# thygate/stable-diffusion-webui-depthmap-script

Measured on AMD Instinct MI355X. Metric: depth+stereo pairs/sec @1024x1024, higher is better.
Workload: dtype f16 (network) / f64 (stereo, normal map); 1 GPU; BASELINE config c3: MiDaS 3.1 DPT BEiT-L/16 512 forward (fp16, random-init weights seed 0, net 512x512, 1025 tokens) + depth->u16 + create_stereoimages(polylines_sharp, left-right, divergence 2.5%) + create_normalmap (Sobel 3) on 32 x 1024x1024 RGB per GPU, inputs resident in HBM; depth_network=dpt_beit_large_512, height=1024, width=1024, forward_launch=eager, library_convolutions=MIOpen, heuristic solver choice, overlap=single stream, parallelism=units sharded over 1 GPU(s), no data-path collective

## Files before the change

include/depthstereo.h:

```cpp
#ifndef DEPTHSTEREO_H
#define DEPTHSTEREO_H

#include <stddef.h>
#include <stdint.h>

#ifdef __cplusplus
extern "C" {
#endif

#define DS_VERSION 100

#define DS_OK            0
#define DS_EINVAL       -1
#define DS_EUNSUPPORTED -2
#define DS_EHIP         -3
#define DS_ENOMEM       -4

#define DS_DEPTH_U16 0
#define DS_DEPTH_F32 1
#define DS_DEPTH_F64 2

#define DS_FILL_NONE                0
#define DS_FILL_NAIVE               1
#define DS_FILL_NAIVE_INTERPOLATING 2
// ... 72 lines not shown
int ds_normalmap_gradient_blur_f32_wrap(ds_ctx *ctx, const float *depth, int n, int h, int w, int pre_blur, int post_blur, int invert,
                                        uint8_t *out, void *stream);

int ds_bilateral_u16(ds_ctx *ctx, const uint16_t *depth, int n, int h, int w, int radius, const double *ws, const double *wr,
                     int wrap, double *out, void *stream);

int ds_frame_luma_hist(ds_ctx *ctx, const uint8_t *frames, int n, int h, int w, int c, uint32_t *hist, void *stream);

int ds_temporal_smooth5_f32(ds_ctx *ctx, const float *src, int m, int64_t plane, int first, int count, int lo, int hi, float *out,
                            void *stream);

int ds_normalmap_selfcheck(ds_ctx *ctx, unsigned long long k0, unsigned long long stride, unsigned long long count,
                           unsigned long long *mismatches, void *stream);

int ds_depth_to_u16(ds_ctx *ctx, const float *pred, int n, int h, int w, int invert,
                    uint16_t *out, float *norm_out, void *stream);

int ds_colorize_u16(ds_ctx *ctx, const uint16_t *depth, int n, int h, int w, const double *vmin_vmax,
                    const uint8_t *lut_rgba, int lut_n, uint8_t *out, void *stream);

int ds_convert_to_i16(ds_ctx *ctx, const void *arr, int is_f64, int64_t count, uint16_t *out, void *stream);

#define DS_PIX_U8  0
#define DS_PIX_U16 1
#define DS_PIX_I32 2
#define DS_PIX_F32 3

int ds_resize_lanczos(ds_ctx *ctx, const void *src, int pix, int n, int in_h, int in_w, int64_t src_px_stride, int64_t src_row_stride,
                      int64_t src_img_stride, void *dst, int out_h, int out_w, const int32_t *h_bounds, const void *h_coeffs, int h_taps,
                      const int32_t *v_bounds, const void *v_coeffs, int v_taps, void *tmp, void *stream);

#define DS_CD_WIDEN       0
#define DS_CD_SINGLE_BAND 1
#define DS_CD_MULTI_BAND  2
#define DS_CD_WORKSPACE_BLOCKS 256
int ds_custom_depth_to_f64(ds_ctx *ctx, const void *src, int pix, int n, int h, int w, int64_t src_px_stride, int64_t src_row_stride,
                           int64_t src_img_stride, int rule, double *out, double *workspace, void *stream);

#define DS_DTYPE_F16  1
#define DS_DTYPE_BF16 2
#define DS_DTYPE_F32  3

int ds_attention_fwd(ds_ctx *ctx, const void *qk, const void *vt, const void *bias_packed, void *out,
                     int B, int Np, int H, int n_valid, float scale, int dtype, void *stream);

int ds_attention_bias_pack(ds_ctx *ctx, const float *bias, int H, int n, int Np, int dtype, void *packed, void *stream);

int ds_attention_reload_env(void);

int ds_preprocess_bicubic(ds_ctx *ctx, const void *images, void *out, int batch, int in_h, int in_w, int out_h, int out_w,
                          int flip_channels, const float *mean, const float *std, int dtype, void *stream);

int ds_residual_layernorm(ds_ctx *ctx, const void *x, const void *branch, const void *gamma, const void *ln_weight,
                          const void *ln_bias, void *x_out, void *h_out, int64_t rows, int channels, float eps, int dtype,
                          void *stream);

int ds_reassemble_readout(ds_ctx *ctx, const void *proj, const void *clsvec, void *out, int batch, int tokens, int channels,
                          int dtype, void *stream);

int ds_bias_act_nhwc(ds_ctx *ctx, const void *x, const void *bias, const void *res1, const void *res2, void *out,
                     int64_t elements, int channels, int relu, int dtype, void *stream);

int ds_group_norm_nchw(ds_ctx *ctx, const void *x, const void *gamma, const void *beta, const void *res, void *out, int n, int channels,
                       int hw, int groups, float eps, int relu, int dtype, void *stream);

int ds_linear(ds_ctx *ctx, const void *x, const void *w, const void *bias, void *y, int64_t rows, int64_t out_features,
              int64_t in_features, int64_t ldy, int act, int dtype, void *stream);

int ds_linear_residual(ds_ctx *ctx, const void *x, const void *w, const void *bias, const void *gamma, const void *res, void *y,
                       int64_t rows, int64_t out_features, int64_t in_features, int dtype, void *stream);

int ds_linear_vt(ds_ctx *ctx, const void *w_v, const void *h, void *vt, int64_t channels, int64_t batch, int64_t tokens,
                 int64_t in_features, int dtype, void *stream);

int ds_linear_qkv(ds_ctx *ctx, const void *h, const void *w_qk, const void *b_qk, const void *w_v, void *qk, void *vt,
                  int64_t batch, int64_t tokens, int64_t qk_features, int64_t v_channels, int64_t in_features, int dtype, void *stream);

int ds_linear_shuffle(ds_ctx *ctx, const void *x, const void *w, const void *bias, void *y, int64_t pixels, int64_t in_features,
                      int width, int stride, int out_channels, int dtype, void *stream);

int ds_linear_readout(ds_ctx *ctx, const void *x, const void *w_tok, const void *cls_vec, void *y, int64_t images,
                      int64_t tokens_padded, int64_t tokens, int64_t out_features, int64_t in_features, int dtype, void *stream);

int ds_row_stats(ds_ctx *ctx, const void *x, void *stats, int64_t rows, int channels, float eps, int dtype, void *stream);
int ds_linear_ln(ds_ctx *ctx, const void *x, const void *w_scaled, const float *colsum, const void *bias, const void *stats, void *y,
                 int64_t rows, int64_t out_features, int64_t in_features, int64_t ldy, int act, int dtype, void *stream);
int ds_linear_vt_ln(ds_ctx *ctx, const void *w_v_scaled, const float *colsum, const void *x, const void *stats, void *vt,
                    int64_t channels, int64_t batch, int64_t tokens, int64_t in_features, int dtype, void *stream);

int ds_linear_reload_env(void);

int ds_conv3x3_nhwc(ds_ctx *ctx, const void *x, const void *w, const void *bias, const void *res1, const void *res2, void *y,
                    int batch, int height, int width, int in_channels, int out_channels, int act, int dtype, void *stream);

int ds_conv3x3_nhwc_circular(ds_ctx *ctx, const void *x, const void *w, const void *bias, const void *res1, const void *res2, void *y,
                             int batch, int height, int width, int in_channels, int out_channels, int act, int dtype, void *stream);

int ds_upsample_bilinear_nhwc(ds_ctx *ctx, const void *in, void *out, int batch, int channels, int in_h, int in_w,
                              int out_h, int out_w, int align_corners, int dtype, void *stream);

int ds_dpt_head_tail(ds_ctx *ctx, const void *x, int batch, int in_h, int in_w, int out_h, int out_w,
                     const void *conv3_wfrag, const float *conv3_bias, const float *conv1_weight, float conv1_bias,
                     int relu_out, void *out, int dtype, void *stream);

int ds_dpt_head_tail_circular(ds_ctx *ctx, const void *x, int batch, int in_h, int in_w, int out_h, int out_w,
                              const void *conv3_wfrag, const float *conv3_bias, const float *conv1_weight, float conv1_bias,
                              int relu_out, void *out, int dtype, void *stream);

int ds_gconv3x3_nhwc_f32(ds_ctx *ctx, const float *x, const float *w_gtio, const float *bias, float *y, int batch, int height, int width,
                         int channels, int channels_per_group, int relu, void *stream);
int ds_add_relu_f32(ds_ctx *ctx, const float *a, const float *b, float *y, int64_t count, void *stream);

int ds_bias_act_f32(ds_ctx *ctx, const float *x, const float *bias, const float *res, float *y, int64_t pixels, int channels, int relu,
                    void *stream);

int ds_dwconv_nhwc(ds_ctx *ctx, const void *x, const float *w, const float *bias_in, const float *bias, void *y, int batch, int in_h,
                   int in_w, int channels, int out_h, int out_w, int kernel, int stride, int pad_top, int pad_left, int dtype, void *stream);
int ds_relu_cat_f32(ds_ctx *ctx, const float *a, const float *b, float *y, int batch, int64_t plane, int channels_a, int channels_b, int layout,
                    void *stream);

int ds_boost_blend(ds_ctx *ctx, float *dst, int64_t dst_row_stride, int height, int width, const void *patches,
                   int n_patches, const float *preds, int pred_size, const float *mask_template, int mask_size,
                   void *stream);

int ds_preprocess_bicubic_rows(ds_ctx *ctx, const void *images, void *rows, int batch, int in_h, int in_w, int out_h, int out_w,
                               int flip_channels, const float *mean, const float *std, int patch, int n_pad, int kpad, int dtype,
                               void *stream);

int ds_tokens_fixup(ds_ctx *ctx, void *tokens, const void *cls, int batch, int n_pad, int n_valid, int channels, int dtype, void *stream);

int ds_upsample_bicubic_to_f32(ds_ctx *ctx, const void *in, void *out, int batch, int in_h, int in_w, int out_h, int out_w, int dtype,
                               void *stream);

int ds_im2col3x3_s2_nhwc(ds_ctx *ctx, const void *x, void *rows, int batch, int height, int width, int channels, int circular, int dtype,
                         void *stream);

#ifdef __cplusplus
}
#endif
#endif
```

stable-diffusion-webui-depthmap-script_amd/csrc/ds_linear.hip:

```cpp
#include "ds_common.h"

#include <stdlib.h>
#include <atomic>
#include <type_traits>

typedef _Float16 lf16x8 __attribute__((ext_vector_type(8)));
typedef __bf16 lbf16x8 __attribute__((ext_vector_type(8)));
typedef _Float16 lf16x4 __attribute__((ext_vector_type(4)));
typedef __bf16 lbf16x4 __attribute__((ext_vector_type(4)));
typedef float lf32x16 __attribute__((ext_vector_type(16)));
typedef float lf32x4 __attribute__((ext_vector_type(4)));

#if defined(DS_EXPERIMENTS) && defined(DS_LIN_MFMA32)
#define LN_MF16 0
#else
#define LN_MF16 1
#endif

#define LN_THREADS 512
#define LN_LDS_BYTES 131072
#define LN_HALF 16384
#define LN_B_BASE 65536

template <int BF16> struct ln_traits;
template <> struct ln_traits<0> {
    typedef _Float16 T; typedef lf16x8 V8; typedef lf16x4 V4;
    static __device__ __forceinline__ lf32x16 mfma(V8 a, V8 b, lf32x16 c) { return __builtin_amdgcn_mfma_f32_32x32x16_f16(a, b, c, 0, 0, 0); }
    static __device__ __forceinline__ lf32x4 mfma16(V8 a, V8 b, lf32x4 c) { return __builtin_amdgcn_mfma_f32_16x16x32_f16(a, b, c, 0, 0, 0); }
    static __device__ __forceinline__ V8 relu(V8 v)
    {
        typedef unsigned lu32x4 __attribute__((ext_vector_type(4)));
        const lu32x4 x = __builtin_bit_cast(lu32x4, v);
        unsigned r0, r1, r2, r3;
        asm("v_pk_max_f16 %0, %1, 0" : "=v"(r0) : "v"(x[0]));
        asm("v_pk_max_f16 %0, %1, 0" : "=v"(r1) : "v"(x[1]));
        asm("v_pk_max_f16 %0, %1, 0" : "=v"(r2) : "v"(x[2]));
        asm("v_pk_max_f16 %0, %1, 0" : "=v"(r3) : "v"(x[3]));
        return __builtin_bit_cast(V8, (lu32x4){r0, r1, r2, r3});
    }
};
template <> struct ln_traits<1> {
    typedef __bf16 T; typedef lbf16x8 V8; typedef lbf16x4 V4;
    static __device__ __forceinline__ lf32x16 mfma(V8 a, V8 b, lf32x16 c) { return __builtin_amdgcn_mfma_f32_32x32x16_bf16(a, b, c, 0, 0, 0); }
    static __device__ __forceinline__ lf32x4 mfma16(V8 a, V8 b, lf32x4 c) { return __builtin_amdgcn_mfma_f32_16x16x32_bf16(a, b, c, 0, 0, 0); }
    static __device__ __forceinline__ V8 relu(V8 v)
    {
        typedef unsigned lu32x4 __attribute__((ext_vector_type(4)));
        lu32x4 x = __builtin_bit_cast(lu32x4, v);
#pragma unroll
        for (int i = 0; i < 4; ++i) {
            const unsigned neg = (x[i] >> 15) & 0x00010001u;
            x[i] &= ~(neg * 0xffffu);
        }
        return __builtin_bit_cast(V8, x);
    }
};

struct LinParams {
    const void *x, *w, *bias;
    const void *res1, *res2;
    const void *zeros;
    void *y;
    int M, N, K;
    int nbm, nbn;
    int bnw;
    int ablate;
    int stagger;
    int H, W, C, cpt, magic;
    long long ldy;
    const void *gamma;
    int early;
    int n_main;
    int vt_np, vt_c;
    unsigned vt_magic;
    int ps_w, ps_s, ps_c;
    unsigned ps_w_magic, ps_c_magic;
    int rd_np, rd_n, rd_dummy;
    unsigned rd_magic;
    float *rg_ws;
    int *rg_cnt;
    int rg_ksl;
    int th_nrb;
    int kt_kind;
    const float2 *ln_stats;
    const float *ln_colsum;
    const void *x1, *w1;
    void *y1;
    int seg_t0, M1, nbm1, nbn1;
};
typedef const __attribute__((address_space(4))) LinParams *LinParamsK;
__device__ __forceinline__ LinParamsK ln_kernarg()
{
    LinParamsK pk = (LinParamsK)__builtin_amdgcn_kernarg_segment_ptr();
    asm volatile("" : "+s"(pk));
    return pk;
}

__device__ __forceinline__ void ln_tile_origin(const int nbm, const int nbn, const int M, const int bnw, const int tile, int &bm0, int &bn0)
{
    const int grp8 = tile / (8 * nbn), rem8 = tile - grp8 * (8 * nbn);
    const int rows8 = min(8, nbm - 8 * grp8);
    const int bn = rem8 / rows8, bm = 8 * grp8 + (rem8 - bn * rows8);
    bm0 = min(bm * 256, M - 256);
    bn0 = bn * bnw;
}
__device__ __forceinline__ void ln_tile_origin(const LinParams &P, const int tile, int &bm0, int &bn0)
{
    ln_tile_origin(P.nbm, P.nbn, P.M, P.bnw, tile, bm0, bn0);
}

template <int VT>
__device__ __forceinline__ size_t ln_out_off(const LinParams &P, const int row, const int col)
{
    if (VT == 0) return (size_t)row * P.ldy + col;
    if (VT == 1) {
        const unsigned b = __umulhi((unsigned)col, P.vt_magic);
        const unsigned n = (unsigned)col - b * (unsigned)P.vt_np;
        return ((size_t)b * P.vt_c + row) * (size_t)P.vt_np + n;
    }
    if (VT == 2) {
        const unsigned q = __umulhi((unsigned)row, P.ps_w_magic), x = (unsigned)row - q * (unsigned)P.ps_w;
        const unsigned t = __umulhi((unsigned)col, P.ps_c_magic), co = (unsigned)col - t * (unsigned)P.ps_c;
        const unsigned ky = t / (unsigned)P.ps_s, kx = t - ky * (unsigned)P.ps_s;
        const size_t opix = ((size_t)q * P.ps_s + ky) * ((size_t)P.ps_w * P.ps_s) + (size_t)x * P.ps_s + kx;
        return opix * (size_t)P.ps_c + co;
    }
    const unsigned b = __umulhi((unsigned)row, P.rd_magic), t = (unsigned)row - b * (unsigned)P.rd_np;
    const bool live = t >= 1u && t < (unsigned)P.rd_n;
    const size_t orow = live ? (size_t)b * (size_t)(P.rd_n - 1) + (t - 1u) : (size_t)P.rd_dummy;
    return orow * (size_t)P.ldy + col;
}
template <int VT>
__device__ __forceinline__ size_t ln_res_off(const LinParams &P, const int row, const int col)
{
    if (VT != 3) return ln_out_off<VT>(P, row, col);
    const unsigned b = __umulhi((unsigned)row, P.rd_magic);
    return (size_t)b * (size_t)P.ldy + col;
}

__device__ __forceinline__ float ln_gelu(float v)
{
    const float u = fminf(fabsf(v), 6.0f);
    float q = 1.8896206483987044e-06f;
    q = __builtin_fmaf(q, u, -6.268127617659047e-05f);
    q = __builtin_fmaf(q, u, 0.000938866869546473f);
    q = __builtin_fmaf(q, u, -0.008539456874132156f);
    q = __builtin_fmaf(q, u, 0.054020676761865616f);
    q = __builtin_fmaf(q, u, 0.45840978622436523f);
    q = __builtin_fmaf(q, u, 1.1512691974639893f);
    q = __builtin_fmaf(q, u, 0.9999943375587463f);
    const float h = __builtin_amdgcn_exp2f(-q);
    return __builtin_fmaf(-u, h, fmaxf(v, 0.0f));
}
typedef float lf32x2 __attribute__((ext_vector_type(2)));
__device__ __forceinline__ lf32x2 ln_gelu2(lf32x2 v)
{
    const lf32x2 u = {fminf(fabsf(v[0]), 6.0f), fminf(fabsf(v[1]), 6.0f)};
    lf32x2 q = {1.8896206483987044e-06f, 1.8896206483987044e-06f};
#define LN_PK(c) q = __builtin_elementwise_fma(q, u, (lf32x2){c, c})
    LN_PK(-6.268127617659047e-05f); LN_PK(0.000938866869546473f); LN_PK(-0.008539456874132156f); LN_PK(0.054020676761865616f);
    LN_PK(0.45840978622436523f); LN_PK(1.1512691974639893f); LN_PK(0.9999943375587463f);
#undef LN_PK
    const lf32x2 h = {__builtin_amdgcn_exp2f(-q[0]), __builtin_amdgcn_exp2f(-q[1])};
    const lf32x2 r = {fmaxf(v[0], 0.0f), fmaxf(v[1], 0.0f)};
    return __builtin_elementwise_fma(-u, h, r);
}

__device__ __forceinline__ void ln_dma_s(const void *base_uniform, unsigned voff, unsigned lds_uniform)
{
    asm volatile("s_mov_b32 m0, %2\n\ts_nop 0\n\tglobal_load_lds_dwordx4 %0, %1" ::"v"(voff), "s"(base_uniform), "s"(lds_uniform) : "memory");
}
__device__ __forceinline__ void ln_dma_v(const void *ptr, unsigned lds_uniform)
{
    asm volatile("s_mov_b32 m0, %1\n\ts_nop 0\n\tglobal_load_lds_dwordx4 %0, off" ::"v"(ptr), "s"(lds_uniform) : "memory");
}

#ifdef DS_EXPERIMENTS
#define LN_ABLATE(bit) (P.ablate & (bit))
#define LN_STAGGER() (P.stagger)
#else
#define LN_ABLATE(bit) 0
#define LN_STAGGER() 0
#endif
#define LN_WAIT_VM(n) asm volatile("s_waitcnt vmcnt(" #n ")" ::: "memory")
template <int N> __device__ __forceinline__ void ln_wait_vm() { asm volatile("s_waitcnt vmcnt(%0)" ::"n"(N) : "memory"); }
#define LN_WAIT_LGKM0() asm volatile("s_waitcnt lgkmcnt(0)" ::: "memory")
#define LN_BARRIER()                              \
    do {                                          \
        __builtin_amdgcn_sched_barrier(0);        \
        __builtin_amdgcn_s_barrier();             \
        __builtin_amdgcn_sched_barrier(0);        \
    } while (0)

template <int BF16, int EPI, int CONV, int RES, int VT = 0, int NH = 0>
__global__ __launch_bounds__(LN_THREADS) void k_linear256(LinParams P)
{
    typedef ln_traits<BF16> TR;
    typedef typename TR::T T;
    typedef typename TR::V8 V8;
    extern __shared__ __attribute__((aligned(1024))) unsigned char lds[];

    const int tid = threadIdx.x;
    const int lane = tid & 63;
    const int wid = __builtin_amdgcn_readfirstlane(tid >> 6);
    const int wr = wid >> 2, wc = wid & 3;

    const int nwg = P.n_main;
    const int K = P.K;
    const int rowbytes = (CONV ? P.C : K) * (int)sizeof(T);

    unsigned srcA[2], srcB[2];
    int rowA[2];
#pragma unroll
    for (int i = 0; i < 2; ++i) {
        const int c = 2 * wid + i;
        const int j = 8 * c + (lane >> 3);
        const int slot = (lane & 7) ^ ((j >> 1) & 7);
        rowA[i] = (j >> 6) * 128 + (j & 63);
        srcA[i] = (unsigned)rowA[i] * (unsigned)rowbytes + slot * 16;
        const int col = NH ? j : (j >> 5) * 64 + (j & 31);
        srcB[i] = (unsigned)col * (unsigned)K * (unsigned)sizeof(T) + slot * 16;
    }
    const unsigned a_half = 64u * (unsigned)rowbytes;
    const unsigned b_half = NH ? 0u : 32u * (unsigned)K * (unsigned)sizeof(T);
    const unsigned lds_stage = (unsigned)(size_t)(__attribute__((address_space(3))) void *)lds + (unsigned)(2 * wid) * 1024u;

    static_assert(VT != 4 || (EPI == 0 && CONV == 0 && RES == 0 && NH == 0), "the two-segment tile list is built for the plain dense epilogue");
    int bm0 = 0, bn0 = 0;
    int seg = 0;
    const unsigned char *xb = nullptr, *wb = nullptr;
    unsigned okA = 0;
    auto set_tile = [&](const int orig) {
        const int xcd = orig & 7, q8 = nwg >> 3, r8 = nwg & 7;
        const int tile = (xcd < r8 ? xcd * (q8 + 1) : r8 * (q8 + 1) + (xcd - r8) * q8) + (orig >> 3);
        if constexpr (VT == 4) {
            const LinParamsK pk = ln_kernarg();
            const int t0 = pk->seg_t0;
            seg = tile >= t0 ? 1 : 0;
            if (seg) {
                ln_tile_origin(pk->nbm1, pk->nbn1, pk->M1, 256, tile - t0, bm0, bn0);
                xb = (const unsigned char *)pk->x1 + (size_t)bm0 * rowbytes;
                wb = (const unsigned char *)pk->w1 + (size_t)bn0 * K * sizeof(T);
                return;
            }
        }
        ln_tile_origin(P, tile, bm0, bn0);
        xb = (const unsigned char *)P.x + (size_t)bm0 * rowbytes;
        wb = (const unsigned char *)P.w + (size_t)bn0 * K * sizeof(T);
        if (CONV) {
            okA = 0;
#pragma unroll
            for (int i = 0; i < 2; ++i)
#pragma unroll
                for (int h = 0; h < 2; ++h) {
                    const unsigned pix = (unsigned)(bm0 + rowA[i] + 64 * h) % (unsigned)(P.H * P.W);
                    const int py = (int)(pix / (unsigned)P.W), px = (int)(pix % (unsigned)P.W);
                    const unsigned bits = (py > 0 ? 1u : 0u) | 2u | (py < P.H - 1 ? 4u : 0u) | (px > 0 ? 8u : 0u) | 16u | (px < P.W - 1 ? 32u : 0u);
                    okA |= bits << (6 * (2 * h + i));
                }
        }
    };

#define LN_STAGE(kind, kt, s)                                                                                            \
    do {                                                                                                                 \
        unsigned koff_ = (unsigned)(kt) * 128u;                                                                          \
        const unsigned dst_ = ((kind) >> 1) * LN_B_BASE + ((kind) & 1) * 2 * LN_HALF + (s) * LN_HALF + lds_stage;   \
        int dy_ = 0, dx_ = 0, aoff_ = (int)koff_;                                                                        \
        long wrapy_ = 0, wrapx_ = 0;      \
        if (CONV) {               \
            const int cc_ = ((kt) * 7282) >> 16, tap_ = (kt) - 9 * cc_;       \
            dy_ = ((tap_ * 11) >> 5) - 1; dx_ = tap_ - 3 * (dy_ + 1) - 1;                                                \
            aoff_ = cc_ * 128 + (dy_ * P.W + dx_) * rowbytes;                                                            \
            koff_ = (unsigned)(tap_ * P.cpt + cc_) * 128u;                            \
            if (CONV >= 3) { wrapy_ = -(long)dy_ * ((long)P.H * P.W * rowbytes); wrapx_ = -(long)dx_ * ((long)P.W * rowbytes); } \
        }                                                                                                                \
                   \
        const unsigned char *ub_ = ((kind) < 2) ? xb + ((long)aoff_ + (long)(((kind) & 1) * a_half))                     \
                                                : wb + (size_t)(((kind) & 1) * b_half + koff_);                          \
        _Pragma("unroll") for (int i_ = 0; i_ < 2; ++i_) {                                                               \
            if (CONV >= 3 && (kind) < 2) {    \
                const unsigned sh_ = 6 * (2 * ((kind) & 1) + i_);     \
                const long wrap_ = (((okA >> (sh_ + dy_ + 1)) & 1u) ? 0l : wrapy_) + (((okA >> (sh_ + 4 + dx_)) & 1u) ? 0l : wrapx_); \
                ln_dma_v(ub_ + ((long)srcA[i_] + wrap_), dst_ + i_ * 1024);                                              \
            } else if (CONV && (kind) < 2) {                                                                             \
                const unsigned sh_ = 6 * (2 * ((kind) & 1) + i_);                                                        \
                const unsigned ok_ = (okA >> (sh_ + dy_ + 1)) & (okA >> (sh_ + 4 + dx_)) & 1u;                           \
                const unsigned char *g_ = ok_ ? ub_ + (size_t)srcA[i_] : (const unsigned char *)P.zeros;                 \
                ln_dma_v(g_, dst_ + i_ * 1024);                                                                          \
            } else {                                                                                                     \
                ln_dma_s(ub_, ((kind) < 2) ? srcA[i_] : srcB[i_], dst_ + i_ * 1024);                                     \
            }                                                                                                            \
        }                                                                                                                \
    } while (0)

    constexpr bool MF16 = LN_MF16 && CONV == 0;
    constexpr int NKS = MF16 ? 2 : 4;
    unsigned offA[NKS], offB[NKS];
#pragma unroll
    for (int ks = 0; ks < NKS; ++ks) {
        const int lrow = MF16 ? (lane & 15) : (lane & 31);
        const unsigned sl = (unsigned)((MF16 ? 4 * ks + (lane >> 4) : 2 * ks + (lane >> 5)) ^ ((lane >> 1) & 7)) << 4;
        offA[ks] = (unsigned)(wr * 64 + lrow) * 128u + sl;
        offB[ks] = LN_B_BASE + (unsigned)(wc * 32 + lrow) * 128u + sl;
    }
    const int c8 = MF16 ? 16 * ((lane >> 4) & 1) + 8 * (lane >> 5) : 8 * (lane >> 5);
    constexpr int NBK = MF16 ? 1 : 2;
    constexpr int NBIAS = 2 * NBK;
    V8 bv[2][2];
#define LN_NULL_BIAS() (!P.bias || (VT == 4 && seg))
#define LN_LOAD_BIAS()                                                                                                   \
    do {                                                                                                                 \
        const T *bias_ = LN_NULL_BIAS() ? (const T *)nullptr : (const T *)P.bias;                                        \
        _Pragma("unroll") for (int hb_ = 0; hb_ < 2; ++hb_) _Pragma("unroll") for (int k_ = 0; k_ < NBK; ++k_) {         \
            const int c_ = bn0 + (NH ? wc * 32 : wc * 64 + hb_ * 32) + c8 + 16 * k_;                                     \
            bv[hb_][k_] = *(const V8 *)(bias_ ? bias_ + c_ : (const T *)P.w);                                            \
        }                                                                                                                \
    } while (0)
#define LN_ZERO_NULL_BIAS()                                                                                              \
    do {                                                                                                                 \
        if (LN_NULL_BIAS()) {                                                                                            \
            _Pragma("unroll") for (int hb_ = 0; hb_ < 2; ++hb_) _Pragma("unroll") for (int k_ = 0; k_ < NBK; ++k_)       \
                _Pragma("unroll") for (int t_ = 0; t_ < 8; ++t_) bv[hb_][k_][t_] = (T)0.f;                               \
        }                                                                                                                \
    } while (0)
    V8 fa[2][2][4];
    V8 fb[2][4];
    lf32x16 acc[2][2][2];
    V8 fa16[2][4][2];
    V8 fb16[2][2][2];
    lf32x4 acc16[2][4][2][2];

#define LN_READ_A(h, s)                                                                                                  \
    do {                                                                                                                 \
        if constexpr (MF16) {                                                                                            \
            _Pragma("unroll") for (int rb_ = 0; rb_ < 4; ++rb_) _Pragma("unroll") for (int ks_ = 0; ks_ < 2; ++ks_)      \
                fa16[h][rb_][ks_] = *(const V8 *)(lds + offA[ks_] + ((h) * 2 * LN_HALF + (s) * LN_HALF + rb_ * 2048));   \
        } else {                                                                                                         \
            _Pragma("unroll") for (int rb_ = 0; rb_ < 2; ++rb_) _Pragma("unroll") for (int ks_ = 0; ks_ < 4; ++ks_)      \
                fa[h][rb_][ks_] = *(const V8 *)(lds + offA[ks_] + ((h) * 2 * LN_HALF + (s) * LN_HALF + rb_ * 4096));     \
        }                                                                                                                \
    } while (0)
#define LN_RELU_A(h)                                                                                                     \
    do {                                                                                                                 \
        if constexpr (CONV == 2 || CONV == 4) {                                                                          \
            _Pragma("unroll") for (int rb_ = 0; rb_ < 2; ++rb_) _Pragma("unroll") for (int ks_ = 0; ks_ < 4; ++ks_)      \
                fa[h][rb_][ks_] = TR::relu(fa[h][rb_][ks_]);                                                             \
        }                                                                                                                \
    } while (0)
#define LN_READ_B(h, s)                                                                                                  \
    do {                                                                                                                 \
        if constexpr (MF16) {                                                                                            \
            _Pragma("unroll") for (int cb_ = 0; cb_ < 2; ++cb_) _Pragma("unroll") for (int ks_ = 0; ks_ < 2; ++ks_)      \
                if (!(NH && (h) == 1)) fb16[h][cb_][ks_] = *(const V8 *)(lds + offB[ks_] + ((h) * 2 * LN_HALF + (s) * LN_HALF + cb_ * 2048)); \
        } else {                                                                                                         \
            _Pragma("unroll") for (int ks_ = 0; ks_ < 4; ++ks_)                                                          \
// ... 32 lines not shown
    } while (0)
#define LN_MEM(READ, STAGE)                                                                                              \
    do { READ; STAGE; } while (0)

    auto iteration = [&](const int i, auto kind_c) {
        constexpr int KIND = decltype(kind_c)::value;
        constexpr bool LAST = KIND == 1;
        const int e2 = 2 * i + 2, o2 = 2 * i + 3;
#define LN_WAIT_HEAD()                                                                                                   \
        do {                                                                                                             \
            if constexpr (KIND == 2) { if constexpr (NH) LN_WAIT_VM(18); else LN_WAIT_VM(26); }                          \
            else if constexpr (KIND == 1) ln_wait_vm<10 + NBIAS>();                                                   \
            else LN_WAIT_VM(10);                                                                                         \
        } while (0)
        LN_MEM(LN_READ_B(0, 0), LN_STAGE(1, 2 * i + 1, 1)); LN_WAIT_HEAD();
        LN_PHASE_END(0, 0);
        if constexpr (!LAST) { LN_MEM(LN_READ_B(1, 0), LN_STAGE(0, e2, 0)); LN_WAIT_HEAD(); } else { LN_READ_B(1, 0); ln_wait_vm<8 + NBIAS>(); }
        LN_PHASE_END(0, 1);
        if constexpr (!LAST) { LN_MEM(LN_READ_A(1, 0), LN_STAGE(2, e2, 0)); LN_RELU_A(1); LN_WAIT_HEAD(); } else { LN_READ_A(1, 0); LN_RELU_A(1); ln_wait_vm<6 + NBIAS>(); }
        LN_PHASE_END(1, 1);
        if constexpr (!LAST) { LN_MEM(LN_READ_A(0, 1), LN_STAGE(3, e2, 0)); LN_RELU_A(0); LN_WAIT_HEAD(); } else { LN_READ_A(0, 1); LN_RELU_A(0); ln_wait_vm<4 + NBIAS>(); }
        LN_PHASE_END(1, 0);
        if constexpr (!LAST) { LN_MEM(LN_READ_B(0, 1), LN_STAGE(1, e2, 0)); LN_WAIT_HEAD(); } else { LN_READ_B(0, 1); ln_wait_vm<2 + NBIAS>(); }
        LN_PHASE_END(0, 0);
#undef LN_WAIT_HEAD
        if constexpr (!LAST) { LN_MEM(LN_READ_B(1, 1), LN_STAGE(0, o2, 1)); LN_WAIT_VM(10); } else { LN_READ_B(1, 1); LN_WAIT_VM(0); }
        LN_PHASE_END(0, 1);
        if constexpr (!LAST) { LN_MEM(LN_READ_A(1, 1), LN_STAGE(2, o2, 1)); LN_RELU_A(1); LN_WAIT_VM(10); } else { LN_READ_A(1, 1); LN_RELU_A(1); }
        LN_PHASE_END(1, 1);
        if constexpr (!LAST) { LN_MEM(LN_READ_A(0, 0), LN_STAGE(3, o2, 1)); LN_RELU_A(0); LN_WAIT_VM(10); }
        LN_PHASE_END(1, 0);
    };
    if (LN_STAGGER() > 0 && ((blockIdx.x >> 3) & 1)) {
        const unsigned long long t0 = wall_clock64();
        while (wall_clock64() - t0 < (unsigned long long)LN_STAGGER()) __builtin_amdgcn_s_sleep(32);
    }
    const bool early = P.early != 0;
    bool stores_ahead = false;
    set_tile(blockIdx.x);
    LN_PROLOGUE();
    for (int orig = blockIdx.x;;) {
    if constexpr (MF16) {
#pragma unroll
        for (int a = 0; a < 2; ++a)
#pragma unroll
            for (int b = 0; b < 4; ++b)
#pragma unroll
                for (int c = 0; c < 2; ++c)
#pragma unroll
                    for (int d = 0; d < 2; ++d)
#pragma unroll
                        for (int r = 0; r < 4; ++r) acc16[a][b][c][d][r] = 0.f;
    } else {
#pragma unroll
        for (int a = 0; a < 2; ++a)
#pragma unroll
            for (int b = 0; b < 2; ++b)
#pragma unroll
                for (int c = 0; c < 2; ++c)
#pragma unroll
                    for (int r = 0; r < 16; ++r) acc[a][b][c][r] = 0.f;
    }
    if (!early) LN_WAIT_VM(10);
    else if (stores_ahead) { if constexpr (NH) LN_WAIT_VM(18); else LN_WAIT_VM(26); }
    else LN_WAIT_VM(0);
    LN_BARRIER();
    LN_READ_A(0, 0);
    LN_WAIT_LGKM0();
    LN_RELU_A(0);
    if (wr == 1) LN_BARRIER();
    if (LN_ABLATE(2)) {
        LN_LOAD_BIAS();
        LN_WAIT_VM(0);
        if (wr == 0) LN_BARRIER();
    } else {
        int i0 = 0;
        if (early && ni >= 2) { iteration(0, std::integral_constant<int, 2>()); i0 = 1; }
        for (int i = i0; i < ni - 1; ++i) iteration(i, std::integral_constant<int, 0>());
        LN_LOAD_BIAS();
        iteration(ni - 1, std::integral_constant<int, 1>());
        if (wr == 0) LN_BARRIER();
    }
    const int cbm0 = bm0, cbn0 = bn0;
    const bool cseg = VT == 4 && seg != 0;
    const int next = orig + (int)gridDim.x;
    int elane = lane;
    if constexpr (VT == 4) asm volatile("" : "+v"(elane));
    const int hi8 = 8 * (elane >> 5);
    const int ec8 = MF16 ? 16 * ((elane >> 4) & 1) + 8 * (elane >> 5) : 8 * (elane >> 5);
    LN_ZERO_NULL_BIAS();
    T *yb = (T *)P.y;
    unsigned s1_np = 0, s1_c = 0, s1_magic = 0;
    if constexpr (VT == 4) {
        if (cseg) {
            const LinParamsK pk = ln_kernarg();
            yb = (T *)pk->y1;
            s1_np = (unsigned)pk->vt_np; s1_c = (unsigned)pk->vt_c; s1_magic = pk->vt_magic;
        }
    }
    auto tile_out_off = [&](const int row, const int col, const size_t o0) -> size_t {
        if constexpr (VT == 4) {
            if (!cseg) return o0;
            const unsigned b = __umulhi((unsigned)col, s1_magic), n = (unsigned)col - b * s1_np;
            return ((size_t)b * s1_c + row) * (size_t)s1_np + n;
        } else return VT ? ln_out_off<VT>(P, row, col) : o0;
    };
    if constexpr (CONV >= 3) asm volatile("" : "+s"(yb));
    const T *r1 = (const T *)P.res1, *r2 = (const T *)P.res2;
    if (early && next < nwg) {
#pragma unroll
        for (int hb = 0; hb < 2; ++hb)
#pragma unroll
            for (int k = 0; k < NBK; ++k) {
                asm volatile("" ::"v"(bv[hb][k]));
            }
        set_tile(next);
        LN_PROLOGUE();
    }

    if constexpr (MF16) {
        V8 gv[2];
        if (EPI == 3) {
#pragma unroll
            for (int hb = 0; hb < 2; ++hb) gv[hb] = *(const V8 *)((const T *)P.gamma + cbn0 + (NH ? wc * 32 : wc * 64 + hb * 32) + ec8);
        }
        constexpr int NHB = NH ? 1 : 2;
        const int wcol = NH ? wc * 32 : wc * 64;
#pragma unroll
        for (int ha = 0; ha < 2; ++ha)
#pragma unroll
            for (int rb = 0; rb < 4; ++rb) {
                const int row = cbm0 + wr * 128 + ha * 64 + rb * 16 + (elane & 15);
                const int col = cbn0 + wcol + ec8;
                const size_t o0 = (size_t)row * P.ldy + col;
                V8 ra[2], rb2[2];
                constexpr bool LNF = EPI == 4 || EPI == 5;
                float2 st_row = {1.f, 0.f};
                float cs_row = 0.f;
                static_assert(!LNF || VT == 0 || VT == 1, "the folded LayerNorm exists for the row-major and the V^T store only");
                if (LNF && VT == 0) st_row = P.ln_stats[row];
                if (LNF && VT == 1) cs_row = P.ln_colsum[row];
#pragma unroll
                for (int hb = 0; hb < NHB; ++hb) {
                    if (RES >= 1) ra[hb] = *(const V8 *)(r1 + (VT == 3 ? ln_res_off<VT>(P, row, col + hb * 32) : o0 + hb * 32));
                    if (RES >= 2) rb2[hb] = *(const V8 *)(r2 + o0 + hb * 32);
                }
#pragma unroll
                for (int hb = 0; hb < NHB; ++hb) {
                    float v[8];
#pragma unroll
                    for (int t = 0; t < 4; ++t) {
                        const float fa = acc16[ha][rb][hb][0][t], fb = acc16[ha][rb][hb][1][t];
                        const auto sw = __builtin_amdgcn_permlane16_swap(__float_as_uint(fa), __float_as_uint(fb), false, false);
                        v[t] = __uint_as_float(sw[0]);
                        v[4 + t] = __uint_as_float(sw[1]);
                    }
                    V8 o;
                    if (LNF) {
                        const int c0 = col + hb * 32;
                        if (!VT) {
                            const float4 s0 = *(const float4 *)(P.ln_colsum + c0), s1 = *(const float4 *)(P.ln_colsum + c0 + 4);
                            const float sc[8] = {s0.x, s0.y, s0.z, s0.w, s1.x, s1.y, s1.z, s1.w};
#pragma unroll
                            for (int t = 0; t < 8; ++t) v[t] = __builtin_fmaf(v[t], st_row.x, st_row.y * sc[t]);
                        } else {
                            const float4 *sp = (const float4 *)(P.ln_stats + c0);
                            const float4 q0 = sp[0], q1 = sp[1], q2 = sp[2], q3 = sp[3];
                            const float rs[8] = {q0.x, q0.z, q1.x, q1.z, q2.x, q2.z, q3.x, q3.z};
                            const float nm[8] = {q0.y, q0.w, q1.y, q1.w, q2.y, q2.w, q3.y, q3.w};
#pragma unroll
                            for (int t = 0; t < 8; ++t) v[t] = __builtin_fmaf(v[t], rs[t], nm[t] * cs_row);
                        }
                    }
#pragma unroll
                    for (int t = 0; t < 8; t += 2) {
                        lf32x2 u = {v[t] + (float)bv[hb][0][t], v[t + 1] + (float)bv[hb][0][t + 1]};
                        if (EPI == 3) u *= (lf32x2){(float)gv[hb][t], (float)gv[hb][t + 1]};
                        if (RES >= 1) u += (lf32x2){(float)ra[hb][t], (float)ra[hb][t + 1]};
                        if (RES >= 2) u += (lf32x2){(float)rb2[hb][t], (float)rb2[hb][t + 1]};
                        if (EPI == 1 || EPI == 5) u = ln_gelu2(u);
                        if (EPI == 2) u = (lf32x2){fmaxf(u[0], 0.f), fmaxf(u[1], 0.f)};
                        o[t] = (T)u[0];
                        o[t + 1] = (T)u[1];
                    }
                    T *dst = yb + tile_out_off(row, col + hb * 32, o0 + hb * 32);
                    if (!LN_ABLATE(1)) *(V8 *)dst = o;
                    else asm volatile("" ::"v"(o));
// ... 362 lines not shown
        const int j = 8 * (wid & 3) + (lane >> 3);
        srcA = (unsigned)j * rowbytes + (unsigned)(((lane & 7) ^ ((j >> 1) & 7)) << 4) + (unsigned)(wid >> 2) * 128u;
    }
#pragma unroll
    for (int i = 0; i < 2; ++i) {
        const int j = 8 * ((2 * wid + i) & 7) + (lane >> 3);
        srcB[i] = (unsigned)j * rowbytes + (unsigned)(((lane & 7) ^ ((j >> 1) & 7)) << 4) + (unsigned)(wid >> 2) * 128u;
    }
    const unsigned char *xb = (const unsigned char *)P.x + (size_t)row0 * rowbytes;
    const unsigned char *wb = (const unsigned char *)P.w + (size_t)col0 * rowbytes;
    const unsigned lds0 = (unsigned)(size_t)(__attribute__((address_space(3))) void *)lds;
#define TH_STAGE(st_)                                                                                                    \
    do {                                                                                                                 \
        const int sc_ = min((st_), nst - 1);                 \
        const unsigned sl_ = lds0 + (unsigned)((st_) % S) * RG_SLOT;                                                      \
        const unsigned char *xa_ = xb + (size_t)sc_ * 256, *wa_ = wb + (size_t)sc_ * 256;                                 \
        ln_dma_s(xa_, srcA, sl_ + (unsigned)wid * 1024u);                                                                 \
        ln_dma_s(wa_, srcB[0], sl_ + 8192u + (unsigned)(2 * wid) * 1024u);                                                \
        ln_dma_s(wa_, srcB[1], sl_ + 8192u + (unsigned)(2 * wid + 1) * 1024u);                                            \
    } while (0)
    const bool mw = wid < 2;
    unsigned offA[8], offB[8];
#pragma unroll
    for (int u = 0; u < 8; ++u) {
        const int j = u >> 2, ks = u & 3;
        const unsigned sl = (unsigned)((LN_MF16 ? 4 * (ks >> 1) + (lane >> 4) : 2 * ks + hi) ^ ((lane >> 1) & 7)) << 4;
        const int lrow = LN_MF16 ? 16 * (ks & 1) + (lane & 15) : l31;
        offA[u] = (unsigned)j * 4096u + (unsigned)lrow * 128u + sl;
        offB[u] = 8192u + (unsigned)j * 8192u + (unsigned)((wid & 1) * 32 + lrow) * 128u + sl;
    }
    LN_SMALL_ACC(mine);
    const int e_row = row0 + LN_SMALL_ROW;
    const int e_cb = col0 + (wid & 1) * 32 + LN_SMALL_COL;
    V8 e_bv[2], e_gv[2], e_rv[2];
    if (mw) {
#pragma unroll
        for (int k = 0; k < 2; ++k) {
            const int row = e_row + LN_SMALL_DROW(k), col = e_cb + LN_SMALL_DCOL(k);
            if (P.bias) e_bv[k] = *(const V8 *)((const T *)P.bias + col);
            if (EPI == 3) e_gv[k] = *(const V8 *)((const T *)P.gamma + col);
            if (RES >= 1) e_rv[k] = *(const V8 *)((const T *)P.res1 + (size_t)row * P.ldy + col);
        }
    }
#pragma unroll
    for (int t = 0; t < S - 1; ++t) TH_STAGE(t);
    V8 fa0[8], fb0[8], fa1[8], fb1[8];
#define TH_READ(fa_, fb_, st_)                                                                                           \
    do {                                                                                                                 \
        const unsigned char *sb_ = lds + ((st_) % S) * RG_SLOT;                                                          \
        _Pragma("unroll") for (int u = 0; u < 8; ++u) {                                                                  \
            fa_[u] = *(const V8 *)(sb_ + offA[u]);                                                                       \
            fb_[u] = *(const V8 *)(sb_ + offB[u]);                                                                       \
        }                                                                                                                \
    } while (0)
#define TH_STEP(ca_, cb_, na_, nb_, st_)                                                                                 \
    do {                                                                                                                 \
        LN_WAIT_VM(9);                                                                                                   \
        LN_BARRIER();                                                                                                    \
        TH_STAGE((st_) + S - 1);                                                                                         \
        if (mw) {                                                                                                        \
            TH_READ(na_, nb_, (st_) + 1);                                                                                \
            __builtin_amdgcn_sched_barrier(0);                                                                           \
            LN_SMALL_MMA(mine, cb_, ca_, 0);                                                                             \
            LN_SMALL_MMA(mine, cb_, ca_, 4);                                                                             \
            __builtin_amdgcn_sched_barrier(0);                                                                           \
            LN_WAIT_LGKM0();                                                                                             \
            __builtin_amdgcn_sched_barrier(0);                                                                           \
        }                                                                                                                \
    } while (0)
    LN_WAIT_VM(12);
    LN_BARRIER();
    if (mw) {
        TH_READ(fa0, fb0, 0);
        __builtin_amdgcn_sched_barrier(0);
        LN_WAIT_LGKM0();
        __builtin_amdgcn_sched_barrier(0);
    }
    int st = 0;
    for (; st + 1 < nst; st += 2) {
        TH_STEP(fa0, fb0, fa1, fb1, st);
        TH_STEP(fa1, fb1, fa0, fb0, st + 1);
    }
    if (st < nst) TH_STEP(fa0, fb0, fa1, fb1, st);
#undef TH_STEP
#undef TH_READ
#undef TH_STAGE
    LN_WAIT_VM(0);
    if (!mw) return;

    T *yb = (T *)P.y;
#pragma unroll
    for (int k = 0; k < 2; ++k) {
        const int row = e_row + LN_SMALL_DROW(k), col = e_cb + LN_SMALL_DCOL(k);
        const size_t off = (size_t)row * P.ldy + col;
        V8 bv;
        if (P.bias) bv = e_bv[k];
        else {
#pragma unroll
            for (int t = 0; t < 8; ++t) bv[t] = (T)0.f;
        }
        float v[8];
        LN_SMALL_V(v, mine, k);
        if (EPI == 4 || EPI == 5) {
            const float2 stt = P.ln_stats[row];
            const float4 s0 = *(const float4 *)(P.ln_colsum + col), s1 = *(const float4 *)(P.ln_colsum + col + 4);
            const float sc[8] = {s0.x, s0.y, s0.z, s0.w, s1.x, s1.y, s1.z, s1.w};
#pragma unroll
            for (int t = 0; t < 8; ++t) v[t] = __builtin_fmaf(v[t], stt.x, stt.y * sc[t]);
        }
        V8 o;
#pragma unroll
        for (int t = 0; t < 8; t += 2) {
            lf32x2 u = {v[t] + (float)bv[t], v[t + 1] + (float)bv[t + 1]};
            if (EPI == 3) u *= (lf32x2){(float)e_gv[k][t], (float)e_gv[k][t + 1]};
            if (RES >= 1) u += (lf32x2){(float)e_rv[k][t], (float)e_rv[k][t + 1]};
            if (EPI == 1 || EPI == 5) u = ln_gelu2(u);
            if (EPI == 2) u = (lf32x2){fmaxf(u[0], 0.f), fmaxf(u[1], 0.f)};
            o[t] = (T)u[0];
            o[t + 1] = (T)u[1];
        }
        *(V8 *)(yb + off) = o;
    }
}

struct LinOptions { int early, grid, ragged, ragged_den, ragged_ring, ragged_ksplit, ragged_ksplit_min, ragged_ksplit_keep, ragged_pipe, ragged_thin; };
static LinOptions g_lin_options;
static std::atomic<int> g_lin_options_state{0};
static void ln_read_options()
{
    auto geti = [](const char *name, int dflt) { const char *e = getenv(name); return e ? atoi(e) : dflt; };
    LinOptions o;
    o.early = geti("DS_LIN_EARLY", 1);
    o.grid = geti("DS_LIN_GRID", 0);
    o.ragged = geti("DS_LIN_RAGGED", 1);
    o.ragged_den = geti("DS_LIN_RAGGED_DEN", 4);
    o.ragged_ring = geti("DS_LIN_RAGGED_RING", 0);
    o.ragged_ksplit = geti("DS_LIN_RAGGED_KSPLIT", 1);
    o.ragged_ksplit_min = geti("DS_LIN_RAGGED_KSPLIT_MIN", 32);
    o.ragged_ksplit_keep = geti("DS_LIN_RAGGED_KSPLIT_KEEP", 8);
    if (o.ragged_ksplit_keep < 1) o.ragged_ksplit_keep = 1;
    o.ragged_pipe = geti("DS_LIN_RAGGED_PIPE", 1);
    o.ragged_thin = geti("DS_LIN_RAGGED_THIN", 1);
    g_lin_options = o;
    g_lin_options_state.store(1, std::memory_order_release);
}
static const LinOptions &ln_options()
{
    if (!g_lin_options_state.load(std::memory_order_acquire)) ln_read_options();
    return g_lin_options;
}
DS_API int ds_linear_reload_env(void)
{
    ln_read_options();
    return DS_OK;
}

#define LN_RG_COUNTER_BYTES 4096
#define LN_RG_MAX_WG 1024
static int ln_ragged_workspace(ds_ctx *ctx, int grid, hipStream_t stream)
{
    if (grid > LN_RG_MAX_WG) return 1;
    if (ctx->lin_ws && ctx->lin_ws_cleared == ctx->lin_ws) return DS_OK;
    hipStreamCaptureStatus cap = hipStreamCaptureStatusNone;
    if (hipStreamIsCapturing(stream, &cap) != hipSuccess || cap != hipStreamCaptureStatusNone) { (void)hipGetLastError(); return 1; }
    if (!ctx->lin_ws) {
        const int rc = ds_ctx_reserve(ctx, &ctx->lin_ws, &ctx->lin_ws_bytes, LN_RG_COUNTER_BYTES + (size_t)LN_RG_MAX_WG * 32768);
        if (rc != DS_OK) return rc;
    }
    DS_HIP_CHECK(hipMemsetAsync(ctx->lin_ws, 0, LN_RG_COUNTER_BYTES, stream));
    DS_HIP_CHECK(hipStreamSynchronize(stream));
    ctx->lin_ws_cleared = ctx->lin_ws;
    return DS_OK;
}

static int ln_ksplit_arch_ok(ds_ctx *ctx)
{
    static std::atomic<uint64_t> checked{0}, ok{0};
    const uint64_t bit = 1ull << (ctx->device & 63);
    if (!(checked.load(std::memory_order_acquire) & bit)) {
        hipDeviceProp_t prop;
        bool good = false;
        if (hipGetDeviceProperties(&prop, ctx->device) == hipSuccess)
            good = strncmp(prop.gcnArchName, "gfx950", 6) == 0 || strncmp(prop.gcnArchName, "gfx942", 6) == 0;
        else (void)hipGetLastError();
        if (good) ok.fetch_or(bit, std::memory_order_relaxed);
        checked.fetch_or(bit, std::memory_order_release);
    }
    return (ok.load(std::memory_order_relaxed) & bit) != 0;
}

template <int BF16, int EPI, int CONV, int RES, int VT = 0, int NH = 0>
static int ln_launch(ds_ctx *ctx, const LinParams &P0, hipStream_t stream)
{
    static std::atomic<uint64_t> attr_done{0};
    auto fn = k_linear256<BF16, EPI, CONV, RES, VT, NH>;
    DS_HIP_CHECK(hipSetDevice(ctx->device));
    const uint64_t bit = 1ull << (ctx->device & 63);
    if (!(attr_done.load(std::memory_order_relaxed) & bit)) {
        DS_HIP_CHECK(hipFuncSetAttribute((const void *)fn, hipFuncAttributeMaxDynamicSharedMemorySize, LN_LDS_BYTES));
        if constexpr (CONV == 0) {
            DS_HIP_CHECK(hipFuncSetAttribute((const void *)k_linear_ragged<BF16, EPI, RES, VT, 3>, hipFuncAttributeMaxDynamicSharedMemorySize, 3 * RG_SLOT));
            DS_HIP_CHECK(hipFuncSetAttribute((const void *)k_linear_ragged<BF16, EPI, RES, VT, 6>, hipFuncAttributeMaxDynamicSharedMemorySize, 6 * RG_SLOT));
            DS_HIP_CHECK(hipFuncSetAttribute((const void *)k_linear_ragged<BF16, EPI, RES, VT, 6, 1>, hipFuncAttributeMaxDynamicSharedMemorySize, 6 * RG_SLOT));
            if constexpr (VT == 0 && RES <= 1)
                DS_HIP_CHECK(hipFuncSetAttribute((const void *)k_linear_thin<BF16, EPI, RES>, hipFuncAttributeMaxDynamicSharedMemorySize, 6 * RG_SLOT));
        }
// ... 165 lines not shown
    P.ablate = getenv("DS_LIN_ABLATE") ? atoi(getenv("DS_LIN_ABLATE")) : 0;
    P.stagger = getenv("DS_LIN_STAGGER_US") ? (int)(atof(getenv("DS_LIN_STAGGER_US")) * 100.0) : 0;
#endif
    return dtype == DS_DTYPE_F16 ? ln_dispatch_dense<0>(ctx, P, act, (hipStream_t)stream) : ln_dispatch_dense<1>(ctx, P, act, (hipStream_t)stream);
}

DS_API int ds_linear_residual(ds_ctx *ctx, const void *x, const void *w, const void *bias, const void *gamma, const void *res, void *y,
                              int64_t rows, int64_t out_features, int64_t in_features, int dtype, void *stream)
{
    DS_REQUIRE(ctx && x && w && y && res, DS_EINVAL, "ds_linear_residual: null argument");
    DS_REQUIRE(rows >= 256 && rows < (1ll << 31) - 256, DS_EINVAL, "ds_linear_residual: rows must be >= 256 (one tile)");
    DS_REQUIRE(out_features > 0 && out_features % 256 == 0, DS_EINVAL, "ds_linear_residual: out_features must be a multiple of 256");
    DS_REQUIRE(in_features >= 128 && in_features % 128 == 0 && in_features <= 16384, DS_EINVAL,
               "ds_linear_residual: in_features must be a multiple of 128 (<= 16384)");
    DS_REQUIRE(dtype == DS_DTYPE_F16 || dtype == DS_DTYPE_BF16, DS_EINVAL, "ds_linear_residual: dtype must be f16 or bf16");
    DS_REQUIRE(((uintptr_t)x & 15) == 0 && ((uintptr_t)w & 15) == 0 && ((uintptr_t)y & 15) == 0 && ((uintptr_t)res & 15) == 0 &&
               ((uintptr_t)bias & 15) == 0 && ((uintptr_t)gamma & 15) == 0 && y != res,
               DS_EINVAL, "ds_linear_residual: x, w, y, res, bias and gamma must be 16-byte aligned, and y must not alias res");
    LinParams P;
    memset(&P, 0, sizeof(P));
    P.x = x; P.w = w; P.bias = bias; P.gamma = gamma; P.res1 = res; P.y = y;
    P.M = (int)rows; P.N = (int)out_features; P.K = (int)in_features;
    P.nbm = (int)((rows + 255) / 256); P.nbn = (int)(out_features / 256);
    P.ldy = out_features;
    P.kt_kind = DS_KT_LINEAR_RESIDUAL;
    hipStream_t st = (hipStream_t)stream;
    if (dtype == DS_DTYPE_F16) return gamma ? ln_launch<0, 3, 0, 1>(ctx, P, st) : ln_launch<0, 0, 0, 1>(ctx, P, st);
    return gamma ? ln_launch<1, 3, 0, 1>(ctx, P, st) : ln_launch<1, 0, 0, 1>(ctx, P, st);
}

template <int CIRC>
static int ln_conv3x3(const char *NAME, ds_ctx *ctx, const void *x, const void *w, const void *bias, const void *res1, const void *res2, void *y,
                      int batch, int height, int width, int in_channels, int out_channels, int act, int dtype, void *stream)
{
    DS_REQUIRE(ctx && x && w && y, DS_EINVAL, "%s: null argument", NAME);
    DS_REQUIRE(batch > 0 && height > 0 && width > 0 && height < 32768 && width < 32768, DS_EINVAL, "%s: bad image shape", NAME);
    DS_REQUIRE((int64_t)batch * height * width < (1ll << 31) - 256 && (int64_t)batch * height * width >= 256, DS_EINVAL,
               "%s: batch * height * width must be in [256, 2^31)", NAME);
    DS_REQUIRE(in_channels >= 64 && in_channels % 64 == 0 && (9 * in_channels / 64) % 2 == 0 && in_channels <= 4096, DS_EINVAL,
               "%s: in_channels must be a multiple of 128 (<= 4096)", NAME);
    DS_REQUIRE(out_channels > 0 && out_channels % 128 == 0, DS_EINVAL, "%s: out_channels must be a multiple of 128", NAME);
    DS_REQUIRE(out_channels % 256 == 0 || (!res1 && !res2), DS_EUNSUPPORTED,
               "%s: residual operands need out_channels to be a multiple of 256 (the 128-column tiles have no residual epilogue)", NAME);
    DS_REQUIRE(act == 0 || act == 2 || act == 6, DS_EINVAL, "%s: act must be 0 (none), 2 (ReLU) or 6 (ReLU, and ReLU on x)", NAME);
    DS_REQUIRE(dtype == DS_DTYPE_F16 || dtype == DS_DTYPE_BF16, DS_EINVAL, "%s: dtype must be f16 or bf16", NAME);
    DS_REQUIRE(((uintptr_t)x & 15) == 0 && ((uintptr_t)w & 15) == 0 && ((uintptr_t)y & 15) == 0 && (!bias || ((uintptr_t)bias & 15) == 0) &&
               ((uintptr_t)res1 & 15) == 0 && ((uintptr_t)res2 & 15) == 0,
               DS_EINVAL, "%s: x, w, y, bias, res1 and res2 must be 16-byte aligned", NAME);
    int rc = ds_ctx_reserve(ctx, &ctx->zero_line, &ctx->zero_line_bytes, 256);
    if (rc != DS_OK) return rc;
    if (!ctx->zero_line_cleared) {
        DS_HIP_CHECK(hipMemsetAsync(ctx->zero_line, 0, 256, (hipStream_t)stream));
        DS_HIP_CHECK(hipStreamSynchronize((hipStream_t)stream));
        ctx->zero_line_cleared = 1;
    }
    LinParams P;
    memset(&P, 0, sizeof(P));
    if (!res1 && res2) { res1 = res2; res2 = nullptr; }
    P.x = x; P.w = w; P.bias = bias; P.res1 = res1; P.res2 = res2; P.y = y; P.zeros = ctx->zero_line;
    P.M = batch * height * width; P.N = out_channels; P.K = 9 * in_channels;
    P.nbm = (P.M + 255) / 256; P.nbn = out_channels % 256 == 0 ? out_channels / 256 : out_channels / 128;
    P.H = height; P.W = width; P.C = in_channels; P.cpt = in_channels / 64; P.magic = 65536 / P.cpt + 1;
    for (int kt = 0; kt < P.K / 64; ++kt)
        DS_REQUIRE(((kt * 7282) >> 16) == kt / 9, DS_EUNSUPPORTED, "%s: K-tile arithmetic does not cover %d channels", NAME, in_channels);
    P.ldy = out_channels;
    P.kt_kind = DS_KT_CONV3X3;
#ifdef DS_EXPERIMENTS
    P.ablate = getenv("DS_LIN_ABLATE") ? atoi(getenv("DS_LIN_ABLATE")) : 0;
    P.stagger = getenv("DS_LIN_STAGGER_US") ? (int)(atof(getenv("DS_LIN_STAGGER_US")) * 100.0) : 0;
#endif
    return dtype == DS_DTYPE_F16 ? ln_dispatch_conv<0, CIRC>(ctx, P, act, (hipStream_t)stream) : ln_dispatch_conv<1, CIRC>(ctx, P, act, (hipStream_t)stream);
}

DS_API int ds_conv3x3_nhwc(ds_ctx *ctx, const void *x, const void *w, const void *bias, const void *res1, const void *res2, void *y,
                           int batch, int height, int width, int in_channels, int out_channels, int act, int dtype, void *stream)
{
    return ln_conv3x3<0>("ds_conv3x3_nhwc", ctx, x, w, bias, res1, res2, y, batch, height, width, in_channels, out_channels, act, dtype, stream);
}

DS_API int ds_conv3x3_nhwc_circular(ds_ctx *ctx, const void *x, const void *w, const void *bias, const void *res1, const void *res2, void *y,
                                    int batch, int height, int width, int in_channels, int out_channels, int act, int dtype, void *stream)
{
    return ln_conv3x3<1>("ds_conv3x3_nhwc_circular", ctx, x, w, bias, res1, res2, y, batch, height, width, in_channels, out_channels, act, dtype, stream);
}

DS_API int ds_linear_vt(ds_ctx *ctx, const void *w_v, const void *h, void *vt, int64_t channels, int64_t batch, int64_t tokens,
                        int64_t in_features, int dtype, void *stream)
{
    DS_REQUIRE(ctx && w_v && h && vt, DS_EINVAL, "ds_linear_vt: null argument");
    DS_REQUIRE(channels >= 256, DS_EINVAL, "ds_linear_vt: channels must be >= 256 (one tile)");
    DS_REQUIRE(batch > 0 && tokens > 0 && tokens % 8 == 0 && (batch * tokens) % 256 == 0 && batch * tokens < (1ll << 31) - 256, DS_EINVAL,
               "ds_linear_vt: tokens must be a multiple of 8 and batch * tokens a multiple of 256");
    DS_REQUIRE(batch * tokens * tokens < (1ll << 32), DS_EUNSUPPORTED, "ds_linear_vt: batch * tokens^2 must stay below 2^32");
    DS_REQUIRE(in_features >= 128 && in_features % 128 == 0 && in_features <= 16384, DS_EINVAL,
               "ds_linear_vt: in_features must be a multiple of 128 (<= 16384)");
    DS_REQUIRE(dtype == DS_DTYPE_F16 || dtype == DS_DTYPE_BF16, DS_EINVAL, "ds_linear_vt: dtype must be f16 or bf16");
    DS_REQUIRE(((uintptr_t)w_v & 15) == 0 && ((uintptr_t)h & 15) == 0 && ((uintptr_t)vt & 15) == 0, DS_EINVAL,
               "ds_linear_vt: w_v, h and vt must be 16-byte aligned");
    LinParams P;
    memset(&P, 0, sizeof(P));
    P.x = w_v; P.w = h; P.y = vt;
    P.M = (int)channels; P.N = (int)(batch * tokens); P.K = (int)in_features;
    P.nbm = (int)((channels + 255) / 256); P.nbn = (int)(batch * tokens / 256);
    P.ldy = batch * tokens;
    P.vt_np = (int)tokens; P.vt_c = (int)channels; P.vt_magic = (unsigned)((1ull << 32) / (unsigned long long)tokens + 1ull);
    P.kt_kind = DS_KT_LINEAR_VT;
    hipStream_t st = (hipStream_t)stream;
    return dtype == DS_DTYPE_F16 ? ln_launch<0, 0, 0, 0, 1>(ctx, P, st) : ln_launch<1, 0, 0, 0, 1>(ctx, P, st);
}

DS_API int ds_linear_qkv(ds_ctx *ctx, const void *h, const void *w_qk, const void *b_qk, const void *w_v, void *qk, void *vt,
                         int64_t batch, int64_t tokens, int64_t qk_features, int64_t v_channels, int64_t in_features, int dtype, void *stream)
{
    DS_REQUIRE(ctx && h && w_qk && w_v && qk && vt, DS_EINVAL, "ds_linear_qkv: null argument");
    DS_REQUIRE(batch > 0 && tokens > 0 && tokens % 8 == 0 && (batch * tokens) % 256 == 0 && batch * tokens < (1ll << 31) - 256, DS_EINVAL,
               "ds_linear_qkv: tokens must be a multiple of 8 and batch * tokens a multiple of 256");
    DS_REQUIRE(batch * tokens * tokens < (1ll << 32), DS_EUNSUPPORTED, "ds_linear_qkv: batch * tokens^2 must stay below 2^32");
    DS_REQUIRE(qk_features > 0 && qk_features % 256 == 0, DS_EINVAL, "ds_linear_qkv: qk_features must be a multiple of 256");
    DS_REQUIRE(v_channels >= 256 && v_channels < (1ll << 31) - 256, DS_EINVAL, "ds_linear_qkv: v_channels must be >= 256 (one tile)");
    DS_REQUIRE(in_features >= 128 && in_features % 128 == 0 && in_features <= 16384, DS_EINVAL,
               "ds_linear_qkv: in_features must be a multiple of 128 (<= 16384)");
    DS_REQUIRE((batch * tokens / 256) * (qk_features / 256) + ((v_channels + 255) / 256) * (batch * tokens / 256) < (1ll << 31), DS_EINVAL,
               "ds_linear_qkv: too many tiles");
    DS_REQUIRE(dtype == DS_DTYPE_F16 || dtype == DS_DTYPE_BF16, DS_EINVAL, "ds_linear_qkv: dtype must be f16 or bf16");
    DS_REQUIRE(((uintptr_t)h & 15) == 0 && ((uintptr_t)w_qk & 15) == 0 && ((uintptr_t)w_v & 15) == 0 && ((uintptr_t)qk & 15) == 0 &&
               ((uintptr_t)vt & 15) == 0 && (!b_qk || ((uintptr_t)b_qk & 15) == 0), DS_EINVAL,
               "ds_linear_qkv: h, w_qk, w_v (the LDS-DMA sources), qk, vt and b_qk must be 16-byte aligned");
    const int64_t rows = batch * tokens;
    LinParams PQ, PV;
    memset(&PQ, 0, sizeof(PQ));
    memset(&PV, 0, sizeof(PV));
    PQ.x = h; PQ.w = w_qk; PQ.bias = b_qk; PQ.y = qk;
    PQ.M = (int)rows; PQ.N = (int)qk_features; PQ.K = (int)in_features;
    PQ.nbm = (int)(rows / 256); PQ.nbn = (int)(qk_features / 256);
    PQ.ldy = qk_features;
    PQ.kt_kind = DS_KT_LINEAR;
    PV.x = w_v; PV.w = h; PV.y = vt;
    PV.M = (int)v_channels; PV.N = (int)rows; PV.K = (int)in_features;
    PV.nbm = (int)((v_channels + 255) / 256); PV.nbn = (int)(rows / 256);
    PV.ldy = rows;
    PV.vt_np = (int)tokens; PV.vt_c = (int)v_channels; PV.vt_magic = (unsigned)((1ull << 32) / (unsigned long long)tokens + 1ull);
    PV.kt_kind = DS_KT_LINEAR;
    hipStream_t st = (hipStream_t)stream;
    return dtype == DS_DTYPE_F16 ? ln_launch_qkv<0>(ctx, PQ, PV, st) : ln_launch_qkv<1>(ctx, PQ, PV, st);
}

DS_API int ds_linear_shuffle(ds_ctx *ctx, const void *x, const void *w, const void *bias, void *y, int64_t pixels, int64_t in_features,
                             int width, int stride, int out_channels, int dtype, void *stream)
{
    DS_REQUIRE(ctx && x && w && y, DS_EINVAL, "ds_linear_shuffle: null argument");
    DS_REQUIRE(stride >= 1 && stride <= 8 && width >= 1 && out_channels >= 8 && out_channels % 8 == 0, DS_EINVAL,
               "ds_linear_shuffle: stride must be 1..8, out_channels a multiple of 8");
    const int64_t n = (int64_t)stride * stride * out_channels;
    DS_REQUIRE(pixels >= 256 && pixels % width == 0 && pixels < (1ll << 31) - 256, DS_EINVAL,
               "ds_linear_shuffle: pixels must be >= 256 (one tile) and a whole number of image rows");
    DS_REQUIRE(n % 256 == 0, DS_EUNSUPPORTED, "ds_linear_shuffle: stride^2 * out_channels must be a multiple of 256 (got %lld)", (long long)n);
    DS_REQUIRE(in_features >= 128 && in_features % 128 == 0 && in_features <= 16384, DS_EINVAL,
               "ds_linear_shuffle: in_features must be a multiple of 128 (<= 16384)");
    DS_REQUIRE(pixels * width < (1ll << 32) && n * out_channels < (1ll << 32) && pixels * n < (1ll << 40), DS_EUNSUPPORTED,
               "ds_linear_shuffle: shape too large for the index arithmetic");
    DS_REQUIRE(dtype == DS_DTYPE_F16 || dtype == DS_DTYPE_BF16, DS_EINVAL, "ds_linear_shuffle: dtype must be f16 or bf16");
    DS_REQUIRE(((uintptr_t)x & 15) == 0 && ((uintptr_t)w & 15) == 0 && ((uintptr_t)y & 15) == 0 && (!bias || ((uintptr_t)bias & 15) == 0), DS_EINVAL,
               "ds_linear_shuffle: x, w, y and bias must be 16-byte aligned");
    LinParams P;
    memset(&P, 0, sizeof(P));
    P.x = x; P.w = w; P.bias = bias; P.y = y;
    P.M = (int)pixels; P.N = (int)n; P.K = (int)in_features;
    P.nbm = (int)((pixels + 255) / 256); P.nbn = (int)(n / 256);
    P.ldy = n;
    P.ps_w = width; P.ps_s = stride; P.ps_c = out_channels;
    P.ps_w_magic = (unsigned)((1ull << 32) / (unsigned long long)width + 1ull);
    P.ps_c_magic = (unsigned)((1ull << 32) / (unsigned long long)out_channels + 1ull);
    P.kt_kind = DS_KT_LINEAR_SHUFFLE;
    hipStream_t st = (hipStream_t)stream;
    return dtype == DS_DTYPE_F16 ? ln_launch<0, 0, 0, 0, 2>(ctx, P, st) : ln_launch<1, 0, 0, 0, 2>(ctx, P, st);
}

DS_API int ds_linear_readout(ds_ctx *ctx, const void *x, const void *w_tok, const void *cls_vec, void *y, int64_t images,
                             int64_t tokens_padded, int64_t tokens, int64_t out_features, int64_t in_features, int dtype, void *stream)
{
    DS_REQUIRE(ctx && x && w_tok && cls_vec && y, DS_EINVAL, "ds_linear_readout: null argument");
    DS_REQUIRE(images > 0 && tokens >= 2 && tokens <= tokens_padded, DS_EINVAL, "ds_linear_readout: need 2 <= tokens <= tokens_padded");
    const int64_t rows = images * tokens_padded;
    DS_REQUIRE(rows >= 256 && rows < (1ll << 31) - 256 && rows * tokens_padded < (1ll << 32), DS_EINVAL,
               "ds_linear_readout: images * tokens_padded must be in [256, 2^31) and images * tokens_padded^2 below 2^32");
    DS_REQUIRE(out_features > 0 && out_features % 256 == 0, DS_EINVAL, "ds_linear_readout: out_features must be a multiple of 256");
    DS_REQUIRE(in_features >= 128 && in_features % 128 == 0 && in_features <= 16384, DS_EINVAL,
               "ds_linear_readout: in_features must be a multiple of 128 (<= 16384)");
    DS_REQUIRE(dtype == DS_DTYPE_F16 || dtype == DS_DTYPE_BF16, DS_EINVAL, "ds_linear_readout: dtype must be f16 or bf16");
    DS_REQUIRE(((uintptr_t)x & 15) == 0 && ((uintptr_t)w_tok & 15) == 0 && ((uintptr_t)y & 15) == 0 && ((uintptr_t)cls_vec & 15) == 0, DS_EINVAL,
               "ds_linear_readout: x, w_tok, cls_vec and y must be 16-byte aligned");
    LinParams P;
    memset(&P, 0, sizeof(P));
    P.x = x; P.w = w_tok; P.res1 = cls_vec; P.y = y;
    P.M = (int)rows; P.N = (int)out_features; P.K = (int)in_features;
    P.nbm = (int)((rows + 255) / 256); P.nbn = (int)(out_features / 256);
    P.ldy = out_features;
    P.rd_np = (int)tokens_padded; P.rd_n = (int)tokens; P.rd_dummy = (int)(images * (tokens - 1));
    P.rd_magic = (unsigned)((1ull << 32) / (unsigned long long)tokens_padded + 1ull);
    P.kt_kind = DS_KT_LINEAR_READOUT;
    hipStream_t st = (hipStream_t)stream;
    return dtype == DS_DTYPE_F16 ? ln_launch<0, 1, 0, 1, 3>(ctx, P, st) : ln_launch<1, 1, 0, 1, 3>(ctx, P, st);
}

DS_API int ds_linear_ln(ds_ctx *ctx, const void *x, const void *w_scaled, const float *colsum, const void *bias, const void *stats, void *y,
                        int64_t rows, int64_t out_features, int64_t in_features, int64_t ldy, int act, int dtype, void *stream)
{
    DS_REQUIRE(ctx && x && w_scaled && colsum && stats && y, DS_EINVAL, "ds_linear_ln: null argument");
    DS_REQUIRE(rows >= 256 && rows < (1ll << 31) - 256, DS_EINVAL, "ds_linear_ln: rows must be >= 256 (one tile)");
    DS_REQUIRE(out_features > 0 && out_features % 256 == 0, DS_EINVAL, "ds_linear_ln: out_features must be a multiple of 256");
    DS_REQUIRE(in_features >= 128 && in_features % 128 == 0 && in_features <= 16384, DS_EINVAL, "ds_linear_ln: in_features must be a multiple of 128 (<= 16384)");
    DS_REQUIRE(ldy >= out_features && ldy % 8 == 0, DS_EINVAL, "ds_linear_ln: ldy must be >= out_features and a multiple of 8");
    DS_REQUIRE(((uintptr_t)x & 15) == 0 && ((uintptr_t)w_scaled & 15) == 0 && ((uintptr_t)y & 15) == 0 && (!bias || ((uintptr_t)bias & 15) == 0) &&
               ((uintptr_t)colsum & 15) == 0 && ((uintptr_t)stats & 15) == 0, DS_EINVAL, "ds_linear_ln: operands must be 16-byte aligned");
    DS_REQUIRE(act == 0 || act == 1, DS_EINVAL, "ds_linear_ln: act must be 0 (none) or 1 (erf-GELU)");
    DS_REQUIRE(dtype == DS_DTYPE_F16 || dtype == DS_DTYPE_BF16, DS_EINVAL, "ds_linear_ln: dtype must be f16 or bf16");
    LinParams P;
    memset(&P, 0, sizeof(P));
    P.x = x; P.w = w_scaled; P.bias = bias; P.y = y; P.ln_stats = (const float2 *)stats; P.ln_colsum = colsum;
    P.M = (int)rows; P.N = (int)out_features; P.K = (int)in_features;
    P.nbm = (int)((rows + 255) / 256); P.nbn = (int)(out_features / 256);
    P.ldy = ldy;
    P.kt_kind = act == 1 ? DS_KT_LINEAR_GELU : DS_KT_LINEAR;
    hipStream_t st = (hipStream_t)stream;
    if (dtype == DS_DTYPE_F16) return act == 1 ? ln_launch<0, 5, 0, 0>(ctx, P, st) : ln_launch<0, 4, 0, 0>(ctx, P, st);
    return act == 1 ? ln_launch<1, 5, 0, 0>(ctx, P, st) : ln_launch<1, 4, 0, 0>(ctx, P, st);
}

DS_API int ds_linear_vt_ln(ds_ctx *ctx, const void *w_v_scaled, const float *colsum, const void *x, const void *stats, void *vt,
                           int64_t channels, int64_t batch, int64_t tokens, int64_t in_features, int dtype, void *stream)
{
    DS_REQUIRE(ctx && w_v_scaled && colsum && x && stats && vt, DS_EINVAL, "ds_linear_vt_ln: null argument");
    DS_REQUIRE(channels >= 256, DS_EINVAL, "ds_linear_vt_ln: channels must be >= 256 (one tile)");
    DS_REQUIRE(batch > 0 && tokens > 0 && tokens % 8 == 0 && (batch * tokens) % 256 == 0 && batch * tokens < (1ll << 31) - 256, DS_EINVAL,
               "ds_linear_vt_ln: tokens must be a multiple of 8 and batch * tokens a multiple of 256");
    DS_REQUIRE(batch * tokens * tokens < (1ll << 32), DS_EUNSUPPORTED, "ds_linear_vt_ln: batch * tokens^2 must stay below 2^32");
    DS_REQUIRE(in_features >= 128 && in_features % 128 == 0 && in_features <= 16384, DS_EINVAL, "ds_linear_vt_ln: in_features must be a multiple of 128 (<= 16384)");
    DS_REQUIRE(dtype == DS_DTYPE_F16 || dtype == DS_DTYPE_BF16, DS_EINVAL, "ds_linear_vt_ln: dtype must be f16 or bf16");
    DS_REQUIRE(((uintptr_t)w_v_scaled & 15) == 0 && ((uintptr_t)x & 15) == 0 && ((uintptr_t)vt & 15) == 0 && ((uintptr_t)colsum & 15) == 0 &&
               ((uintptr_t)stats & 15) == 0, DS_EINVAL, "ds_linear_vt_ln: operands must be 16-byte aligned");
    LinParams P;
    memset(&P, 0, sizeof(P));
    P.x = w_v_scaled; P.w = x; P.y = vt; P.ln_stats = (const float2 *)stats; P.ln_colsum = colsum;
    P.M = (int)channels; P.N = (int)(batch * tokens); P.K = (int)in_features;
    P.nbm = (int)((channels + 255) / 256); P.nbn = (int)(batch * tokens / 256);
    P.ldy = batch * tokens;
    P.vt_np = (int)tokens; P.vt_c = (int)channels; P.vt_magic = (unsigned)((1ull << 32) / (unsigned long long)tokens + 1ull);
    P.kt_kind = DS_KT_LINEAR_VT;
    hipStream_t st = (hipStream_t)stream;
    return dtype == DS_DTYPE_F16 ? ln_launch<0, 4, 0, 0, 1>(ctx, P, st) : ln_launch<1, 4, 0, 0, 1>(ctx, P, st);
}
```

stable-diffusion-webui-depthmap-script_amd/ddepth_anything_v2/depth_anything_v2/dpt.py:

```python
import numpy as np
import torch
import torch.nn as nn
import torch.nn.functional as F

from src import vit_mi355x as vm

from .dinov2 import DINOv2


class ResidualConvUnit(nn.Module):
    def __init__(self, features):
        super().__init__()
        self.conv1 = nn.Conv2d(features, features, kernel_size=3, stride=1, padding=1, bias=True)
        self.conv2 = nn.Conv2d(features, features, kernel_size=3, stride=1, padding=1, bias=True)

    def forward(self, x):
        return vm.residual_conv_unit(self.conv1, self.conv2, x)


class FeatureFusionBlock(nn.Module):
    def __init__(self, features):
        super().__init__()
        self.out_conv = nn.Conv2d(features, features, kernel_size=1, stride=1, padding=0, bias=True)
        self.resConfUnit1 = ResidualConvUnit(features)
        self.resConfUnit2 = ResidualConvUnit(features)

    def forward(self, *xs, size=None):
        output = xs[0]
        if len(xs) == 2:
            output = vm.residual_conv_unit(self.resConfUnit1.conv1, self.resConfUnit1.conv2, xs[1], skip=output)
        output = self.resConfUnit2(output)
        output = vm.conv_module(self.out_conv, output)
        if size is None:
            return vm.interpolate_bilinear(output, scale_factor=2, align_corners=True)
        return vm.interpolate_bilinear(output, size=tuple(size), align_corners=True)


class DPTHead(nn.Module):
    def __init__(self, in_channels, features=256, use_bn=False, out_channels=(256, 512, 1024, 1024), use_clstoken=False):
        super().__init__()
        if use_bn or use_clstoken:
            raise NotImplementedError("use_bn / use_clstoken are never enabled by the reference's model table "
                                      "(src/depthmap_generation.py:243-247)")
        oc = list(out_channels)
        self.projects = nn.ModuleList([nn.Conv2d(in_channels, c, kernel_size=1) for c in oc])
        self.resize_layers = nn.ModuleList([
            nn.ConvTranspose2d(oc[0], oc[0], kernel_size=4, stride=4, padding=0),
            nn.ConvTranspose2d(oc[1], oc[1], kernel_size=2, stride=2, padding=0),
            nn.Identity(),
            nn.Conv2d(oc[3], oc[3], kernel_size=3, stride=2, padding=1)])
        scratch = nn.Module()
        for i in range(4):
            setattr(scratch, f"layer{i + 1}_rn", nn.Conv2d(oc[i], features, kernel_size=3, stride=1, padding=1, bias=False))
        for i in range(1, 5):
            setattr(scratch, f"refinenet{i}", FeatureFusionBlock(features))
        scratch.output_conv1 = nn.Conv2d(features, features // 2, kernel_size=3, stride=1, padding=1)
        scratch.output_conv2 = nn.Sequential(
            nn.Conv2d(features // 2, 32, kernel_size=3, stride=1, padding=1), nn.ReLU(True),
            nn.Conv2d(32, 1, kernel_size=1, stride=1, padding=0), nn.ReLU(True), nn.Identity())
        self.scratch = scratch

    def forward(self, out_features, patch_h, patch_w):
        out = []
        for i, x in enumerate(out_features):
            x = x[0]
            x = x.reshape(x.shape[0], patch_h, patch_w, x.shape[-1]).permute(0, 3, 1, 2)
            if vm.half_on_gpu(x) and not x.is_contiguous(memory_format=torch.channels_last):
                x = x.contiguous(memory_format=torch.channels_last)
            x = vm.conv_module(self.resize_layers[i], vm.conv_module(self.projects[i], x))
            out.append(x)
        l1, l2, l3, l4 = out
        s = self.scratch
        l1, l2, l3, l4 = vm.conv2d(s.layer1_rn, l1), vm.conv2d(s.layer2_rn, l2), vm.conv2d(s.layer3_rn, l3), vm.conv2d(s.layer4_rn, l4)
        path_4 = s.refinenet4(l4, size=l3.shape[2:])
        path_3 = s.refinenet3(path_4, l3, size=l2.shape[2:])
        path_2 = s.refinenet2(path_3, l2, size=l1.shape[2:])
        path_1 = s.refinenet1(path_2, l1)
        out = vm.conv2d(s.output_conv1, path_1)
        size = (int(patch_h * 14), int(patch_w * 14))
        if (vm.half_on_gpu(out) and tuple(s.output_conv2[0].weight.shape) == (32, 128, 3, 3)
                and s.output_conv2[0].padding_mode in ('zeros', 'circular') and vm.circular_hip_ok(s.output_conv2[0])):
            from src import _native
            return _native.dpt_head_tail(out, size, s.output_conv2[0], s.output_conv2[2], relu_out=True)
        out = vm.interpolate_bilinear(out, size=size, align_corners=True)
        return s.output_conv2(out)


_LAYER_IDX = {'vits': [2, 5, 8, 11], 'vitb': [2, 5, 8, 11], 'vitl': [4, 11, 17, 23]}


def _constrain(x, multiple, min_val):
    y = int(np.round(x / multiple) * multiple)
    if y < min_val:
        y = int(np.ceil(x / multiple) * multiple)
    return y


def lower_bound_size(width, height, target, multiple=14):
    scale_h, scale_w = target / height, target / width
    if scale_w > scale_h:
        scale_h = scale_w
    else:
        scale_w = scale_h
    return _constrain(scale_w * width, multiple, target), _constrain(scale_h * height, multiple, target)


class DepthAnythingV2(nn.Module):
    def __init__(self, encoder='vitl', features=256, out_channels=(256, 512, 1024, 1024), use_bn=False, use_clstoken=False):
        super().__init__()
        self.intermediate_layer_idx = dict(_LAYER_IDX)
        self.encoder = encoder
        self.pretrained = DINOv2(model_name=encoder)
        self.depth_head = DPTHead(self.pretrained.embed_dim, features, use_bn, out_channels=out_channels, use_clstoken=use_clstoken)

    @vm.deterministic_forward
    def forward(self, x):
        patch_h, patch_w = x.shape[-2] // 14, x.shape[-1] // 14
        features = self.pretrained.get_intermediate_layers(x, self.intermediate_layer_idx[self.encoder], return_class_token=True)
        depth = self.depth_head(features, patch_h, patch_w)
        return F.relu(depth).squeeze(1)

    @torch.no_grad()
    def image2tensor_device(self, images_u8, input_size=518):
        b, h, w, _ = images_u8.shape
        nw, nh = lower_bound_size(w, h, input_size)
        if images_u8.is_cuda and vm.PREPROCESS_HIP and not vm.STOCK[0]:
            from src import _native
            dtype = self.pretrained.blocks[0].norm1.weight.dtype
            return _native.preprocess_bicubic(images_u8, (nh, nw), vm.IMAGENET_MEAN, vm.IMAGENET_STD, flip=True, dtype=dtype), (h, w)
        x = images_u8.flip(-1).permute(0, 3, 1, 2).float() / 255.0
        x = F.interpolate(x, size=(nh, nw), mode="bicubic", align_corners=False)
        mean = vm.device_constant(vm.IMAGENET_MEAN, x.device).view(1, 3, 1, 1)
        std = vm.device_constant(vm.IMAGENET_STD, x.device).view(1, 3, 1, 1)
        return (x - mean) / std, (h, w)

    @torch.no_grad()
    def infer_batch(self, images_u8, input_size=518):
        x, (h, w) = self.image2tensor_device(images_u8, input_size)
        dtype = self.pretrained.blocks[0].norm1.weight.dtype
        depth = self.forward(x.to(dtype)).float()
        return F.interpolate(depth[:, None], (h, w), mode="bilinear", align_corners=True)[:, 0]
```

stable-diffusion-webui-depthmap-script_amd/dmidas/backbones/beit.py:

```python
import torch
import torch.nn as nn
import torch.nn.functional as F

from src import vit_mi355x as vm


def gen_relative_position_index(window_size):
    num_relative_distance = (2 * window_size[0] - 1) * (2 * window_size[1] - 1) + 3
    window_area = window_size[0] * window_size[1]
    coords = torch.stack(torch.meshgrid([torch.arange(window_size[0]), torch.arange(window_size[1])], indexing='ij'))
    coords_flatten = torch.flatten(coords, 1)
    relative_coords = coords_flatten[:, :, None] - coords_flatten[:, None, :]
    relative_coords = relative_coords.permute(1, 2, 0).contiguous()
    relative_coords[:, :, 0] += window_size[0] - 1
    relative_coords[:, :, 1] += window_size[1] - 1
    relative_coords[:, :, 0] *= 2 * window_size[1] - 1
    relative_position_index = torch.zeros(size=(window_area + 1,) * 2, dtype=relative_coords.dtype)
    relative_position_index[1:, 1:] = relative_coords.sum(-1)
    relative_position_index[0, 0:] = num_relative_distance - 3
    relative_position_index[0:, 0] = num_relative_distance - 2
    relative_position_index[0, 0] = num_relative_distance - 1
    return relative_position_index


# ... 112 lines not shown
        if qe > q0:
            out[:, :qe - q0, :self.n] = self.table[index[q0:qe].reshape(-1)].view(qe - q0, self.n, -1).permute(2, 0, 1)
        return out


class PatchEmbed(nn.Module):
    def __init__(self, patch_size, embed_dim):
        super().__init__()
        self.proj = nn.Conv2d(3, embed_dim, kernel_size=patch_size, stride=patch_size)

    def forward(self, x):
        if vm.patch_embed_hip_ok(self.proj, x):
            return vm.patch_embed_tokens(self.proj, x)
        return self.proj(x).flatten(2).transpose(1, 2)


class Beit(nn.Module):

    def __init__(self, img_size, embed_dim, depth, num_heads, init_values, num_classes=1000):
        super().__init__()
        self.patch_size = [16, 16]
        self.embed_dim = embed_dim
        window = (img_size // 16, img_size // 16)
        self.patch_embed = PatchEmbed(16, embed_dim)
        self.cls_token = nn.Parameter(torch.zeros(1, 1, embed_dim))
        self.blocks = nn.ModuleList([Block(embed_dim, num_heads, window, 4.0, init_values) for _ in range(depth)])
        self.fc_norm = nn.LayerNorm(embed_dim, eps=1e-6)
        self.head = nn.Linear(embed_dim, num_classes)
        nn.init.trunc_normal_(self.cls_token, std=0.02)
        for m in self.modules():
            if isinstance(m, nn.Linear):
                nn.init.trunc_normal_(m.weight, std=0.02)
                if m.bias is not None:
                    nn.init.zeros_(m.bias)

    def forward_taps(self, x, hooks, padded=False):
        grid = (x.shape[2] // 16, x.shape[3] // 16)
        t = self.patch_embed(x)
        t = torch.cat((self.cls_token.expand(t.shape[0], -1, -1).to(t.dtype), t), dim=1)
        n_valid = t.shape[1]
        t = vm.pad_tokens(t, vm.pad_len(n_valid, t.shape[0]))
        _, taps = vm.run_blocks(self.blocks, t, n_valid, grid, set(hooks), padded_taps=padded)
        return [taps[i] for i in hooks], grid, n_valid

    def forward_taps_rows(self, rows, grid, hooks, padded=False):
        n_valid = grid[0] * grid[1] + 1
        t = vm.patch_rows_tokens(self.patch_embed.proj, self.cls_token, rows, n_valid)
        _, taps = vm.run_blocks(self.blocks, t, n_valid, grid, set(hooks), padded_taps=padded)
        return [taps[i] for i in hooks], grid, n_valid


class ProjectReadout(nn.Module):

    def __init__(self, in_features, start_index=1):
        super().__init__()
        self.start_index = start_index
        self.project = nn.Sequential(nn.Linear(2 * in_features, in_features), nn.GELU())

    def _split(self):
        lin = self.project[0]
        key = (lin.weight._version, lin.weight.data_ptr(), lin.weight.dtype)
        hit = getattr(self, "_w_split", None)
        if hit is None or hit[0] != key:
            if hit is not None:
                vm.cache_evicted()
            c = lin.in_features // 2
            hit = (key, lin.weight[:, :c].contiguous(), lin.weight[:, c:].contiguous())
            if not torch.is_grad_enabled():
                self._w_split = hit
        return hit[1], hit[2]

    def forward(self, x):
        if self.start_index != 1:
            readout = x[:, 0].unsqueeze(1).expand_as(x[:, self.start_index:])
            return self.project(torch.cat((x[:, self.start_index:], readout), -1))
        w_tok, w_cls = self._split()
        clsvec = F.linear(x[:, 0], w_cls, self.project[0].bias)
        proj = F.linear(x, w_tok)
        if vm.half_on_gpu(x) and x.shape[-1] % 8 == 0:
            from src import _native
            return _native.reassemble_readout(proj, clsvec)
        return F.gelu(proj[:, 1:] + clsvec[:, None])

    def forward_padded(self, xp, n_valid):
        from src import _native
        w_tok, w_cls = self._split()
        if (self.start_index == 1 and vm.READOUT_HIP and vm.LINEAR_HIP == "all" and vm.half_on_gpu(xp) and xp.is_contiguous()
                and _native.linear_readout_supported(xp, w_tok) and vm.hip_gemm_ok(xp.shape[0] * xp.shape[1], w_tok.shape[0])):
            x0 = xp[:, 0].contiguous()
            if vm.invariant() and _native.linear_supported(x0, w_cls):
                clsvec = _native.linear(x0, w_cls, self.project[0].bias)
            else:
                clsvec = F.linear(x0, w_cls, self.project[0].bias)
            return _native.linear_readout(xp, n_valid, w_tok, clsvec)
        return self.forward(xp[:, :n_valid])


class _Skip(nn.Module):
    def forward(self, x):
        return x


def _postprocess(vit_features, out_features, tail):
    return nn.Sequential(ProjectReadout(vit_features), _Skip(), _Skip(), nn.Conv2d(vit_features, out_features, 1), *tail)


class BeitBackbone(nn.Module):

    def __init__(self, model, features, vit_features, hooks):
        super().__init__()
        self.model = model
        self.hooks = list(hooks)
        f = features
        self.act_postprocess1 = _postprocess(vit_features, f[0], [nn.ConvTranspose2d(f[0], f[0], 4, 4, 0)])
        self.act_postprocess2 = _postprocess(vit_features, f[1], [nn.ConvTranspose2d(f[1], f[1], 2, 2, 0)])
        self.act_postprocess3 = _postprocess(vit_features, f[2], [])
        self.act_postprocess4 = _postprocess(vit_features, f[3], [nn.Conv2d(f[3], f[3], 3, 2, 1)])

    def forward(self, x, rows=None):
        if rows is not None:
            taps, grid, n_valid = self.model.forward_taps_rows(rows[0], rows[1], self.hooks, padded=True)
        else:
            taps, grid, n_valid = self.model.forward_taps(x, self.hooks, padded=True)
        outs = []
        for tap, post in zip(taps, (self.act_postprocess1, self.act_postprocess2, self.act_postprocess3, self.act_postprocess4)):
            y = post[0].forward_padded(tap, n_valid)
            y = y.reshape(y.shape[0], grid[0], grid[1], y.shape[2]).permute(0, 3, 1, 2)
            for layer in list(post)[3:]:
                y = vm.conv_module(layer, y)
            outs.append(y)
        return outs


def make_beit(name, hooks):
    cfg = {"beitl16_512": (512, 1024, 24, 16, [256, 512, 1024, 1024]),
           "beitl16_384": (384, 1024, 24, 16, [256, 512, 1024, 1024]),
           "beitb16_384": (384, 768, 12, 12, [96, 192, 384, 768])}[name]
    img, dim, depth, heads, features = cfg
    model = Beit(img, dim, depth, heads, init_values=1e-5 if dim == 1024 else 0.1)
    return BeitBackbone(model, features, dim, hooks), features
```

stable-diffusion-webui-depthmap-script_amd/dmidas/backbones/vit.py:

```python
import math
import os

import torch
import torch.nn as nn
import torch.nn.functional as F

from src import vit_mi355x as vm
from .beit import ProjectReadout, _Skip


def _pad_same(x, k, s, value=0.0):
    ih, iw = x.shape[-2:]
    ph = max((math.ceil(ih / s) - 1) * s + (k - 1) + 1 - ih, 0)
    pw = max((math.ceil(iw / s) - 1) * s + (k - 1) + 1 - iw, 0)
    if ph > 0 or pw > 0:
        x = F.pad(x, (pw // 2, pw - pw // 2, ph // 2, ph - ph // 2), value=value)
    return x


class StdConv2dSame(nn.Conv2d):

    def __init__(self, in_ch, out_ch, kernel_size, stride=1, eps=1e-8):
        super().__init__(in_ch, out_ch, kernel_size, stride=stride, padding=0, bias=False)
        self.eps = eps
        self._std_cache = None

    def std_weight(self):
        w = self.weight
        key = (w._version, w.dtype, w.device, w.data_ptr())
        if self._std_cache is not None and self._std_cache[0] == key:
            return self._std_cache[1]
        wf = w.float().reshape(w.shape[0], -1)
        mean = wf.mean(dim=1, keepdim=True)
        var = wf.var(dim=1, keepdim=True, unbiased=False)
        ws = ((wf - mean) / torch.sqrt(var + self.eps)).reshape_as(w).to(w.dtype)
        if not torch.is_grad_enabled():
            if self._std_cache is not None:
                vm.cache_evicted()
            self._std_cache = (key, ws)
        return ws

    def forward(self, x):
        k, st = self.kernel_size[0], self.stride[0]
        ih, iw = x.shape[-2:]
        ph = max((math.ceil(ih / st) - 1) * st + (k - 1) + 1 - ih, 0)
        pw = max((math.ceil(iw / st) - 1) * st + (k - 1) + 1 - iw, 0)
        if ph % 2 == 0 and pw % 2 == 0:
            return F.conv2d(x, self.std_weight(), None, self.stride, (ph // 2, pw // 2))
        x = _pad_same(x, k, st)
        return F.conv2d(x, self.std_weight(), None, self.stride, 0)


GROUPNORM_HIP = os.environ.get("DS_GROUPNORM", "1") != "0"


class GroupNormAct(nn.GroupNorm):
    def __init__(self, ch, apply_act=True):
        super().__init__(32, ch, eps=1e-5)
        self.apply_act = apply_act

    def forward(self, x, res=None, relu_after_res=False):
        if GROUPNORM_HIP and vm.half_on_gpu(x) and not vm.STOCK[0] and not (torch.is_grad_enabled() and x.requires_grad):
            from src import _native
            if not x.is_contiguous():
                x = x.contiguous()
            if res is not None and not res.is_contiguous():
                res = res.contiguous()
            if _native.group_norm_supported(x, self.num_groups):
                return _native.group_norm(x, self.num_groups, self.weight, self.bias, self.eps,
                                          relu=self.apply_act or (res is not None and relu_after_res), res=res)
        x = F.group_norm(x, self.num_groups, self.weight, self.bias, self.eps)
        if res is not None:
            x = x + res
            return F.relu(x) if relu_after_res else x
        return F.relu(x) if self.apply_act else x


class _Downsample(nn.Module):
    def __init__(self, in_ch, out_ch, stride):
        super().__init__()
        self.conv = StdConv2dSame(in_ch, out_ch, 1, stride)
        self.norm = GroupNormAct(out_ch, apply_act=False)

    def forward(self, x):
        return self.norm(self.conv(x))


class _Bottleneck(nn.Module):
    def __init__(self, in_ch, out_ch, stride, downsample):
        super().__init__()
        mid = out_ch // 4
# ... 93 lines not shown
        self.start_index = 1
        self.hybrid = hybrid
        self.patch_embed = _HybridEmbed(embed_dim) if hybrid else _PatchEmbed(embed_dim)
        n = (img_size // 16) ** 2
        self.cls_token = nn.Parameter(torch.zeros(1, 1, embed_dim))
        self.pos_embed = nn.Parameter(torch.zeros(1, n + 1, embed_dim))
        self.blocks = nn.ModuleList([Block(embed_dim, num_heads) for _ in range(depth)])
        self.norm = nn.LayerNorm(embed_dim, eps=1e-6)
        self.head = nn.Linear(embed_dim, num_classes)
        self._pos_cache = {}
        nn.init.trunc_normal_(self.pos_embed, std=0.02)
        nn.init.normal_(self.cls_token, std=1e-6)
        for m in self.modules():
            if isinstance(m, nn.Linear):
                nn.init.trunc_normal_(m.weight, std=0.02)
                nn.init.zeros_(m.bias)

    def resized_pos_embed(self, gs_h, gs_w, dtype):
        key = (gs_h, gs_w, dtype, self.pos_embed.device, self.pos_embed._version)
        hit = self._pos_cache.get(key)
        if hit is not None:
            return hit
        posemb = self.pos_embed
        tok, grid = posemb[:, :1], posemb[0, 1:]
        gs_old = int(math.sqrt(len(grid)))
        grid = grid.reshape(1, gs_old, gs_old, -1).permute(0, 3, 1, 2)
        grid = F.interpolate(grid.float(), size=(gs_h, gs_w), mode="bilinear").to(posemb.dtype)
        grid = grid.permute(0, 2, 3, 1).reshape(1, gs_h * gs_w, -1)
        out = torch.cat([tok, grid], dim=1).to(dtype)
        if not torch.is_grad_enabled():
            vm.cache_store(self._pos_cache, key, out)
        return out

    def forward_taps(self, x, hooks, n_stage_taps):
        b, c, h, w = x.shape
        grid = (h // 16, w // 16)
        stage_outs = []
        if self.hybrid:
            feats = self.patch_embed.backbone.forward_stages(x)
            stage_outs = feats[:n_stage_taps]
            t = self.patch_embed.proj(feats[-1]).flatten(2).transpose(1, 2)
        elif vm.patch_embed_hip_ok(self.patch_embed.proj, x):
            t = vm.patch_embed_tokens(self.patch_embed.proj, x)
        else:
            t = self.patch_embed.proj(x).flatten(2).transpose(1, 2)
        t = torch.cat((self.cls_token.expand(b, -1, -1).to(t.dtype), t), dim=1)
        t = t + self.resized_pos_embed(grid[0], grid[1], t.dtype)
        n_valid = t.shape[1]
        t = vm.pad_tokens(t, vm.pad_len(n_valid, t.shape[0]))
        block_hooks = list(hooks[n_stage_taps:])
        _, taps = vm.run_blocks(self.blocks, t, n_valid, grid, set(block_hooks), padded_taps=True)
        return stage_outs, [taps[i] for i in block_hooks], grid, n_valid


def _token_postprocess(vit_features, out_features, tail):
    return nn.Sequential(ProjectReadout(vit_features), _Skip(), _Skip(), nn.Conv2d(vit_features, out_features, 1), *tail)


class VitBackbone(nn.Module):

    def __init__(self, model, features, vit_features, hooks, number_stages):
        super().__init__()
        self.model = model
        self.hooks = list(hooks)
        self.number_stages = number_stages
        f = features
        posts = []
        for s in range(4):
            if s < number_stages:
                posts.append(nn.Sequential(nn.Identity(), nn.Identity(), nn.Identity()))
                continue
            if number_stages == 0:
                tail = [[nn.ConvTranspose2d(f[0], f[0], 4, 4, 0)], [nn.ConvTranspose2d(f[1], f[1], 2, 2, 0)], [],
                        [nn.Conv2d(f[3], f[3], 3, 2, 1)]][s]
            else:
                tail = [] if s == number_stages else [nn.Conv2d(f[3], f[3], 3, 2, 1)]
            posts.append(_token_postprocess(vit_features, f[s], tail))
        self.act_postprocess1, self.act_postprocess2, self.act_postprocess3, self.act_postprocess4 = posts

    def forward(self, x):
        stage_outs, taps, grid, n_valid = self.model.forward_taps(x, self.hooks, self.number_stages)
        posts = (self.act_postprocess1, self.act_postprocess2, self.act_postprocess3, self.act_postprocess4)
        outs = list(stage_outs)
        for tap, post in zip(taps, posts[self.number_stages:]):
            y = post[0].forward_padded(tap, n_valid)
            y = y.reshape(y.shape[0], grid[0], grid[1], y.shape[2]).permute(0, 3, 1, 2)
            for layer in list(post)[3:]:
                y = vm.conv_module(layer, y)
            outs.append(y)
        return outs


def make_vit(name, hooks):
    if name == "vitl16_384":
        model = VisionTransformer(1024, 24, 16, hybrid=False)
        features = [256, 512, 1024, 1024]
        return VitBackbone(model, features, 1024, hooks, 0), features
    if name == "vitb_rn50_384":
        model = VisionTransformer(768, 12, 12, hybrid=True)
        features = [256, 512, 768, 768]
        return VitBackbone(model, features, 768, hooks, 2), features
    raise KeyError(name)
```

stable-diffusion-webui-depthmap-script_amd/dmidas/dpt_depth.py:

```python
import numpy as np
import torch
import torch.nn as nn
import torch.nn.functional as F

from src import vit_mi355x as vm

from .backbones.beit import make_beit
from .backbones.vit import make_vit

_HOOKS = {"beitl16_512": [5, 11, 17, 23], "beitl16_384": [5, 11, 17, 23], "beitb16_384": [2, 5, 8, 11],
          "vitl16_384": [5, 11, 17, 23], "vitb_rn50_384": [0, 1, 8, 11]}


class ResidualConvUnit_custom(nn.Module):
    def __init__(self, features):
        super().__init__()
        self.conv1 = nn.Conv2d(features, features, kernel_size=3, stride=1, padding=1, bias=True)
        self.conv2 = nn.Conv2d(features, features, kernel_size=3, stride=1, padding=1, bias=True)

    def forward(self, x):
        return vm.residual_conv_unit(self.conv1, self.conv2, x)


class FeatureFusionBlock_custom(nn.Module):
    def __init__(self, features):
        super().__init__()
        self.out_conv = nn.Conv2d(features, features, kernel_size=1, stride=1, padding=0, bias=True)
        self.resConfUnit1 = ResidualConvUnit_custom(features)
        self.resConfUnit2 = ResidualConvUnit_custom(features)

    def forward(self, *xs, size=None):
        output = xs[0]
        if len(xs) == 2:
            output = vm.residual_conv_unit(self.resConfUnit1.conv1, self.resConfUnit1.conv2, xs[1], skip=output)
        output = self.resConfUnit2(output)
        output = vm.conv_module(self.out_conv, output)
        if size is None:
            return vm.interpolate_bilinear(output, scale_factor=2, align_corners=True)
        return vm.interpolate_bilinear(output, size=tuple(size), align_corners=True)


class Interpolate(nn.Module):
    def __init__(self, scale_factor, mode, align_corners=False):
        super().__init__()
        self.scale_factor, self.mode, self.align_corners = scale_factor, mode, align_corners

    def forward(self, x):
        if self.mode == "bilinear":
            return vm.interpolate_bilinear(x, scale_factor=self.scale_factor, align_corners=bool(self.align_corners))
        return F.interpolate(x, scale_factor=self.scale_factor, mode=self.mode, align_corners=self.align_corners)


class DPT(nn.Module):
    def __init__(self, head, features=256, backbone="beitl16_512", readout="project", channels_last=False, use_bn=False, **kwargs):
        super().__init__()
        if backbone not in _HOOKS:
            raise NotImplementedError(f"DPT backbone '{backbone}' is not built (built: {sorted(_HOOKS)})")
        if readout != "project" or use_bn:
            raise NotImplementedError("only readout='project', use_bn=False (what src/depthmap_generation.py:129-176 uses)")
        self.channels_last = channels_last
        self.size_routed = backbone == "vitb_rn50_384"
        make = make_beit if backbone.startswith("beit") else make_vit
        self.pretrained, in_shape = make(backbone, _HOOKS[backbone])
        scratch = nn.Module()
        for i in range(4):
            setattr(scratch, f"layer{i + 1}_rn", nn.Conv2d(in_shape[i], features, kernel_size=3, stride=1, padding=1, bias=False))
        for i in range(1, 5):
            setattr(scratch, f"refinenet{i}", FeatureFusionBlock_custom(features))
        scratch.output_conv = head
        self.scratch = scratch

    def forward(self, x, features=None, rows=None):
        if getattr(self, "size_routed", False):
            with vm.size_routed():
                return self._forward(x, features, rows)
        return self._forward(x, features, rows)

    def _forward(self, x, features=None, rows=None):
        l1, l2, l3, l4 = self.pretrained(x) if rows is None else self.pretrained(x, rows=rows)
        s = self.scratch
        l1, l2, l3, l4 = vm.conv2d(s.layer1_rn, l1), vm.conv2d(s.layer2_rn, l2), vm.conv2d(s.layer3_rn, l3), vm.conv2d(s.layer4_rn, l4)
        path_4 = s.refinenet4(l4, size=l3.shape[2:])
        path_3 = s.refinenet3(path_4, l3, size=l2.shape[2:])
        path_2 = s.refinenet2(path_3, l2, size=l1.shape[2:])
        path_1 = s.refinenet1(path_2, l1)
        head = s.output_conv
        if features is not None:
            features.update(l4_rn=l4, r4=path_4, r3=path_3, r2=path_2, r1=path_1)
            y = path_1
            for i, layer in enumerate(head):
                y = layer(y)
                if i == 3:
                    features['out_conv'] = y
            return y
        if (vm.half_on_gpu(path_1) and isinstance(head[1], Interpolate)
                and head[1].mode == "bilinear" and head[1].align_corners and tuple(head[2].weight.shape) == (32, 128, 3, 3)
                and head[2].padding_mode in ('zeros', 'circular') and vm.circular_hip_ok(head[2])):
            from src import _native
            y = vm.conv2d(head[0], path_1) if vm.conv3x3_hip_ok(head[0], path_1) else vm.conv_module(head[0], path_1)
            size = (int(y.shape[2] * head[1].scale_factor), int(y.shape[3] * head[1].scale_factor))
            return _native.dpt_head_tail(y, size, head[2], head[4], relu_out=isinstance(head[5], nn.ReLU))
        return head(path_1)


def _constrain(x, multiple, min_val=0, max_val=None):
    y = int(np.round(x / multiple) * multiple)
    if max_val is not None and y > max_val:
        y = int(np.floor(x / multiple) * multiple)
    if y < min_val:
        y = int(np.ceil(x / multiple) * multiple)
    return y


def midas_net_size(width, height, net_w, net_h, resize_method="minimal", multiple=32):
    scale_h, scale_w = net_h / height, net_w / width
    if resize_method == "lower_bound":
        scale_h = scale_w = max(scale_w, scale_h)
    elif resize_method == "upper_bound":
        scale_h = scale_w = min(scale_w, scale_h)
    elif resize_method == "minimal":
        if abs(1 - scale_w) < abs(1 - scale_h):
            scale_h = scale_w
        else:
            scale_w = scale_h
    else:
        raise ValueError(f"resize_method {resize_method} not implemented")
    if resize_method == "lower_bound":
        return _constrain(scale_w * width, multiple, min_val=net_w), _constrain(scale_h * height, multiple, min_val=net_h)
    if resize_method == "upper_bound":
        return _constrain(scale_w * width, multiple, max_val=net_w), _constrain(scale_h * height, multiple, max_val=net_h)
    return _constrain(scale_w * width, multiple), _constrain(scale_h * height, multiple)


def _patch_rows(model, images_u8, net_size, net_h, resize_mode, mean, std, dtype):
    from .backbones.beit import BeitBackbone
    pre = getattr(model, "pretrained", None)
    if not (images_u8.is_cuda and isinstance(pre, BeitBackbone)):
        return None
    b, h, w, _ = images_u8.shape
    nw, nh = midas_net_size(w, h, int(net_size), int(net_size if net_h is None else net_h), resize_mode)
    conv = pre.model.patch_embed.proj
    if not (vm.patch_rows_ok(conv, dtype, (nh, nw)) and pre.model.cls_token.dtype == dtype):
        return None
    from src import _native
    grid, _, n_pad, kpad = vm.patch_rows_geometry(conv, (nh, nw), b)
    rows = _native.preprocess_bicubic_rows(images_u8, (nh, nw), mean, std, conv.kernel_size[0], n_pad, kpad, flip=True, dtype=dtype)
    return rows, grid


class DPTDepthModel(DPT):
    def __init__(self, path=None, non_negative=True, **kwargs):
        features = kwargs.get("features", 256)
        head_features_1 = kwargs.pop("head_features_1", features)
        head_features_2 = kwargs.pop("head_features_2", 32)
        head = nn.Sequential(
            nn.Conv2d(head_features_1, head_features_1 // 2, kernel_size=3, stride=1, padding=1),
            Interpolate(scale_factor=2, mode="bilinear", align_corners=True),
            nn.Conv2d(head_features_1 // 2, head_features_2, kernel_size=3, stride=1, padding=1),
            nn.ReLU(True),
            nn.Conv2d(head_features_2, 1, kernel_size=1, stride=1, padding=0),
            nn.ReLU(True) if non_negative else nn.Identity(),
            nn.Identity())
        super().__init__(head, **kwargs)
        if path is not None:
# ... 45 lines not shown
```

stable-diffusion-webui-depthmap-script_amd/src/_native.py:

```python
import collections
import ctypes
import math
import os
import threading

import numpy as np

_PKG_ROOT = os.path.dirname(os.path.dirname(os.path.abspath(__file__)))
LIB_PATH = os.environ.get("DS_NATIVE_LIB") or os.path.join(_PKG_ROOT, "libdepthstereo_hip.so")

DS_DEPTH_U16, DS_DEPTH_F32, DS_DEPTH_F64 = 0, 1, 2
FILL_IDS = {"none": 0, "naive": 1, "naive_interpolating": 2, "polylines_soft": 3, "polylines_sharp": 4}

EXPORTS = [
    "ds_version", "ds_last_error", "ds_normalmap_f64", "ds_normalmap_gradient_f32", "ds_reassemble_readout", "ds_bias_act_nhwc", "ds_linear", "ds_linear_residual", "ds_linear_vt", "ds_linear_qkv", "ds_conv3x3_nhwc", "ds_ctx_create", "ds_ctx_destroy", "ds_stereo_warp", "ds_depth_minmax",
    "ds_stereo_last_exact_rows", "ds_copy_view", "ds_overlap_red_cyan", "ds_normalmap", "ds_depth_to_u16",
    "ds_convert_to_i16", "ds_profile_enable", "ds_profile_last_ms", "ds_stereo_last_stats", "ds_attention_fwd", "ds_attention_bias_pack", "ds_colorize_u16", "ds_residual_layernorm", "ds_boost_blend", "ds_upsample_bilinear_nhwc", "ds_dpt_head_tail", "ds_preprocess_bicubic", "ds_linear_reload_env", "ds_attention_reload_env", "ds_normalmap_selfcheck", "ds_normalmap_gradient_f16", "ds_normalmap_gradient_blur_f32",
    "ds_linear_shuffle", "ds_linear_readout", "ds_kernel_timer_enable", "ds_kernel_timer_read", "ds_kernel_timer_read_each", "ds_group_norm_nchw",
    "ds_row_stats", "ds_linear_ln", "ds_linear_vt_ln", "ds_gconv3x3_nhwc_f32", "ds_add_relu_f32", "ds_bias_act_f32", "ds_relu_cat_f32",
    "ds_dwconv_nhwc", "ds_resize_lanczos", "ds_custom_depth_to_f64", "ds_conv3x3_nhwc_circular", "ds_dpt_head_tail_circular",
    "ds_normalmap_wrap", "ds_normalmap_f64_wrap", "ds_normalmap_gradient_f32_wrap", "ds_normalmap_gradient_f16_wrap", "ds_normalmap_gradient_blur_f32_wrap",
    "ds_bilateral_u16", "ds_frame_luma_hist", "ds_temporal_smooth5_f32",
    "ds_preprocess_bicubic_rows", "ds_tokens_fixup", "ds_upsample_bicubic_to_f32", "ds_im2col3x3_s2_nhwc",
]


class DepthStereoError(RuntimeError):
    pass


class ds_eye(ctypes.Structure):
    _fields_ = [("divergence_px", ctypes.c_double), ("separation_px", ctypes.c_double),
                ("out", ctypes.c_void_p), ("out_row_stride", ctypes.c_int64), ("out_img_stride", ctypes.c_int64)]


_lib = None
_lib_lock = threading.Lock()

CALLS = collections.Counter()


def lib():
    global _lib
    with _lib_lock:
        if _lib is None:
            if not os.path.exists(LIB_PATH):
                raise DepthStereoError(
                    f"{LIB_PATH} is missing: build it with `python __graft_entry__.py build` "
                    "(hipcc --offload-arch=gfx950).  There is no CPU fallback.")
            L = ctypes.CDLL(LIB_PATH)
            vp, ci, cd, i64 = ctypes.c_void_p, ctypes.c_int, ctypes.c_double, ctypes.c_int64
            L.ds_version.restype = ci
            L.ds_last_error.restype = ctypes.c_char_p
            L.ds_ctx_create.argtypes = [ctypes.POINTER(vp), ci]
            L.ds_ctx_destroy.argtypes = [vp]
            L.ds_stereo_warp.argtypes = [vp, vp, vp, ci, ci, ci, ci, ci, cd, vp, ci, ctypes.POINTER(ds_eye), ci, vp]
            L.ds_depth_minmax.argtypes = [vp, vp, ci, ci, ci, ci, vp, vp]
            L.ds_stereo_last_exact_rows.argtypes = [vp, ctypes.POINTER(i64), vp]
            L.ds_copy_view.argtypes = [vp, vp, i64, i64, vp, i64, i64, ci, ci, i64, vp]
            L.ds_overlap_red_cyan.argtypes = [vp, vp, i64, i64, vp, i64, i64, ci, ci, ci, ci, vp, vp]
            L.ds_normalmap.argtypes = [vp, vp, ci, ci, ci, ci, ci, ci, ci, vp, vp]
            L.ds_normalmap_f64.argtypes = [vp, vp, ci, ci, ci, ci, ci, ci, ci, vp, vp]
            L.ds_normalmap_gradient_f32.argtypes = [vp, vp, ci, ci, ci, ci, vp, vp]
            L.ds_normalmap_gradient_f16.argtypes = [vp, vp, ci, ci, ci, ci, vp, vp]
            L.ds_normalmap_gradient_blur_f32.argtypes = [vp, vp, ci, ci, ci, ci, ci, ci, vp, vp]
            for name in ("ds_normalmap", "ds_normalmap_f64", "ds_normalmap_gradient_f32", "ds_normalmap_gradient_f16", "ds_normalmap_gradient_blur_f32"):
                getattr(L, name + "_wrap").argtypes = getattr(L, name).argtypes
            L.ds_bilateral_u16.argtypes = [vp, vp, ci, ci, ci, ci, vp, vp, ci, vp, vp]
            L.ds_frame_luma_hist.argtypes = [vp, vp, ci, ci, ci, ci, vp, vp]
            L.ds_temporal_smooth5_f32.argtypes = [vp, vp, ci, i64, ci, ci, ci, ci, vp, vp]
            L.ds_depth_to_u16.argtypes = [vp, vp, ci, ci, ci, ci, vp, vp, vp]
            L.ds_convert_to_i16.argtypes = [vp, vp, ci, i64, vp, vp]
            L.ds_stereo_last_stats.argtypes = [vp, ctypes.POINTER(i64), vp]
            L.ds_attention_fwd.argtypes = [vp, vp, vp, vp, vp, ci, ci, ci, ci, ctypes.c_float, ci, vp]
            L.ds_normalmap_selfcheck.argtypes = [vp, ctypes.c_ulonglong, ctypes.c_ulonglong, ctypes.c_ulonglong, ctypes.POINTER(ctypes.c_ulonglong), vp]
            L.ds_attention_bias_pack.argtypes = [vp, vp, ci, ci, ci, ci, vp, vp]
            L.ds_colorize_u16.argtypes = [vp, vp, ci, ci, ci, vp, vp, ci, vp, vp]
            L.ds_residual_layernorm.argtypes = [vp, vp, vp, vp, vp, vp, vp, vp, i64, ci, ctypes.c_float, ci, vp]
            L.ds_boost_blend.argtypes = [vp, vp, i64, ci, ci, vp, ci, vp, ci, vp, ci, vp]
            L.ds_upsample_bilinear_nhwc.argtypes = [vp, vp, vp, ci, ci, ci, ci, ci, ci, ci, ci, vp]
            L.ds_dpt_head_tail.argtypes = [vp, vp, ci, ci, ci, ci, ci, vp, vp, vp, ctypes.c_float, ci, vp, ci, vp]
            L.ds_dpt_head_tail_circular.argtypes = L.ds_dpt_head_tail.argtypes
            L.ds_preprocess_bicubic.argtypes = [vp, vp, vp, ci, ci, ci, ci, ci, ci, ctypes.POINTER(ctypes.c_float),
                                                ctypes.POINTER(ctypes.c_float), ci, vp]
            L.ds_preprocess_bicubic_rows.argtypes = [vp, vp, vp, ci, ci, ci, ci, ci, ci, ctypes.POINTER(ctypes.c_float),
                                                     ctypes.POINTER(ctypes.c_float), ci, ci, ci, ci, vp]
            L.ds_tokens_fixup.argtypes = [vp, vp, vp, ci, ci, ci, ci, ci, vp]
            L.ds_upsample_bicubic_to_f32.argtypes = [vp, vp, vp, ci, ci, ci, ci, ci, ci, vp]
            L.ds_im2col3x3_s2_nhwc.argtypes = [vp, vp, vp, ci, ci, ci, ci, ci, ci, vp]
            L.ds_reassemble_readout.argtypes = [vp, vp, vp, vp, ci, ci, ci, ci, vp]
            L.ds_bias_act_nhwc.argtypes = [vp, vp, vp, vp, vp, vp, i64, ci, ci, ci, vp]
            L.ds_group_norm_nchw.argtypes = [vp, vp, vp, vp, vp, vp, ci, ci, ci, ci, ctypes.c_float, ci, ci, vp]
            L.ds_linear.argtypes = [vp, vp, vp, vp, vp, i64, i64, i64, i64, ci, ci, vp]
            L.ds_linear_residual.argtypes = [vp, vp, vp, vp, vp, vp, vp, i64, i64, i64, ci, vp]
            L.ds_linear_vt.argtypes = [vp, vp, vp, vp, i64, i64, i64, i64, ci, vp]
            L.ds_linear_qkv.argtypes = [vp, vp, vp, vp, vp, vp, vp, i64, i64, i64, i64, i64, ci, vp]
            L.ds_conv3x3_nhwc.argtypes = [vp, vp, vp, vp, vp, vp, vp, ci, ci, ci, ci, ci, ci, ci, vp]
            L.ds_conv3x3_nhwc_circular.argtypes = L.ds_conv3x3_nhwc.argtypes
            L.ds_linear_shuffle.argtypes = [vp, vp, vp, vp, vp, i64, i64, ci, ci, ci, ci, vp]
            L.ds_linear_readout.argtypes = [vp, vp, vp, vp, vp, i64, i64, i64, i64, i64, ci, vp]
            L.ds_row_stats.argtypes = [vp, vp, vp, i64, ci, ctypes.c_float, ci, vp]
            L.ds_linear_ln.argtypes = [vp, vp, vp, vp, vp, vp, vp, i64, i64, i64, i64, ci, ci, vp]
            L.ds_linear_vt_ln.argtypes = [vp, vp, vp, vp, vp, vp, i64, i64, i64, i64, ci, vp]
            L.ds_gconv3x3_nhwc_f32.argtypes = [vp, vp, vp, vp, vp, ci, ci, ci, ci, ci, ci, vp]
            L.ds_add_relu_f32.argtypes = [vp, vp, vp, vp, i64, vp]
            L.ds_bias_act_f32.argtypes = [vp, vp, vp, vp, vp, i64, ci, ci, vp]
            L.ds_relu_cat_f32.argtypes = [vp, vp, vp, vp, ci, i64, ci, ci, ci, vp]
            L.ds_dwconv_nhwc.argtypes = [vp, vp, vp, vp, vp, vp, ci, ci, ci, ci, ci, ci, ci, ci, ci, ci, ci, vp]
            L.ds_resize_lanczos.argtypes = [vp, vp, ci, ci, ci, ci, i64, i64, i64, vp, ci, ci, vp, vp, ci, vp, vp, ci, vp, vp]
            L.ds_custom_depth_to_f64.argtypes = [vp, vp, ci, ci, ci, ci, i64, i64, i64, ci, vp, vp, vp]
            L.ds_kernel_timer_enable.argtypes = [vp, ci]
            L.ds_kernel_timer_read.argtypes = [vp, ci, ctypes.POINTER(i64), ctypes.POINTER(cd)]
            L.ds_kernel_timer_read_each.argtypes = [vp, ci, ctypes.POINTER(ctypes.c_float), i64, ctypes.POINTER(i64)]
            L.ds_profile_enable.argtypes = [vp, ci]
            L.ds_profile_last_ms.argtypes = [vp, ctypes.POINTER(ctypes.c_float), ctypes.POINTER(ctypes.c_float)]
            for name in EXPORTS:
                getattr(L, name)
            _lib = L
    return _lib


def _check(rc):
    if rc != 0:
        raise DepthStereoError(f"libdepthstereo_hip error {rc}: {lib().ds_last_error().decode(errors='replace')}")


_ctxs = {}


def ctx_for(device_index):
    key = (threading.get_ident(), int(device_index))
    c = _ctxs.get(key)
    if c is None:
        h = ctypes.c_void_p()
        _check(lib().ds_ctx_create(ctypes.byref(h), int(device_index)))
        _ctxs[key] = c = h
    return c


def _torch():
    import torch
    return torch


def require_gpu():
    torch = _torch()
    if not torch.cuda.is_available():
        raise DepthStereoError("no MI355X visible to torch (torch.cuda.is_available() is False); "
                               "this package has no CPU path")
    return torch


def _stream(t):
    torch = _torch()
    return ctypes.c_void_p(torch.cuda.current_stream(t.device).cuda_stream)


def _dev_index(t):
    torch = _torch()
    return t.device.index if t.device.index is not None else torch.cuda.current_device()


def _depth_dtype_id(t):
    torch = _torch()
    if t.dtype in (torch.uint16, torch.int16):
        return DS_DEPTH_U16
    if t.dtype == torch.float32:
        return DS_DEPTH_F32
    if t.dtype == torch.float64:
        return DS_DEPTH_F64
    raise DepthStereoError(f"unsupported device depth dtype {t.dtype}")


def depth_minmax(depth):
    torch = require_gpu()
    n, h, w = depth.shape
    out = torch.empty((n, 2), dtype=torch.float64, device=depth.device)
    CALLS["ds_depth_minmax"] += 1
    _check(lib().ds_depth_minmax(ctx_for(_dev_index(depth)), depth.data_ptr(), _depth_dtype_id(depth), n, h, w,
                                 out.data_ptr(), _stream(depth)))
    return out


# ... 392 lines not shown
    for k, v in switches.items():
        assert k.startswith("DS_ATT_")
        if v is None:
            os.environ.pop(k, None)
        else:
            os.environ[k] = str(v)
    _check(lib().ds_attention_reload_env())


def linear_supported(x, weight):
    return weight.shape[0] % 256 == 0 and weight.shape[1] % 128 == 0 and 128 <= weight.shape[1] <= 16384 and x.numel() > 0


def linear(x, weight, bias=None, gelu=False):
    torch = require_gpu()
    assert x.is_cuda and x.dtype in (torch.float16, torch.bfloat16) and linear_supported(x, weight)
    k = x.shape[-1]
    n = weight.shape[0]
    assert weight.shape[1] == k
    x2 = x.reshape(-1, k)
    if not x2.is_contiguous():
        x2 = x2.contiguous()
    rows = x2.shape[0]
    if rows < 256:
        x2 = torch.cat([x2, x2.new_zeros((256 - rows, k))])
    w = weight.detach()
    w = w if (w.dtype == x.dtype and w.is_contiguous()) else w.to(x.dtype).contiguous()
    b = None
    if bias is not None:
        b = bias.detach()
        b = b if (b.dtype == x.dtype and b.is_contiguous()) else b.to(x.dtype).contiguous()
    out = torch.empty((x2.shape[0], n), dtype=x.dtype, device=x.device)
    CALLS["ds_linear"] += 1
    _check(lib().ds_linear(ctx_for(_dev_index(x)), x2.data_ptr(), w.data_ptr(), None if b is None else b.data_ptr(),
                           out.data_ptr(), x2.shape[0], n, k, n, 1 if gelu else 0,
                           1 if x.dtype == torch.float16 else 2, _stream(x)))
    return out[:rows].view(x.shape[:-1] + (n,))


def linear_residual(x, weight, bias, gamma, residual):
    torch = require_gpu()
    assert x.is_cuda and x.dtype in (torch.float16, torch.bfloat16) and linear_supported(x, weight)
    k, n = x.shape[-1], weight.shape[0]
    x2 = x.reshape(-1, k).contiguous()
    r2 = residual.reshape(-1, n).contiguous()
    assert x2.shape[0] == r2.shape[0] >= 256 and r2.dtype == x.dtype

    def prep(t):
        if t is None:
            return None
        t = t.detach()
        return t if (t.dtype == x.dtype and t.is_contiguous()) else t.to(x.dtype).contiguous()
    w, b, g = prep(weight), prep(bias), prep(gamma)
    out = torch.empty_like(r2)
    CALLS["ds_linear_residual"] += 1
    _check(lib().ds_linear_residual(ctx_for(_dev_index(x)), x2.data_ptr(), w.data_ptr(), None if b is None else b.data_ptr(),
                                    None if g is None else g.data_ptr(), r2.data_ptr(), out.data_ptr(), x2.shape[0], n, k,
                                    1 if x.dtype == torch.float16 else 2, _stream(x)))
    return out.view(residual.shape)


def linear_readout_supported(x_padded, w_tok):
    return (x_padded.dim() == 3 and x_padded.is_contiguous() and x_padded.shape[0] * x_padded.shape[1] >= 256
            and w_tok.shape[0] % 256 == 0 and w_tok.shape[1] == x_padded.shape[2] and x_padded.shape[2] % 128 == 0
            and 128 <= x_padded.shape[2] <= 16384 and x_padded.shape[0] * x_padded.shape[1] * x_padded.shape[1] < (1 << 32))


def linear_readout(x_padded, n_tokens, w_tok, cls_vec):
    torch = require_gpu()
    assert x_padded.is_cuda and x_padded.dtype in (torch.float16, torch.bfloat16) and linear_readout_supported(x_padded, w_tok)
    b, npad, k = x_padded.shape
    n = w_tok.shape[0]
    assert 2 <= n_tokens <= npad and tuple(cls_vec.shape) == (b, n)
    w = w_tok.detach()
    w = w if (w.dtype == x_padded.dtype and w.is_contiguous()) else w.to(x_padded.dtype).contiguous()
    cv = cls_vec if (cls_vec.dtype == x_padded.dtype and cls_vec.is_contiguous()) else cls_vec.to(x_padded.dtype).contiguous()
    out = torch.empty((b * (n_tokens - 1) + 1, n), dtype=x_padded.dtype, device=x_padded.device)
    CALLS["ds_linear_readout"] += 1
    _check(lib().ds_linear_readout(ctx_for(_dev_index(x_padded)), x_padded.data_ptr(), w.data_ptr(), cv.data_ptr(), out.data_ptr(),
                                   b, npad, n_tokens, n, k, 1 if x_padded.dtype == torch.float16 else 2, _stream(x_padded)))
    return out[:b * (n_tokens - 1)].view(b, n_tokens - 1, n)


def conv_transpose_shuffle_supported(layer, x):
    ks, st = tuple(layer.kernel_size), tuple(layer.stride)
    return (ks == st and ks[0] == ks[1] and 1 <= ks[0] <= 8 and tuple(layer.padding) == (0, 0) and tuple(layer.output_padding) == (0, 0)
            and tuple(layer.dilation) == (1, 1) and layer.groups == 1 and layer.in_channels % 128 == 0 and 128 <= layer.in_channels <= 16384
            and layer.out_channels % 8 == 0 and (ks[0] * ks[0] * layer.out_channels) % 256 == 0 and x.dim() == 4
            and x.shape[1] == layer.in_channels and x.shape[0] * x.shape[2] * x.shape[3] >= 256)


def conv_transpose_shuffle(layer, x):
    torch = require_gpu()
    assert x.is_cuda and x.dtype in (torch.float16, torch.bfloat16) and conv_transpose_shuffle_supported(layer, x)
    x = x.contiguous(memory_format=torch.channels_last)
    b, c, h, w = x.shape
    s, co = layer.stride[0], layer.out_channels
    key = (layer.weight.data_ptr(), layer.weight._version, x.dtype, None if layer.bias is None else layer.bias._version)
    hit = getattr(layer, "_ds_shuffle", None)
    if hit is None or hit[0] != key:
        if hit is not None:
            from . import vit_mi355x as _vm
            _vm.cache_evicted()
        wg = layer.weight.detach().permute(2, 3, 1, 0).reshape(s * s * co, c).to(x.dtype).contiguous()
        bg = None if layer.bias is None else layer.bias.detach().to(x.dtype).repeat(s * s).contiguous()
        hit = (key, wg, bg)
        if not torch.is_grad_enabled():
            layer._ds_shuffle = hit
    _, wg, bg = hit
    out = torch.empty((b, h * s, w * s, co), dtype=x.dtype, device=x.device)
    xr = x.permute(0, 2, 3, 1)
    CALLS["ds_linear_shuffle"] += 1
    _check(lib().ds_linear_shuffle(ctx_for(_dev_index(x)), xr.data_ptr(), wg.data_ptr(), None if bg is None else bg.data_ptr(), out.data_ptr(),
                                   b * h * w, c, w, s, co, 1 if x.dtype == torch.float16 else 2, _stream(x)))
    return out.permute(0, 3, 1, 2)


def gconv3x3_supported(x, weight, stride, padding, dilation, groups):
    torch = _torch()
    if not (x.is_cuda and x.dtype == torch.float32 and x.dim() == 4 and groups > 1 and tuple(weight.shape[2:]) == (3, 3)):
        return False
    c = x.shape[1]
    cpg = c // groups
    return (weight.shape[0] == c and weight.shape[1] == cpg and cpg in (8, 16, 32) and c % 32 == 0 and tuple(stride) == (1, 1)
            and tuple(padding) == (1, 1) and tuple(dilation) == (1, 1) and x.is_contiguous(memory_format=torch.channels_last))


def gconv_weight_image(weight, groups):
    c, cpg = weight.shape[0], weight.shape[1]
    w = weight.detach().float().reshape(groups, c // groups, cpg, 9)
    return w.permute(0, 3, 2, 1).contiguous()


def gconv3x3(x, w_gtio, bias, relu, cpg):
    torch = require_gpu()
    b, c, h, w = x.shape
    assert x.is_cuda and x.dtype == torch.float32 and x.is_contiguous(memory_format=torch.channels_last)
    assert w_gtio.dtype == torch.float32 and w_gtio.is_contiguous() and w_gtio.numel() == (c // cpg) * 9 * cpg * cpg
    bb = None if bias is None else bias.detach().float().contiguous()
    out = torch.empty_like(x, memory_format=torch.channels_last)
    CALLS["ds_gconv3x3_nhwc_f32"] += 1
    _check(lib().ds_gconv3x3_nhwc_f32(ctx_for(_dev_index(x)), x.data_ptr(), w_gtio.data_ptr(), None if bb is None else bb.data_ptr(), out.data_ptr(),
                                      b, h, w, c, cpg, 1 if relu else 0, _stream(x)))
    return out


def add_relu(a, b):
    torch = require_gpu()
    assert a.is_cuda and a.dtype == torch.float32 and b.dtype == torch.float32 and a.shape == b.shape and a.stride() == b.stride()
    assert a.numel() % 4 == 0 and (a.is_contiguous() or a.is_contiguous(memory_format=torch.channels_last))
    out = torch.empty_like(a)
    assert out.stride() == a.stride()
    CALLS["ds_add_relu_f32"] += 1
    _check(lib().ds_add_relu_f32(ctx_for(_dev_index(a)), a.data_ptr(), b.data_ptr(), out.data_ptr(), a.numel(), _stream(a)))
    return out


def bias_act_f32_ok(x, bias, res=None):
    torch = require_gpu()
    if not (x.is_cuda and x.dtype == torch.float32 and bias is not None and bias.dtype == torch.float32 and bias.is_cuda and bias.numel() == x.shape[1]):
        return False
    if not (x.dim() == 4 and x.shape[1] % 4 == 0 and x.is_contiguous(memory_format=torch.channels_last) and x.numel() > 0):
        return False
    return res is None or (res.dtype == torch.float32 and res.shape == x.shape and res.is_cuda and res.is_contiguous(memory_format=torch.channels_last))


# ... 113 lines not shown
    assert w_v_scaled.dtype == x.dtype and w_v_scaled.is_contiguous() and colsum.dtype == torch.float32 and colsum.numel() == c
    assert stats.dtype == torch.float32 and stats.numel() == 2 * b * npad
    out = torch.empty((b, c, npad), dtype=x.dtype, device=x.device)
    CALLS["ds_linear_vt_ln"] += 1
    _check(lib().ds_linear_vt_ln(ctx_for(_dev_index(x)), w_v_scaled.data_ptr(), colsum.data_ptr(), x.data_ptr(), stats.data_ptr(), out.data_ptr(),
                                 c, b, npad, k, 1 if x.dtype == torch.float16 else 2, _stream(x)))
    return out


def linear_vt_supported(w_v, h):
    return (h.dim() == 3 and h.shape[1] % 8 == 0 and (h.shape[0] * h.shape[1]) % 256 == 0 and w_v.shape[0] >= 256
            and w_v.shape[1] == h.shape[2] and h.shape[2] % 128 == 0 and 128 <= h.shape[2] <= 16384
            and h.shape[0] * h.shape[1] * h.shape[1] < (1 << 32))


def linear_vt(w_v, h):
    torch = require_gpu()
    assert h.is_cuda and h.dtype in (torch.float16, torch.bfloat16) and linear_vt_supported(w_v, h)
    b, npad, k = h.shape
    c = w_v.shape[0]
    h2 = h if h.is_contiguous() else h.contiguous()
    w = w_v.detach()
    w = w if (w.dtype == h.dtype and w.is_contiguous()) else w.to(h.dtype).contiguous()
    out = torch.empty((b, c, npad), dtype=h.dtype, device=h.device)
    CALLS["ds_linear_vt"] += 1
    _check(lib().ds_linear_vt(ctx_for(_dev_index(h)), w.data_ptr(), h2.data_ptr(), out.data_ptr(), c, b, npad, k,
                              1 if h.dtype == torch.float16 else 2, _stream(h)))
    return out


def linear_qkv_supported(h, w_qk, w_v):
    return linear_vt_supported(w_v, h) and linear_supported(h, w_qk) and w_qk.shape[1] == h.shape[2]


def linear_qkv(h, w_qk, b_qk, w_v, out=None):
    torch = require_gpu()
    assert h.is_cuda and h.dtype in (torch.float16, torch.bfloat16) and linear_qkv_supported(h, w_qk, w_v)
    b, npad, k = h.shape
    n, c = w_qk.shape[0], w_v.shape[0]
    h2 = h if h.is_contiguous() else h.contiguous()

    def prep(t):
        if t is None:
            return None
        t = t.detach()
        return t if (t.dtype == h.dtype and t.is_contiguous()) else t.to(h.dtype).contiguous()
    wq, bq, wv = prep(w_qk), prep(b_qk), prep(w_v)
    if out is None:
        qk = torch.empty((b, npad, n), dtype=h.dtype, device=h.device)
        vt = torch.empty((b, c, npad), dtype=h.dtype, device=h.device)
    else:
        qk, vt = out
        assert tuple(qk.shape) == (b, npad, n) and tuple(vt.shape) == (b, c, npad) and qk.is_contiguous() and vt.is_contiguous()
        assert qk.dtype == vt.dtype == h.dtype and qk.device == vt.device == h.device
    CALLS["ds_linear_qkv"] += 1
    CALLS["ds_linear"] += 1
    CALLS["ds_linear_vt"] += 1
    _check(lib().ds_linear_qkv(ctx_for(_dev_index(h)), h2.data_ptr(), wq.data_ptr(), None if bq is None else bq.data_ptr(), wv.data_ptr(),
                               qk.data_ptr(), vt.data_ptr(), b, npad, n, c, k, 1 if h.dtype == torch.float16 else 2, _stream(h)))
    return qk, vt


def conv3x3_supported(conv, x):
    return (tuple(conv.kernel_size) == (3, 3) and tuple(conv.stride) == (1, 1) and tuple(conv.padding) == (1, 1)
            and tuple(conv.dilation) == (1, 1) and conv.groups == 1 and conv.padding_mode == 'zeros'
            and conv.in_channels % 128 == 0 and conv.out_channels % 128 == 0 and x.dim() == 4 and x.shape[1] == conv.in_channels
            and x.shape[0] * x.shape[2] * x.shape[3] >= 256)


def conv3x3_circular_supported(conv, x):
    return (tuple(conv.kernel_size) == (3, 3) and tuple(conv.stride) == (1, 1) and tuple(conv.padding) == (1, 1)
            and tuple(conv.dilation) == (1, 1) and conv.groups == 1 and conv.padding_mode == 'circular'
            and conv.in_channels % 128 == 0 and conv.out_channels % 128 == 0 and x.dim() == 4 and x.shape[1] == conv.in_channels
            and x.shape[0] * x.shape[2] * x.shape[3] >= 256)


def conv3x3(conv, x, relu=False, res1=None, res2=None, relu_in=False):
    torch = require_gpu()
    circular = conv.padding_mode == 'circular'
    assert x.is_cuda and x.dtype in (torch.float16, torch.bfloat16)
    assert conv3x3_circular_supported(conv, x) if circular else conv3x3_supported(conv, x)
    x = x.contiguous(memory_format=torch.channels_last)
    b, c, h, w = x.shape
    key = (conv.weight.data_ptr(), conv.weight._version, x.dtype, None if conv.bias is None else conv.bias._version)
    hit = getattr(conv, "_ds_ohwi", None)
    if hit is None or hit[0] != key:
        if hit is not None:
            from . import vit_mi355x as _vm
            _vm.cache_evicted()
        wk = conv.weight.detach().to(x.dtype).permute(0, 2, 3, 1).contiguous()
        bk = None if conv.bias is None else conv.bias.detach().to(x.dtype).contiguous()
        hit = conv._ds_ohwi = (key, wk, bk)
    _, wk, bk = hit
    out = torch.empty((b, conv.out_channels, h, w), dtype=x.dtype, device=x.device, memory_format=torch.channels_last)
    for r in (res1, res2):
        assert r is None or (r.shape == out.shape and r.dtype == x.dtype and r.is_contiguous(memory_format=torch.channels_last))
    name = "ds_conv3x3_nhwc_circular" if circular else "ds_conv3x3_nhwc"
    CALLS[name] += 1
    _check(getattr(lib(), name)(ctx_for(_dev_index(x)), x.data_ptr(), wk.data_ptr(), None if bk is None else bk.data_ptr(),
                                None if res1 is None else res1.data_ptr(), None if res2 is None else res2.data_ptr(),
                                out.data_ptr(), b, h, w, c, conv.out_channels, (2 if relu else 0) | (4 if relu_in else 0),
                                1 if x.dtype == torch.float16 else 2, _stream(x)))
    return out


def bias_act(x, bias, relu=False, res1=None, res2=None, inplace=True):
    torch = require_gpu()
    assert x.is_cuda and x.dtype in (torch.float16, torch.bfloat16) and x.dim() == 4 and x.shape[1] % 8 == 0
    assert x.is_contiguous(memory_format=torch.channels_last)
    for r in (res1, res2):
        assert r is None or (r.shape == x.shape and r.dtype == x.dtype and r.is_contiguous(memory_format=torch.channels_last))
    out = x if inplace else torch.empty_like(x)
    b = bias.detach().to(x.dtype).contiguous()
    CALLS["ds_bias_act_nhwc"] += 1
    _check(lib().ds_bias_act_nhwc(ctx_for(_dev_index(x)), x.data_ptr(), b.data_ptr(), None if res1 is None else res1.data_ptr(),
                                  None if res2 is None else res2.data_ptr(), out.data_ptr(), x.numel(), x.shape[1], 1 if relu else 0,
                                  1 if x.dtype == torch.float16 else 2, _stream(x)))
    return out


def group_norm_supported(x, groups):
    torch = _torch()
    return (x.is_cuda and x.dtype in (torch.float16, torch.bfloat16) and x.dim() == 4 and x.is_contiguous() and x.shape[1] % groups == 0
            and (x.shape[2] * x.shape[3]) % 8 == 0 and x.shape[0] * groups <= 4096 and x.data_ptr() % 16 == 0)


def group_norm(x, groups, weight, bias, eps, relu=False, res=None):
    torch = require_gpu()
    assert group_norm_supported(x, groups)
    assert res is None or (res.shape == x.shape and res.dtype == x.dtype and res.is_contiguous() and res.data_ptr() % 16 == 0)
    out = torch.empty_like(x)
    g, b = weight.detach().to(x.dtype).contiguous(), bias.detach().to(x.dtype).contiguous()
    CALLS["ds_group_norm_nchw"] += 1
    _check(lib().ds_group_norm_nchw(ctx_for(_dev_index(x)), x.data_ptr(), g.data_ptr(), b.data_ptr(), None if res is None else res.data_ptr(),
                                    out.data_ptr(), x.shape[0], x.shape[1], x.shape[2] * x.shape[3], int(groups), float(eps), 1 if relu else 0,
                                    1 if x.dtype == torch.float16 else 2, _stream(x)))
    return out


def boost_blend(dst, rects, coefs, preds, mask_template):
    torch = require_gpu()
    assert dst.is_cuda and dst.dtype == torch.float32 and dst.dim() == 2 and dst.stride(1) == 1
    n = len(rects)
    if n == 0:
        return dst
    preds = preds.contiguous()
    mask_template = mask_template.contiguous()
    assert preds.dtype == torch.float32 and preds.shape[0] == n and preds.shape[1] == preds.shape[2]
    assert mask_template.dtype == torch.float32 and mask_template.shape[0] == mask_template.shape[1]
    rec = np.zeros(n, dtype=[('x0', '<i4'), ('y0', '<i4'), ('w', '<i4'), ('h', '<i4'), ('p0', '<f8'), ('p1', '<f8')])
    for i, (r, c) in enumerate(zip(rects, coefs)):
        rec[i] = (int(r[0]), int(r[1]), int(r[2]), int(r[3]), float(c[0]), float(c[1]))
    buf = torch.from_numpy(rec.view(np.uint8).copy()).to(dst.device)
    CALLS["ds_boost_blend"] += 1
    _check(lib().ds_boost_blend(ctx_for(_dev_index(dst)), dst.data_ptr(), dst.stride(0), dst.shape[0], dst.shape[1],
                                buf.data_ptr(), n, preds.data_ptr(), preds.shape[1], mask_template.data_ptr(),
                                mask_template.shape[0], _stream(dst)))
    return dst


def preprocess_bicubic(images_u8, size_hw, mean, std, flip=True, dtype=None):
    torch = require_gpu()
    assert images_u8.is_cuda and images_u8.dtype == torch.uint8 and images_u8.dim() == 4 and images_u8.shape[3] == 3
    dtype = torch.float32 if dtype is None else dtype
    code = {torch.float16: 1, torch.bfloat16: 2, torch.float32: 3}[dtype]
    x = images_u8.contiguous()
    b, h, w, _ = x.shape
    oh, ow = int(size_hw[0]), int(size_hw[1])
    out = torch.empty((b, 3, oh, ow), dtype=dtype, device=x.device, memory_format=torch.channels_last)
    m = (ctypes.c_float * 3)(*[float(v) for v in (mean if hasattr(mean, "__len__") else (mean,) * 3)])
    s = (ctypes.c_float * 3)(*[float(v) for v in (std if hasattr(std, "__len__") else (std,) * 3)])
    CALLS["ds_preprocess_bicubic"] += 1
    _check(lib().ds_preprocess_bicubic(ctx_for(_dev_index(x)), x.data_ptr(), out.data_ptr(), b, h, w, oh, ow, 1 if flip else 0, m, s, code,
                                       _stream(x)))
    return out


def preprocess_bicubic_rows(images_u8, size_hw, mean, std, patch, n_pad, kpad, flip=True, dtype=None, out=None):
    torch = require_gpu()
    assert images_u8.is_cuda and images_u8.dtype == torch.uint8 and images_u8.dim() == 4 and images_u8.shape[3] == 3
    code = {torch.float16: 1, torch.bfloat16: 2}[dtype]
    x = images_u8.contiguous()
    b, h, w, _ = x.shape
    oh, ow = int(size_hw[0]), int(size_hw[1])
    if out is None:
        out = torch.empty((b, int(n_pad), int(kpad)), dtype=dtype, device=x.device)
# ... 88 lines not shown
```

stable-diffusion-webui-depthmap-script_amd/src/vit_mi355x.py:

```python
import contextlib
import functools
import math
import os
import threading

import torch
import torch.nn as nn
import torch.nn.functional as F

HEAD_DIM = 64
SEQ_ALIGN = 64

_CONSTANTS = {}

CACHE_EPOCH = [0]
SIZE_CACHE_ENTRIES = 6


def cache_evicted():
    CACHE_EPOCH[0] += 1


def cache_store(cache, key, value, entries=None):
    if len(cache) >= (SIZE_CACHE_ENTRIES if entries is None else entries):
# ... 308 lines not shown

def run_blocks(blocks, x, n_valid, grid_hw, take, padded_taps=False):
    taps = {}
    fast = half_on_gpu(x)
    if not fast:
        for i, blk in enumerate(blocks):
            x = blk.forward_padded(x, n_valid, grid_hw)
            if i in take:
                taps[i] = x if padded_taps else x[:, :n_valid]
        return x, taps
    if _ln_fold_ok(blocks, x):
        return _run_blocks_ln_fold(blocks, x, n_valid, grid_hw, take, padded_taps)
    from . import _native
    n = len(blocks)
    _, h = _native.residual_layernorm(x, None, None, blocks[0].norm1.weight, blocks[0].norm1.bias, blocks[0].norm1.eps)
    big = hip_gemm_ok(x.shape[0] * x.shape[1], x.shape[2])
    for i, blk in enumerate(blocks):
        g1, g2 = blk.gammas()
        pr = getattr(getattr(blk, "attn", None), "proj", None)
        if (LINEAR_HIP in ("proj", "all") and pr is not None and big and _native.linear_supported(x, pr.weight)):
            o, b_v = blk.attend_o(h, n_valid, grid_hw)
            x = _native.linear_residual(o, pr.weight, folded_proj_bias(pr, b_v), g1, x)
            _, h2 = _native.residual_layernorm(x, None, None, blk.norm2.weight, blk.norm2.bias, blk.norm2.eps)
        else:
            p = blk.attend(h, n_valid, grid_hw)
            x, h2 = _native.residual_layernorm(x, p, g1, blk.norm2.weight, blk.norm2.bias, blk.norm2.eps)
        mlp = blk.mlp
        fused_fc2 = (LINEAR_HIP == "all" and isinstance(mlp, Mlp) and big and _native.linear_supported(x, mlp.fc2.weight)
                     and _native.linear_supported(h2, mlp.fc1.weight) and mlp.fc2.bias is not None)
        if fused_fc2:
            a = _native.linear(h2, mlp.fc1.weight, mlp.fc1.bias, True)
            x = _native.linear_residual(a, mlp.fc2.weight, mlp.fc2.bias, g2, x)
            if i + 1 < n:
                nxt = blocks[i + 1].norm1
                _, h = _native.residual_layernorm(x, None, None, nxt.weight, nxt.bias, nxt.eps)
        else:
            m = mlp(h2)
            if i + 1 < n:
                nxt = blocks[i + 1].norm1
                x, h = _native.residual_layernorm(x, m, g2, nxt.weight, nxt.bias, nxt.eps)
            else:
                x = x + (m if g2 is None else g2 * m)
        if i in take:
            taps[i] = x if padded_taps else x[:, :n_valid]
    return x, taps


PATCH_ROWS = os.environ.get("DS_PATCH_ROWS", "1") != "0"
DEPTH_TAIL = os.environ.get("DS_DEPTH_TAIL", "1") != "0"
IM2COL_HIP = os.environ.get("DS_IM2COL", "1") != "0"


def interpolate_bilinear(x, size=None, scale_factor=None, align_corners=True):
    if half_on_gpu(x) and x.shape[1] % 8 == 0:
        from . import _native
        return _native.upsample_bilinear(x, size=size, scale_factor=scale_factor, align_corners=align_corners)
    if size is not None:
        return F.interpolate(x, size=size, mode="bilinear", align_corners=align_corners)
    return F.interpolate(x, scale_factor=scale_factor, mode="bilinear", align_corners=align_corners)


CONV_HIP = os.environ.get("DS_CONV", "1") != "0"
CONV_HIP_MIN_TILES = int(os.environ.get("DS_CONV_MIN_TILES", 48))
CONV_HEAD_HIP = os.environ.get("DS_CONV_HEAD", "1") != "0"
CONV_RELU_IN = os.environ.get("DS_CONV_RELU_IN", "1") != "0"
CONV_CIRCULAR_HIP = os.environ.get("DS_CONV_CIRCULAR", "1") != "0"


def circular_hip_ok(conv):
    return CONV_CIRCULAR_HIP or getattr(conv, "padding_mode", "zeros") != "circular"


def conv3x3_hip_ok(conv, x):
    if not (CONV_HIP and half_on_gpu(x) and x.dim() == 4):
        return False
    from . import _native
    if conv.out_channels % 256 != 0 and not CONV_HEAD_HIP:
        return False
    tiles = (x.shape[0] * x.shape[2] * x.shape[3] + 255) // 256 * ((conv.out_channels + 255) // 256)
    supported = _native.conv3x3_supported(conv, x) or (CONV_CIRCULAR_HIP and _native.conv3x3_circular_supported(conv, x))
    return supported and tiles >= (1 if invariant() else CONV_HIP_MIN_TILES)


def conv2d(conv, x):
    if conv3x3_hip_ok(conv, x):
        from . import _native
        return _native.conv3x3(conv, x)
    return conv(x)


CONV_BIAS_HIP = os.environ.get("DS_CONV_BIAS", "1") != "0"
CONV1X1_HIP = os.environ.get("DS_CONV1X1", "1") != "0"
CONVT_HIP = os.environ.get("DS_CONVT", "1") != "0"
READOUT_HIP = os.environ.get("DS_READOUT", "1") != "0"
CONV1X1_MIN_TILES = int(os.environ.get("DS_CONV1X1_MIN_TILES", 96))


def conv1x1_hip_ok(layer, x):
    if not (CONV1X1_HIP and LINEAR_HIP == "all" and half_on_gpu(x) and x.dim() == 4 and type(layer) is nn.Conv2d):
        return False
    if not (tuple(layer.kernel_size) == (1, 1) and tuple(layer.stride) == (1, 1) and tuple(layer.padding) == (0, 0) and layer.groups == 1
            and tuple(layer.dilation) == (1, 1)):
        return False
    pixels = x.shape[0] * x.shape[2] * x.shape[3]
    return (layer.out_channels % 256 == 0 and layer.in_channels % 128 == 0 and 128 <= layer.in_channels <= 16384 and pixels >= 256
            and ((pixels + 255) // 256) * (layer.out_channels // 256) >= (1 if invariant() else CONV1X1_MIN_TILES)
            and x.is_contiguous(memory_format=torch.channels_last))


def conv1x1(layer, x):
    from . import _native
    b, c, h, w = x.shape
    rows = x.permute(0, 2, 3, 1).reshape(b * h * w, c)
    y = _native.linear(rows, layer.weight.reshape(layer.out_channels, c), layer.bias)
    return y.view(b, h, w, layer.out_channels).permute(0, 3, 1, 2)


def conv_transpose_hip_ok(layer, x):
    if not (CONVT_HIP and LINEAR_HIP == "all" and half_on_gpu(x) and x.dim() == 4 and type(layer) is nn.ConvTranspose2d):
        return False
    from . import _native
    if not (_native.conv_transpose_shuffle_supported(layer, x) and x.is_contiguous(memory_format=torch.channels_last)):
        return False
    pixels = x.shape[0] * x.shape[2] * x.shape[3]
    n = layer.stride[0] * layer.stride[0] * layer.out_channels
    return ((pixels + 255) // 256) * (n // 256) >= (1 if invariant() else CONV1X1_MIN_TILES)


def _gemm_weight(layer, x, kpad):
    w = layer.weight
    key = (w.data_ptr(), w._version, x.dtype, kpad)
    cache = getattr(layer, "_ds_gemm_weight", None)
    if cache is None or cache[0] != key:
        wm = w.detach().permute(0, 2, 3, 1).reshape(w.shape[0], -1).to(x.dtype)
        if wm.shape[1] != kpad:
            wm = torch.cat([wm, wm.new_zeros((wm.shape[0], kpad - wm.shape[1]))], 1)
        cache = (key, wm.contiguous())
        layer._ds_gemm_weight = cache
    return cache[1]


def patch_embed_hip_ok(conv, x):
    if not (invariant() and LINEAR_HIP == "all" and half_on_gpu(x) and x.dim() == 4 and type(conv) is nn.Conv2d):
        return False
    k = conv.kernel_size
    return (k[0] == k[1] and tuple(conv.stride) == tuple(k) and tuple(conv.padding) == (0, 0) and conv.groups == 1
            and tuple(conv.dilation) == (1, 1) and conv.out_channels % 256 == 0 and x.shape[1] == conv.in_channels
            and x.shape[2] >= k[0] and x.shape[3] >= k[1] and x.is_contiguous(memory_format=torch.channels_last))


def patch_embed_tokens(conv, x):
    from . import _native
    b, c, h, w = x.shape
    p = conv.kernel_size[0]
    gh, gw = h // p, w // p
    k = p * p * c
    kpad = (k + 127) // 128 * 128
    xv = x.permute(0, 2, 3, 1)[:, :gh * p, :gw * p].reshape(b, gh, p, gw, p, c).permute(0, 1, 3, 2, 4, 5)
    if kpad == k:
        rows = xv.reshape(b * gh * gw, k)
    else:
        rows = x.new_zeros((b * gh * gw, kpad))
        rows[:, :k] = xv.reshape(b * gh * gw, k)
    y = _native.linear(rows, _gemm_weight(conv, x, kpad), conv.bias)
    return y.view(b, gh * gw, conv.out_channels)


def patch_rows_ok(conv, dtype, size_hw):
    if not (PATCH_ROWS and PREPROCESS_HIP and not STOCK[0] and invariant() and LINEAR_HIP == "all" and type(conv) is nn.Conv2d
            and dtype in (torch.float16, torch.bfloat16) and conv.weight.dtype == dtype):
        return False
    k = conv.kernel_size
    return (k[0] == k[1] and k[0] <= 32 and tuple(conv.stride) == tuple(k) and tuple(conv.padding) == (0, 0) and conv.groups == 1
            and tuple(conv.dilation) == (1, 1) and conv.out_channels % 256 == 0 and conv.in_channels == 3
            and size_hw[0] >= k[0] and size_hw[1] >= k[1])


# ... 114 lines not shown
```

Measured before the change: 909.7 pairs/s.

## Batch paired 3x3 convs and four readout CLS linears into single launches

Adds a two-segment persistent conv3x3 kernel variant that runs two independent same-channel convolutions (with different spatial sizes) in one launch. It also adds a grouped small-row linear kernel that handles up to four tiny GEMMs, such as the readout CLS projections, in one grid. The goal is to cut launch overhead and fill the device better for small DPT refinenet/readout layers, which on their own leave many CUs idle. The cost is extra per-tile index arithmetic and a padded output row per conv buffer. The call sites in the model code are only partly visible.

```diff
diff --git a/include/depthstereo.h b/include/depthstereo.h
--- a/include/depthstereo.h
+++ b/include/depthstereo.h
@@ -178,6 +178,20 @@
 int ds_linear_readout(ds_ctx *ctx, const void *x, const void *w_tok, const void *cls_vec, void *y, int64_t images,
                       int64_t tokens_padded, int64_t tokens, int64_t out_features, int64_t in_features, int dtype, void *stream);
 
+int ds_conv3x3_nhwc_pair(ds_ctx *ctx, const void *x0, const void *w0, void *y0, int batch0, int height0, int width0,
+                         const void *x1, const void *w1, void *y1, int batch1, int height1, int width1,
+                         int in_channels, int out_channels, int dtype, void *stream);
+
+typedef struct ds_rows_problem {
+    const void *x;
+    int64_t x_row_pitch;
+    const void *w;
+    const void *bias;
+    void *y;
+} ds_rows_problem;
+int ds_linear_rows4(ds_ctx *ctx, const ds_rows_problem *problems, int count, int64_t rows, int64_t out_features,
+                    int64_t in_features, int dtype, void *stream);
+
 int ds_row_stats(ds_ctx *ctx, const void *x, void *stats, int64_t rows, int channels, float eps, int dtype, void *stream);
 int ds_linear_ln(ds_ctx *ctx, const void *x, const void *w_scaled, const float *colsum, const void *bias, const void *stats, void *y,
                  int64_t rows, int64_t out_features, int64_t in_features, int64_t ldy, int act, int dtype, void *stream);
diff --git a/stable-diffusion-webui-depthmap-script_amd/csrc/ds_linear.hip b/stable-diffusion-webui-depthmap-script_amd/csrc/ds_linear.hip
--- a/stable-diffusion-webui-depthmap-script_amd/csrc/ds_linear.hip
+++ b/stable-diffusion-webui-depthmap-script_amd/csrc/ds_linear.hip
@@ -87,6 +87,7 @@
     const void *x1, *w1;
     void *y1;
     int seg_t0, M1, nbm1, nbn1;
+    int H1, W1;
 };
 typedef const __attribute__((address_space(4))) LinParams *LinParamsK;
 __device__ __forceinline__ LinParamsK ln_kernarg()
@@ -227,7 +228,9 @@
 
     static_assert(VT != 4 || (EPI == 0 && CONV == 0 && RES == 0 && NH == 0), "the two-segment tile list is built for the plain dense epilogue");
     int bm0 = 0, bn0 = 0;
+    static_assert(VT != 5 || (EPI == 0 && CONV == 1 && RES == 0 && NH == 0), "the convolution pair is built for the plain zero-padded convolution");
     int seg = 0;
+    int curW = 0;
     const unsigned char *xb = nullptr, *wb = nullptr;
     unsigned okA = 0;
     auto set_tile = [&](const int orig) {
@@ -244,6 +247,29 @@
                 return;
             }
         }
+        if constexpr (VT == 5) {
+            const LinParamsK pk = ln_kernarg();
+            const int t0 = pk->seg_t0;
+            seg = tile >= t0 ? 1 : 0;
+            const int ms = seg ? pk->M1 : pk->M, hs = seg ? pk->H1 : pk->H, ws = seg ? pk->W1 : pk->W;
+            ln_tile_origin(seg ? pk->nbm1 : pk->nbm, pk->nbn, ms, 256, tile - (seg ? t0 : 0), bm0, bn0);
+            bm0 = max(bm0, 0);
+            xb = (const unsigned char *)(seg ? pk->x1 : pk->x) + (size_t)bm0 * rowbytes;
+            wb = (const unsigned char *)(seg ? pk->w1 : pk->w) + (size_t)bn0 * K * sizeof(T);
+            curW = ws;
+            okA = 0;
+#pragma unroll
+            for (int i = 0; i < 2; ++i)
+#pragma unroll
+                for (int h = 0; h < 2; ++h) {
+                    const unsigned row = (unsigned)(bm0 + rowA[i] + 64 * h);
+                    const unsigned pix = row % (unsigned)(hs * ws);
+                    const int py = (int)(pix / (unsigned)ws), px = (int)(pix % (unsigned)ws);
+                    const unsigned bits = (py > 0 ? 1u : 0u) | 2u | (py < hs - 1 ? 4u : 0u) | (px > 0 ? 8u : 0u) | 16u | (px < ws - 1 ? 32u : 0u);
+                    okA |= (row < (unsigned)ms ? bits : 0u) << (6 * (2 * h + i));
+                }
+            return;
+        }
         ln_tile_origin(P, tile, bm0, bn0);
         xb = (const unsigned char *)P.x + (size_t)bm0 * rowbytes;
         wb = (const unsigned char *)P.w + (size_t)bn0 * K * sizeof(T);
@@ -270,7 +296,7 @@
         if (CONV) {               \
             const int cc_ = ((kt) * 7282) >> 16, tap_ = (kt) - 9 * cc_;       \
             dy_ = ((tap_ * 11) >> 5) - 1; dx_ = tap_ - 3 * (dy_ + 1) - 1;                                                \
-            aoff_ = cc_ * 128 + (dy_ * P.W + dx_) * rowbytes;                                                            \
+            aoff_ = cc_ * 128 + (dy_ * (VT == 5 ? curW : P.W) + dx_) * rowbytes;                                         \
             koff_ = (unsigned)(tap_ * P.cpt + cc_) * 128u;                            \
             if (CONV >= 3) { wrapy_ = -(long)dy_ * ((long)P.H * P.W * rowbytes); wrapx_ = -(long)dx_ * ((long)P.W * rowbytes); } \
         }                                                                                                                \
@@ -469,7 +495,7 @@
         if (wr == 0) LN_BARRIER();
     }
     const int cbm0 = bm0, cbn0 = bn0;
-    const bool cseg = VT == 4 && seg != 0;
+    const bool cseg = (VT == 4 || VT == 5) && seg != 0;
     const int next = orig + (int)gridDim.x;
     int elane = lane;
     if constexpr (VT == 4) asm volatile("" : "+v"(elane));
@@ -485,11 +511,19 @@
             s1_np = (unsigned)pk->vt_np; s1_c = (unsigned)pk->vt_c; s1_magic = pk->vt_magic;
         }
     }
+    int s1_rows = 0;
+    if constexpr (VT == 5) {
+        const LinParamsK pk = ln_kernarg();
+        yb = (T *)(cseg ? pk->y1 : pk->y);
+        s1_rows = cseg ? pk->M1 : pk->M;
+    }
     auto tile_out_off = [&](const int row, const int col, const size_t o0) -> size_t {
         if constexpr (VT == 4) {
             if (!cseg) return o0;
             const unsigned b = __umulhi((unsigned)col, s1_magic), n = (unsigned)col - b * s1_np;
             return ((size_t)b * s1_c + row) * (size_t)s1_np + n;
+        } else if constexpr (VT == 5) {
+            return row < s1_rows ? o0 : (size_t)s1_rows * P.ldy + col;
         } else return VT ? ln_out_off<VT>(P, row, col) : o0;
     };
     if constexpr (CONV >= 3) asm volatile("" : "+s"(yb));
@@ -1018,9 +1052,6 @@
         TH_STEP(fa1, fb1, fa0, fb0, st + 1);
     }
     if (st < nst) TH_STEP(fa0, fb0, fa1, fb1, st);
-#undef TH_STEP
-#undef TH_READ
-#undef TH_STAGE
     LN_WAIT_VM(0);
     if (!mw) return;
 
@@ -1058,6 +1089,109 @@
         *(V8 *)(yb + off) = o;
     }
 }
+
+struct LinRows4 {
+    const void *x[4], *w[4], *bias[4];
+    void *y[4];
+    long long pitch[4];
+    int rows, N, K;
+};
+template <int BF16>
+__global__ __launch_bounds__(LN_THREADS) void k_linear_rows4(LinRows4 P)
+{
+    typedef ln_traits<BF16> TR;
+    typedef typename TR::T T;
+    typedef typename TR::V8 V8;
+    constexpr int S = 6;
+    extern __shared__ __attribute__((aligned(1024))) unsigned char lds[];
+    const int tid = threadIdx.x, lane = tid & 63, l31 = lane & 31, hi = lane >> 5;
+    const int wid = __builtin_amdgcn_readfirstlane(tid >> 6);
+    const __attribute__((address_space(4))) LinRows4 *pk = (const __attribute__((address_space(4))) LinRows4 *)__builtin_amdgcn_kernarg_segment_ptr();
+    const int prob = (int)blockIdx.y;
+    const int ncb = P.N >> 6;
+    const int rb = (int)blockIdx.x / ncb, cbk = (int)blockIdx.x - rb * ncb;
+    const int row0 = 32 * rb, col0 = cbk * 64, rows = P.rows;
+    const int K = P.K, nst = K >> 7;
+    const unsigned rowbytes = (unsigned)K * (unsigned)sizeof(T);
+    const unsigned pitch = (unsigned)pk->pitch[prob];
+    unsigned srcA, srcB[2];
+    {
+        const int j = 8 * (wid & 3) + (lane >> 3);
+        const int jr = min(row0 + j, rows - 1) - row0;
+        srcA = (unsigned)jr * pitch + (unsigned)(((lane & 7) ^ ((j >> 1) & 7)) << 4) + (unsigned)(wid >> 2) * 128u;
+    }
+#pragma unroll
+    for (int i = 0; i < 2; ++i) {
+        const int j = 8 * ((2 * wid + i) & 7) + (lane >> 3);
+        srcB[i] = (unsigned)j * rowbytes + (unsigned)(((lane & 7) ^ ((j >> 1) & 7)) << 4) + (unsigned)(wid >> 2) * 128u;
+    }
+    const unsigned char *xb = (const unsigned char *)pk->x[prob] + (size_t)row0 * pitch;
+    const unsigned char *wb = (const unsigned char *)pk->w[prob] + (size_t)col0 * rowbytes;
+    const unsigned lds0 = (unsigned)(size_t)(__attribute__((address_space(3))) void *)lds;
+    const bool mw = wid < 2;
+    unsigned offA[8], offB[8];
+#pragma unroll
+    for (int u = 0; u < 8; ++u) {
+        const int j = u >> 2, ks = u & 3;
+        const unsigned sl = (unsigned)((LN_MF16 ? 4 * (ks >> 1) + (lane >> 4) : 2 * ks + hi) ^ ((lane >> 1) & 7)) << 4;
+        const int lrow = LN_MF16 ? 16 * (ks & 1) + (lane & 15) : l31;
+        offA[u] = (unsigned)j * 4096u + (unsigned)lrow * 128u + sl;
+        offB[u] = 8192u + (unsigned)j * 8192u + (unsigned)((wid & 1) * 32 + lrow) * 128u + sl;
+    }
+    LN_SMALL_ACC(mine);
+    const int e_row = row0 + LN_SMALL_ROW;
+    const int e_cb = col0 + (wid & 1) * 32 + LN_SMALL_COL;
+    const T *bias = (const T *)pk->bias[prob];
+    V8 e_bv[2];
+    if (mw && bias) {
+#pragma unroll
+        for (int k = 0; k < 2; ++k) e_bv[k] = *(const V8 *)(bias + e_cb + LN_SMALL_DCOL(k));
+    }
+#pragma unroll
+    for (int t = 0; t < S - 1; ++t) TH_STAGE(t);
+    V8 fa0[8], fb0[8], fa1[8], fb1[8];
+    LN_WAIT_VM(12);
+    LN_BARRIER();
+    if (mw) {
+        TH_READ(fa0, fb0, 0);
+        __builtin_amdgcn_sched_barrier(0);
+        LN_WAIT_LGKM0();
+        __builtin_amdgcn_sched_barrier(0);
+    }
+    int st = 0;
+    for (; st + 1 < nst; st += 2) {
+        TH_STEP(fa0, fb0, fa1, fb1, st);
+        TH_STEP(fa1, fb1, fa0, fb0, st + 1);
+    }
+    if (st < nst) TH_STEP(fa0, fb0, fa1, fb1, st);
+    LN_WAIT_VM(0);
+    if (!mw) return;
+
+    T *yb = (T *)pk->y[prob];
+#pragma unroll
+    for (int k = 0; k < 2; ++k) {
+        const int row = e_row + LN_SMALL_DROW(k), col = e_cb + LN_SMALL_DCOL(k);
+        V8 bv;
+        if (bias) bv = e_bv[k];
+        else {
+#pragma unroll
+            for (int t = 0; t < 8; ++t) bv[t] = (T)0.f;
+        }
+        float v[8];
+        LN_SMALL_V(v, mine, k);
+        V8 o;
+#pragma unroll
+        for (int t = 0; t < 8; t += 2) {
+            const lf32x2 u = {v[t] + (float)bv[t], v[t + 1] + (float)bv[t + 1]};
+            o[t] = (T)u[0];
+            o[t + 1] = (T)u[1];
+        }
+        if (row < rows) *(V8 *)(yb + (size_t)row * P.N + col) = o;
+    }
+}
+#undef TH_STEP
+#undef TH_READ
+#undef TH_STAGE
 
 struct LinOptions { int early, grid, ragged, ragged_den, ragged_ring, ragged_ksplit, ragged_ksplit_min, ragged_ksplit_keep, ragged_pipe, ragged_thin; };
 static LinOptions g_lin_options;
@@ -1389,6 +1523,76 @@
                                     int batch, int height, int width, int in_channels, int out_channels, int act, int dtype, void *stream)
 {
     return ln_conv3x3<1>("ds_conv3x3_nhwc_circular", ctx, x, w, bias, res1, res2, y, batch, height, width, in_channels, out_channels, act, dtype, stream);
+}
+
+template <int BF16>
+static int ln_launch_conv_pair(ds_ctx *ctx, const LinParams &P0, hipStream_t stream)
+{
+    static std::atomic<uint64_t> attr_done{0};
+    auto fn = k_linear256<BF16, 0, 1, 0, 5>;
+    DS_HIP_CHECK(hipSetDevice(ctx->device));
+    const uint64_t bit = 1ull << (ctx->device & 63);
+    if (!(attr_done.load(std::memory_order_relaxed) & bit)) {
+        DS_HIP_CHECK(hipFuncSetAttribute((const void *)fn, hipFuncAttributeMaxDynamicSharedMemorySize, LN_LDS_BYTES));
+        attr_done.fetch_or(bit, std::memory_order_relaxed);
+    }
+    if (!ctx->ncu) {
+        int ncu = 0;
+        DS_HIP_CHECK(hipDeviceGetAttribute(&ncu, hipDeviceAttributeMultiprocessorCount, ctx->device));
+        ctx->ncu = ncu >= 8 ? ncu / 8 * 8 : 8;
+    }
+    const LinOptions &O = ln_options();
+    int grid = ctx->ncu;
+    if (O.grid >= 8) grid = O.grid / 8 * 8;
+    LinParams P = P0;
+    P.bnw = 256;
+    P.early = O.early;
+    P.n_main = P.seg_t0 + P.nbm1 * P.nbn;
+    const int kt0 = ds_kt_begin(ctx, DS_KT_CONV3X3, stream);
+    hipLaunchKernelGGL(fn, dim3(P.n_main < grid ? P.n_main : grid), dim3(LN_THREADS), LN_LDS_BYTES, stream, P);
+    ds_kt_end(ctx, DS_KT_CONV3X3, kt0, stream);
+    DS_HIP_CHECK(hipGetLastError());
+    return DS_OK;
+}
+
+DS_API int ds_conv3x3_nhwc_pair(ds_ctx *ctx, const void *x0, const void *w0, void *y0, int batch0, int height0, int width0,
+                                const void *x1, const void *w1, void *y1, int batch1, int height1, int width1,
+                                int in_channels, int out_channels, int dtype, void *stream)
+{
+    const char *NAME = "ds_conv3x3_nhwc_pair";
+    DS_REQUIRE(ctx && x0 && w0 && y0 && x1 && w1 && y1, DS_EINVAL, "%s: null argument", NAME);
+    DS_REQUIRE(batch0 > 0 && height0 > 0 && width0 > 0 && height0 < 32768 && width0 < 32768 &&
+               batch1 > 0 && height1 > 0 && width1 > 0 && height1 < 32768 && width1 < 32768, DS_EINVAL, "%s: bad image shape", NAME);
+    const int64_t m0 = (int64_t)batch0 * height0 * width0, m1 = (int64_t)batch1 * height1 * width1;
+    DS_REQUIRE(m0 < (1ll << 31) - 256 && m1 < (1ll << 31) - 256 && (m0 + 255) / 256 + (m1 + 255) / 256 < (1ll << 20), DS_EINVAL,
+               "%s: too many pixels", NAME);
+    DS_REQUIRE(in_channels >= 64 && in_channels % 64 == 0 && (9 * in_channels / 64) % 2 == 0 && in_channels <= 4096, DS_EINVAL,
+               "%s: in_channels must be a multiple of 128 (<= 4096)", NAME);
+    DS_REQUIRE(out_channels > 0 && out_channels % 256 == 0, DS_EINVAL, "%s: out_channels must be a multiple of 256", NAME);
+    DS_REQUIRE(dtype == DS_DTYPE_F16 || dtype == DS_DTYPE_BF16, DS_EINVAL, "%s: dtype must be f16 or bf16", NAME);
+    DS_REQUIRE((((uintptr_t)x0 | (uintptr_t)w0 | (uintptr_t)y0 | (uintptr_t)x1 | (uintptr_t)w1 | (uintptr_t)y1) & 15) == 0, DS_EINVAL,
+               "%s: every pointer must be 16-byte aligned", NAME);
+    int rc = ds_ctx_reserve(ctx, &ctx->zero_line, &ctx->zero_line_bytes, 256);
+    if (rc != DS_OK) return rc;
+    if (!ctx->zero_line_cleared) {
+        DS_HIP_CHECK(hipMemsetAsync(ctx->zero_line, 0, 256, (hipStream_t)stream));
+        DS_HIP_CHECK(hipStreamSynchronize((hipStream_t)stream));
+        ctx->zero_line_cleared = 1;
+    }
+    LinParams P;
+    memset(&P, 0, sizeof(P));
+    P.x = x0; P.w = w0; P.y = y0; P.zeros = ctx->zero_line;
+    P.M = (int)m0; P.N = out_channels; P.K = 9 * in_channels;
+    P.nbm = (int)((m0 + 255) / 256); P.nbn = out_channels / 256;
+    P.H = height0; P.W = width0; P.C = in_channels; P.cpt = in_channels / 64; P.magic = 65536 / P.cpt + 1;
+    for (int kt = 0; kt < P.K / 64; ++kt)
+        DS_REQUIRE(((kt * 7282) >> 16) == kt / 9, DS_EUNSUPPORTED, "%s: K-tile arithmetic does not cover %d channels", NAME, in_channels);
+    P.ldy = out_channels;
+    P.x1 = x1; P.w1 = w1; P.y1 = y1;
+    P.seg_t0 = P.nbm * P.nbn; P.M1 = (int)m1; P.nbm1 = (int)((m1 + 255) / 256); P.nbn1 = P.nbn;
+    P.H1 = height1; P.W1 = width1;
+    P.kt_kind = DS_KT_CONV3X3;
+    return dtype == DS_DTYPE_F16 ? ln_launch_conv_pair<0>(ctx, P, (hipStream_t)stream) : ln_launch_conv_pair<1>(ctx, P, (hipStream_t)stream);
 }
 
 DS_API int ds_linear_vt(ds_ctx *ctx, const void *w_v, const void *h, void *vt, int64_t channels, int64_t batch, int64_t tokens,
@@ -1510,6 +1714,52 @@
     return dtype == DS_DTYPE_F16 ? ln_launch<0, 1, 0, 1, 3>(ctx, P, st) : ln_launch<1, 1, 0, 1, 3>(ctx, P, st);
 }
 
+template <int BF16>
+static int ln_launch_rows4(ds_ctx *ctx, const LinRows4 &P, int count, hipStream_t stream)
+{
+    static std::atomic<uint64_t> attr_done{0};
+    auto fn = k_linear_rows4<BF16>;
+    DS_HIP_CHECK(hipSetDevice(ctx->device));
+    const uint64_t bit = 1ull << (ctx->device & 63);
+    if (!(attr_done.load(std::memory_order_relaxed) & bit)) {
+        DS_HIP_CHECK(hipFuncSetAttribute((const void *)fn, hipFuncAttributeMaxDynamicSharedMemorySize, 6 * RG_SLOT));
+        attr_done.fetch_or(bit, std::memory_order_relaxed);
+    }
+    const int kt0 = ds_kt_begin(ctx, DS_KT_LINEAR, stream);
+    hipLaunchKernelGGL(fn, dim3((unsigned)((P.rows + 31) / 32 * (P.N / 64)), (unsigned)count), dim3(LN_THREADS), 6 * RG_SLOT, stream, P);
+    ds_kt_end(ctx, DS_KT_LINEAR, kt0, stream);
+    DS_HIP_CHECK(hipGetLastError());
+    return DS_OK;
+}
+
+DS_API int ds_linear_rows4(ds_ctx *ctx, const ds_rows_problem *problems, int count, int64_t rows, int64_t out_features,
+                           int64_t in_features, int dtype, void *stream)
+{
+    DS_REQUIRE(ctx && problems, DS_EINVAL, "ds_linear_rows4: null argument");
+    DS_REQUIRE(count >= 1 && count <= 4, DS_EINVAL, "ds_linear_rows4: count must be 1 .. 4");
+    DS_REQUIRE(rows >= 1 && rows <= 65536, DS_EINVAL, "ds_linear_rows4: rows must be 1 .. 65536");
+    DS_REQUIRE(out_features > 0 && out_features % 64 == 0 && out_features <= 65536, DS_EINVAL,
+               "ds_linear_rows4: out_features must be a multiple of 64 (<= 65536)");
+    DS_REQUIRE(in_features >= 128 && in_features % 128 == 0 && in_features <= 16384, DS_EINVAL,
+               "ds_linear_rows4: in_features must be a multiple of 128 (<= 16384)");
+    DS_REQUIRE(dtype == DS_DTYPE_F16 || dtype == DS_DTYPE_BF16, DS_EINVAL, "ds_linear_rows4: dtype must be f16 or bf16");
+    DS_REQUIRE((rows + 31) / 32 * (out_features / 64) < (1ll << 31), DS_EINVAL, "ds_linear_rows4: too many pieces for one grid");
+    LinRows4 P;
+    memset(&P, 0, sizeof(P));
+    for (int p = 0; p < count; ++p) {
+        const ds_rows_problem &q = problems[p];
+        DS_REQUIRE(q.x && q.w && q.y, DS_EINVAL, "ds_linear_rows4: null x, w or y");
+        DS_REQUIRE(((uintptr_t)q.x & 15) == 0 && ((uintptr_t)q.w & 15) == 0 && ((uintptr_t)q.y & 15) == 0 && ((uintptr_t)q.bias & 15) == 0, DS_EINVAL,
+                   "ds_linear_rows4: x, w (the LDS-DMA sources), y and bias must be 16-byte aligned");
+        DS_REQUIRE(q.x_row_pitch >= in_features && q.x_row_pitch % 8 == 0 && q.x_row_pitch * 2 * 32 < (1ll << 31), DS_EINVAL,
+                   "ds_linear_rows4: x_row_pitch must be >= in_features, a multiple of 8 elements and below 2^25 elements");
+        P.x[p] = q.x; P.w[p] = q.w; P.bias[p] = q.bias; P.y[p] = q.y;
+        P.pitch[p] = q.x_row_pitch * 2;
+    }
+    P.rows = (int)rows; P.N = (int)out_features; P.K = (int)in_features;
+    return dtype == DS_DTYPE_F16 ? ln_launch_rows4<0>(ctx, P, count, (hipStream_t)stream) : ln_launch_rows4<1>(ctx, P, count, (hipStream_t)stream);
+}
+
 DS_API int ds_linear_ln(ds_ctx *ctx, const void *x, const void *w_scaled, const float *colsum, const void *bias, const void *stats, void *y,
                         int64_t rows, int64_t out_features, int64_t in_features, int64_t ldy, int act, int dtype, void *stream)
 {
diff --git a/stable-diffusion-webui-depthmap-script_amd/ddepth_anything_v2/depth_anything_v2/dpt.py b/stable-diffusion-webui-depthmap-script_amd/ddepth_anything_v2/depth_anything_v2/dpt.py
--- a/stable-diffusion-webui-depthmap-script_amd/ddepth_anything_v2/depth_anything_v2/dpt.py
+++ b/stable-diffusion-webui-depthmap-script_amd/ddepth_anything_v2/depth_anything_v2/dpt.py
@@ -71,7 +71,8 @@
             out.append(x)
         l1, l2, l3, l4 = out
         s = self.scratch
-        l1, l2, l3, l4 = vm.conv2d(s.layer1_rn, l1), vm.conv2d(s.layer2_rn, l2), vm.conv2d(s.layer3_rn, l3), vm.conv2d(s.layer4_rn, l4)
+        l1, l2 = vm.conv2d(s.layer1_rn, l1), vm.conv2d(s.layer2_rn, l2)
+        l3, l4 = vm.conv2d_pair(s.layer3_rn, l3, s.layer4_rn, l4)
         path_4 = s.refinenet4(l4, size=l3.shape[2:])
         path_3 = s.refinenet3(path_4, l3, size=l2.shape[2:])
         path_2 = s.refinenet2(path_3, l2, size=l1.shape[2:])
diff --git a/stable-diffusion-webui-depthmap-script_amd/dmidas/backbones/beit.py b/stable-diffusion-webui-depthmap-script_amd/dmidas/backbones/beit.py
--- a/stable-diffusion-webui-depthmap-script_amd/dmidas/backbones/beit.py
+++ b/stable-diffusion-webui-depthmap-script_amd/dmidas/backbones/beit.py
@@ -218,11 +218,18 @@
             return _native.reassemble_readout(proj, clsvec)
         return F.gelu(proj[:, 1:] + clsvec[:, None])
 
-    def forward_padded(self, xp, n_valid):
+    def takes_hip_route(self, xp):
+        from src import _native
+        w_tok = self._split()[0]
+        return (self.start_index == 1 and vm.READOUT_HIP and vm.LINEAR_HIP == "all" and vm.half_on_gpu(xp) and xp.is_contiguous()
+                and _native.linear_readout_supported(xp, w_tok) and vm.hip_gemm_ok(xp.shape[0] * xp.shape[1], w_tok.shape[0]))
+
+    def forward_padded(self, xp, n_valid, clsvec=None):
         from src import _native
         w_tok, w_cls = self._split()
-        if (self.start_index == 1 and vm.READOUT_HIP and vm.LINEAR_HIP == "all" and vm.half_on_gpu(xp) and xp.is_contiguous()
-                and _native.linear_readout_supported(xp, w_tok) and vm.hip_gemm_ok(xp.shape[0] * xp.shape[1], w_tok.shape[0])):
+        if self.takes_hip_route(xp):
+            if clsvec is not None:
+                return _native.linear_readout(xp, n_valid, w_tok, clsvec)
             x0 = xp[:, 0].contiguous()
             if vm.invariant() and _native.linear_supported(x0, w_cls):
                 clsvec = _native.linear(x0, w_cls, self.project[0].bias)
@@ -232,6 +239,17 @@
         return self.forward(xp[:, :n_valid])
 
 
+def cls_vectors4(readouts, taps):
+    from src import _native
+    none = [None] * len(taps)
+    if not (vm.READOUT_CLS4 and vm.invariant() and 1 <= len(taps) <= 4 and all(r.takes_hip_route(t) for r, t in zip(readouts, taps))):
+        return none
+    w_cls = [r._split()[1] for r in readouts]
+    if not (all(_native.linear_supported(t[:, 0], w) for t, w in zip(taps, w_cls)) and _native.linear_rows4_supported(taps, w_cls)):
+        return none
+    return _native.linear_rows4(taps, w_cls, [r.project[0].bias for r in readouts])
+
+
 class _Skip(nn.Module):
     def forward(self, x):
         return x
@@ -259,8 +277,10 @@
         else:
             taps, grid, n_valid = self.model.forward_taps(x, self.hooks, padded=True)
         outs = []
-        for tap, post in zip(taps, (self.act_postprocess1, self.act_postprocess2, self.act_postprocess3, self.act_postprocess4)):
-            y = post[0].forward_padded(tap, n_valid)
+        posts = (self.act_postprocess1, self.act_postprocess2, self.act_postprocess3, self.act_postprocess4)
+        clsvecs = cls_vectors4([post[0] for post in posts], taps)
+        for tap, post, clsvec in zip(taps, posts, clsvecs):
+            y = post[0].forward_padded(tap, n_valid, clsvec)
             y = y.reshape(y.shape[0], grid[0], grid[1], y.shape[2]).permute(0, 3, 1, 2)
             for layer in list(post)[3:]:
                 y = vm.conv_module(layer, y)
diff --git a/stable-diffusion-webui-depthmap-script_amd/dmidas/backbones/vit.py b/stable-diffusion-webui-depthmap-script_amd/dmidas/backbones/vit.py
--- a/stable-diffusion-webui-depthmap-script_amd/dmidas/backbones/vit.py
+++ b/stable-diffusion-webui-depthmap-script_amd/dmidas/backbones/vit.py
@@ -6,7 +6,7 @@
 import torch.nn.functional as F
 
 from src import vit_mi355x as vm
-from .beit import ProjectReadout, _Skip
+from .beit import ProjectReadout, _Skip, cls_vectors4
 
 
 def _pad_same(x, k, s, value=0.0):
@@ -266,8 +266,9 @@
         stage_outs, taps, grid, n_valid = self.model.forward_taps(x, self.hooks, self.number_stages)
         posts = (self.act_postprocess1, self.act_postprocess2, self.act_postprocess3, self.act_postprocess4)
         outs = list(stage_outs)
-        for tap, post in zip(taps, posts[self.number_stages:]):
-            y = post[0].forward_padded(tap, n_valid)
+        clsvecs = cls_vectors4([post[0] for post in posts[self.number_stages:]], taps)
+        for tap, post, clsvec in zip(taps, posts[self.number_stages:], clsvecs):
+            y = post[0].forward_padded(tap, n_valid, clsvec)
             y = y.reshape(y.shape[0], grid[0], grid[1], y.shape[2]).permute(0, 3, 1, 2)
             for layer in list(post)[3:]:
                 y = vm.conv_module(layer, y)
diff --git a/stable-diffusion-webui-depthmap-script_amd/dmidas/dpt_depth.py b/stable-diffusion-webui-depthmap-script_amd/dmidas/dpt_depth.py
--- a/stable-diffusion-webui-depthmap-script_amd/dmidas/dpt_depth.py
+++ b/stable-diffusion-webui-depthmap-script_amd/dmidas/dpt_depth.py
@@ -79,7 +79,8 @@
     def _forward(self, x, features=None, rows=None):
         l1, l2, l3, l4 = self.pretrained(x) if rows is None else self.pretrained(x, rows=rows)
         s = self.scratch
-        l1, l2, l3, l4 = vm.conv2d(s.layer1_rn, l1), vm.conv2d(s.layer2_rn, l2), vm.conv2d(s.layer3_rn, l3), vm.conv2d(s.layer4_rn, l4)
+        l1, l2 = vm.conv2d(s.layer1_rn, l1), vm.conv2d(s.layer2_rn, l2)
+        l3, l4 = vm.conv2d_pair(s.layer3_rn, l3, s.layer4_rn, l4)
         path_4 = s.refinenet4(l4, size=l3.shape[2:])
         path_3 = s.refinenet3(path_4, l3, size=l2.shape[2:])
         path_2 = s.refinenet2(path_3, l2, size=l1.shape[2:])
diff --git a/stable-diffusion-webui-depthmap-script_amd/src/_native.py b/stable-diffusion-webui-depthmap-script_amd/src/_native.py
--- a/stable-diffusion-webui-depthmap-script_amd/src/_native.py
+++ b/stable-diffusion-webui-depthmap-script_amd/src/_native.py
@@ -16,7 +16,7 @@
     "ds_version", "ds_last_error", "ds_normalmap_f64", "ds_normalmap_gradient_f32", "ds_reassemble_readout", "ds_bias_act_nhwc", "ds_linear", "ds_linear_residual", "ds_linear_vt", "ds_linear_qkv", "ds_conv3x3_nhwc", "ds_ctx_create", "ds_ctx_destroy", "ds_stereo_warp", "ds_depth_minmax",
     "ds_stereo_last_exact_rows", "ds_copy_view", "ds_overlap_red_cyan", "ds_normalmap", "ds_depth_to_u16",
     "ds_convert_to_i16", "ds_profile_enable", "ds_profile_last_ms", "ds_stereo_last_stats", "ds_attention_fwd", "ds_attention_bias_pack", "ds_colorize_u16", "ds_residual_layernorm", "ds_boost_blend", "ds_upsample_bilinear_nhwc", "ds_dpt_head_tail", "ds_preprocess_bicubic", "ds_linear_reload_env", "ds_attention_reload_env", "ds_normalmap_selfcheck", "ds_normalmap_gradient_f16", "ds_normalmap_gradient_blur_f32",
-    "ds_linear_shuffle", "ds_linear_readout", "ds_kernel_timer_enable", "ds_kernel_timer_read", "ds_kernel_timer_read_each", "ds_group_norm_nchw",
+    "ds_linear_shuffle", "ds_linear_readout", "ds_linear_rows4", "ds_conv3x3_nhwc_pair", "ds_kernel_timer_enable", "ds_kernel_timer_read", "ds_kernel_timer_read_each", "ds_group_norm_nchw",
     "ds_row_stats", "ds_linear_ln", "ds_linear_vt_ln", "ds_gconv3x3_nhwc_f32", "ds_add_relu_f32", "ds_bias_act_f32", "ds_relu_cat_f32",
     "ds_dwconv_nhwc", "ds_resize_lanczos", "ds_custom_depth_to_f64", "ds_conv3x3_nhwc_circular", "ds_dpt_head_tail_circular",
     "ds_normalmap_wrap", "ds_normalmap_f64_wrap", "ds_normalmap_gradient_f32_wrap", "ds_normalmap_gradient_f16_wrap", "ds_normalmap_gradient_blur_f32_wrap",
@@ -27,6 +27,11 @@
 
 class DepthStereoError(RuntimeError):
     pass
+
+
+class ds_rows_problem(ctypes.Structure):
+    _fields_ = [("x", ctypes.c_void_p), ("x_row_pitch", ctypes.c_int64), ("w", ctypes.c_void_p), ("bias", ctypes.c_void_p),
+                ("y", ctypes.c_void_p)]
 
 
 class ds_eye(ctypes.Structure):
@@ -97,8 +102,10 @@
             L.ds_linear_qkv.argtypes = [vp, vp, vp, vp, vp, vp, vp, i64, i64, i64, i64, i64, ci, vp]
             L.ds_conv3x3_nhwc.argtypes = [vp, vp, vp, vp, vp, vp, vp, ci, ci, ci, ci, ci, ci, ci, vp]
             L.ds_conv3x3_nhwc_circular.argtypes = L.ds_conv3x3_nhwc.argtypes
+            L.ds_conv3x3_nhwc_pair.argtypes = [vp, vp, vp, vp, ci, ci, ci, vp, vp, vp, ci, ci, ci, ci, ci, ci, vp]
             L.ds_linear_shuffle.argtypes = [vp, vp, vp, vp, vp, i64, i64, ci, ci, ci, ci, vp]
             L.ds_linear_readout.argtypes = [vp, vp, vp, vp, vp, i64, i64, i64, i64, i64, ci, vp]
+            L.ds_linear_rows4.argtypes = [vp, ctypes.POINTER(ds_rows_problem), ci, i64, i64, i64, ci, vp]
             L.ds_row_stats.argtypes = [vp, vp, vp, i64, ci, ctypes.c_float, ci, vp]
             L.ds_linear_ln.argtypes = [vp, vp, vp, vp, vp, vp, vp, i64, i64, i64, i64, ci, ci, vp]
             L.ds_linear_vt_ln.argtypes = [vp, vp, vp, vp, vp, vp, i64, i64, i64, i64, ci, vp]
@@ -657,6 +664,39 @@
     return out[:b * (n_tokens - 1)].view(b, n_tokens - 1, n)
 
 
+def linear_rows4_supported(taps, weights):
+    t0, w0 = taps[0], weights[0]
+    return (1 <= len(taps) == len(weights) <= 4 and t0.dim() == 3 and 1 <= t0.shape[0] <= 65536
+            and all(t.shape == t0.shape and t.dtype == t0.dtype and t.device == t0.device and t.is_contiguous() for t in taps)
+            and all(w.shape == w0.shape for w in weights) and w0.shape[1] == t0.shape[2] and w0.shape[0] % 64 == 0
+            and w0.shape[1] % 128 == 0 and 128 <= w0.shape[1] <= 16384 and t0.shape[1] * t0.shape[2] < (1 << 25))
+
+
+def linear_rows4(taps, weights, biases, out=None):
+    torch = require_gpu()
+    t0 = taps[0]
+    assert t0.is_cuda and t0.dtype in (torch.float16, torch.bfloat16) and linear_rows4_supported(taps, weights) and len(biases) == len(taps)
+    b, npad, k = t0.shape
+    n = weights[0].shape[0]
+
+    def prep(t):
+        if t is None:
+            return None
+        t = t.detach()
+        return t if (t.dtype == t0.dtype and t.is_contiguous()) else t.to(t0.dtype).contiguous()
+    ws, bs = [prep(w) for w in weights], [prep(v) for v in biases]
+    if out is None:
+        out = torch.empty((len(taps), b, n), dtype=t0.dtype, device=t0.device)
+    assert tuple(out.shape) == (len(taps), b, n) and out.dtype == t0.dtype and out.device == t0.device and out.is_contiguous()
+    probs = (ds_rows_problem * len(taps))()
+    for i, (t, w, v) in enumerate(zip(taps, ws, bs)):
+        probs[i] = ds_rows_problem(t.data_ptr(), npad * k, w.data_ptr(), None if v is None else v.data_ptr(), out[i].data_ptr())
+    CALLS["ds_linear_rows4"] += 1
+    CALLS["ds_linear"] += len(taps)
+    _check(lib().ds_linear_rows4(ctx_for(_dev_index(t0)), probs, len(taps), b, n, k, 1 if t0.dtype == torch.float16 else 2, _stream(t0)))
+    return list(out.unbind(0))
+
+
 def conv_transpose_shuffle_supported(layer, x):
     ks, st = tuple(layer.kernel_size), tuple(layer.stride)
     return (ks == st and ks[0] == ks[1] and 1 <= ks[0] <= 8 and tuple(layer.padding) == (0, 0) and tuple(layer.output_padding) == (0, 0)
@@ -936,16 +976,7 @@
     assert conv3x3_circular_supported(conv, x) if circular else conv3x3_supported(conv, x)
     x = x.contiguous(memory_format=torch.channels_last)
     b, c, h, w = x.shape
-    key = (conv.weight.data_ptr(), conv.weight._version, x.dtype, None if conv.bias is None else conv.bias._version)
-    hit = getattr(conv, "_ds_ohwi", None)
-    if hit is None or hit[0] != key:
-        if hit is not None:
-            from . import vit_mi355x as _vm
-            _vm.cache_evicted()
-        wk = conv.weight.detach().to(x.dtype).permute(0, 2, 3, 1).contiguous()
-        bk = None if conv.bias is None else conv.bias.detach().to(x.dtype).contiguous()
-        hit = conv._ds_ohwi = (key, wk, bk)
-    _, wk, bk = hit
+    wk, bk = _conv_weight_image(conv, x.dtype)
     out = torch.empty((b, conv.out_channels, h, w), dtype=x.dtype, device=x.device, memory_format=torch.channels_last)
     for r in (res1, res2):
         assert r is None or (r.shape == out.shape and r.dtype == x.dtype and r.is_contiguous(memory_format=torch.channels_last))
@@ -956,6 +987,49 @@
                                 out.data_ptr(), b, h, w, c, conv.out_channels, (2 if relu else 0) | (4 if relu_in else 0),
                                 1 if x.dtype == torch.float16 else 2, _stream(x)))
     return out
+
+
+def _conv_weight_image(conv, dtype):
+    key = (conv.weight.data_ptr(), conv.weight._version, dtype, None if conv.bias is None else conv.bias._version)
+    hit = getattr(conv, "_ds_ohwi", None)
+    if hit is None or hit[0] != key:
+        if hit is not None:
+            from . import vit_mi355x as _vm
+            _vm.cache_evicted()
+        wk = conv.weight.detach().to(dtype).permute(0, 2, 3, 1).contiguous()
+        bk = None if conv.bias is None else conv.bias.detach().to(dtype).contiguous()
+        hit = conv._ds_ohwi = (key, wk, bk)
+    return hit[1], hit[2]
+
+
+def conv3x3_pair_supported(conv0, x0, conv1, x1):
+    def one(conv, x):
+        return (tuple(conv.kernel_size) == (3, 3) and tuple(conv.stride) == (1, 1) and tuple(conv.padding) == (1, 1)
+                and tuple(conv.dilation) == (1, 1) and conv.groups == 1 and conv.padding_mode == 'zeros' and conv.bias is None
+                and x.dim() == 4 and x.shape[1] == conv.in_channels and x.numel() > 0)
+    return (one(conv0, x0) and one(conv1, x1) and conv0.in_channels == conv1.in_channels and conv0.in_channels % 128 == 0
+            and conv0.in_channels <= 4096 and conv0.out_channels == conv1.out_channels and conv0.out_channels % 256 == 0
+            and x0.dtype == x1.dtype and x0.device == x1.device)
+
+
+def conv3x3_pair(conv0, x0, conv1, x1):
+    torch = require_gpu()
+    assert x0.is_cuda and x0.dtype in (torch.float16, torch.bfloat16) and conv3x3_pair_supported(conv0, x0, conv1, x1)
+    outs, args, xs = [], [], []
+    for conv, x in ((conv0, x0), (conv1, x1)):
+        x = x.contiguous(memory_format=torch.channels_last)
+        b, c, h, w = x.shape
+        wk, _ = _conv_weight_image(conv, x.dtype)
+        n = conv.out_channels
+        buf = torch.empty((b * h * w + 1, n), dtype=x.dtype, device=x.device)
+        outs.append(buf[:b * h * w].view(b, h, w, n).permute(0, 3, 1, 2))
+        args += [x.data_ptr(), wk.data_ptr(), buf.data_ptr(), b, h, w]
+        xs.append(x)
+    CALLS["ds_conv3x3_nhwc_pair"] += 1
+    CALLS["ds_conv3x3_nhwc"] += 2
+    _check(lib().ds_conv3x3_nhwc_pair(ctx_for(_dev_index(x0)), *args, conv0.in_channels, conv0.out_channels,
+                                      1 if x0.dtype == torch.float16 else 2, _stream(x0)))
+    return outs[0], outs[1]
 
 
 def bias_act(x, bias, relu=False, res1=None, res2=None, inplace=True):
diff --git a/stable-diffusion-webui-depthmap-script_amd/src/vit_mi355x.py b/stable-diffusion-webui-depthmap-script_amd/src/vit_mi355x.py
--- a/stable-diffusion-webui-depthmap-script_amd/src/vit_mi355x.py
+++ b/stable-diffusion-webui-depthmap-script_amd/src/vit_mi355x.py
@@ -414,6 +414,19 @@
     return supported and tiles >= (1 if invariant() else CONV_HIP_MIN_TILES)
 
 
+CONV_PAIR = os.environ.get("DS_CONV_PAIR", "1") != "0"
+
+
+def conv2d_pair(conv0, x0, conv1, x1):
+    if CONV_PAIR and conv3x3_hip_ok(conv0, x0) and conv3x3_hip_ok(conv1, x1):
+        from . import _native
+        if _native.conv3x3_pair_supported(conv0, x0, conv1, x1):
+            tiles = sum((x.shape[0] * x.shape[2] * x.shape[3] + 255) // 256 for x in (x0, x1)) * (conv0.out_channels // 256)
+            if tiles <= torch.cuda.get_device_properties(x0.device).multi_processor_count // 8 * 8:
+                return _native.conv3x3_pair(conv0, x0, conv1, x1)
+    return conv2d(conv0, x0), conv2d(conv1, x1)
+
+
 def conv2d(conv, x):
     if conv3x3_hip_ok(conv, x):
         from . import _native
@@ -425,6 +438,7 @@
 CONV1X1_HIP = os.environ.get("DS_CONV1X1", "1") != "0"
 CONVT_HIP = os.environ.get("DS_CONVT", "1") != "0"
 READOUT_HIP = os.environ.get("DS_READOUT", "1") != "0"
+READOUT_CLS4 = os.environ.get("DS_READOUT_CLS4", "1") != "0"
 CONV1X1_MIN_TILES = int(os.environ.get("DS_CONV1X1_MIN_TILES", 96))
 
 
```

After: 919.5 pairs/s (median of 6 runs). 1.1% higher.
